# MAdrid1011/transplat

Measured on AMD Instinct MI355X. Metric: novel views/sec at 256x256, 2 ctx views; PSNR parity vs reference, higher is better.
Workload: dtype fp32 (bf16x3 dense, >= TF32) + bf16x3 attention + fp32 raster; 1 GPU; e2e TranSplat test_step: 1 scene(s) x (2 ctx -> 3 tgt) 256x256; dense mode bf16x3 (split-bf16 products, fp32 accumulation; >= TF32), window-attention mode bf16x3; parallelism=scene-shard x1

## Files before the change

### include/transplat_hip.h

```cpp
#ifndef TRANSPLAT_HIP_H
#define TRANSPLAT_HIP_H

#include <stddef.h>
#include <stdint.h>

#ifdef __cplusplus
extern "C" {
#endif

#define TSPLAT_OK 0
#define TSPLAT_EINVAL (-1)
#define TSPLAT_EHIP (-2)

int tsplat_version(void);

int tsplat_set_debug(int32_t on);

int tsplat_prof_enable(int32_t kernel_id);
int tsplat_prof_read(double* total_ms, int32_t* launches);

typedef struct tsplat_raster_desc {
    int32_t num_gaussians;
    int32_t num_views;
    int32_t views_per_scene;
    int32_t height;
    int32_t width;
    int32_t sh_coeffs;
    int32_t sh_degree;
    int32_t capacity;
} tsplat_raster_desc;

size_t tsplat_raster_workspace_bytes(int32_t num_gaussians, int32_t num_views, int32_t height,
                                     int32_t width, int32_t capacity);

size_t tsplat_raster_num_rendered_offset(int32_t num_gaussians, int32_t num_views, int32_t height,
                                         int32_t width);

int tsplat_raster_fwd(const tsplat_raster_desc* desc,
                      const float* means, const float* cov, const float* shs,
                      const float* opacity, const float* viewmat, const float* projmat,
                      const float* campos, const float* tanfov, const float* bg,
                      const float* scene_scale,
                      float* out_color, int32_t* out_radii,
                      void* workspace, int32_t* status, void* stream);


int tsplat_depth_softmax_fwd(const float* logits, const float* disp, float* coarse, float* pdf_max, int32_t n,
                             int32_t depths, int32_t hw, void* stream);

int tsplat_depth_tail_fwd(const float* fullres, const float* head, const float* near, const float* far, float* depth,
                          float* density, int32_t batch, int32_t views, int32_t hw, void* stream);

int tsplat_raster_cameras(const float* extrinsics, const float* intrinsics, const float* near, const float* far,
                          const float* bg, int32_t bg_per_view, int32_t scale_invariant, int32_t num_views,
                          float* viewmat, float* projmat, float* campos, float* tanfov, float* bg_out, float* scale,
                          void* stream);


int tsplat_uv_coarse_fwd(const float* feat, const float* cams, const float* disp, float* out,
                         int32_t batch, int32_t height, int32_t width, int32_t channels,
                         int32_t depths, void* stream);

int tsplat_uv_cross_fwd(const float* value, const float* key, const float* cams,
                        const float* disp, const float* offsets, const float* logits, float* out,
                        int32_t batch, int32_t height, int32_t width, int32_t channels,
                        int32_t depths, int32_t points, void* stream);

int tsplat_uv_cross_table_fwd(const float* table, const float* cams, const float* disp, const float* offsets,
                              const float* logits, float* out, int32_t batch, int32_t height, int32_t width,
                              int32_t channels, int32_t depths, int32_t points, void* stream);

int tsplat_msda_fwd(const float* value, const float* loc, const float* weights, float* out,
                    int32_t n, int32_t height, int32_t width, int32_t channels, int32_t queries,
                    int32_t points, void* stream);

int tsplat_msda_raw_fwd(const float* value, const float* ow, float* out, int32_t n, int32_t height, int32_t width,
                        int32_t channels, int32_t points, int32_t ow_stride, void* stream);

int tsplat_ms_deform_attn_fwd(const float* value, const int64_t* spatial_shapes, const int64_t* level_start_index,
                              const float* sampling_loc, const float* attn_weight, float* out, int32_t batch,
                              int32_t num_keys, int32_t num_heads, int32_t head_dim, int32_t num_levels,
                              int32_t num_queries, int32_t num_points, int32_t im2col_step, void* stream);

int tsplat_sh_rotation_fwd(const float* rotations, const double* basis, float* out, int32_t num_cameras,
                           int32_t d_sh, void* stream);

size_t tsplat_group_norm_workspace_bytes(int32_t n, int32_t c, int64_t hw, int32_t groups);
int tsplat_group_norm_fwd(const float* x, const float* pre_bias, const float* gamma, const float* beta,
                          const float* residual,
                          float* y, void* workspace, int32_t n, int32_t c, int64_t hw, int32_t groups,
                          float eps, int32_t act, void* stream);
int tsplat_group_norm_cat_res_fwd(const float* x, const float* pre_bias, const float* gamma, const float* beta,
                                  const float* residual, const float* residual2, int32_t c1, float* y,
                                  void* workspace, int32_t n, int32_t c, int64_t hw, int32_t groups, float eps,
                                  int32_t act, void* stream);
int tsplat_group_norm_bf16_fwd(const void* x, const float* pre_bias, const float* gamma, const float* beta,
                               const void* residual, void* y, void* workspace, int32_t n, int32_t c, int64_t hw,
                               int32_t groups, float eps, int32_t act, void* stream);

int tsplat_bias_act_fwd(const float* x, const float* bias, const float* residual, float* y, int32_t n, int32_t c,
                        int64_t hw, int32_t act, void* stream);

int tsplat_bias_act_nhwc_fwd(const float* x, const float* bias, const float* res1, const float* res2, float* y,
                             int64_t rows, int32_t c, int32_t act, void* stream);

int tsplat_residual_ln_fwd(const float* x, const float* y, const float* ls, const float* ln_w, const float* ln_b,
                           float ln_eps, float* x_out, float* n_out, int32_t rows, int32_t dim, void* stream);
int tsplat_layer_norm128_fwd(const void* y, int32_t y_bf16, const float* residual, const float* ln_w,
                             const float* ln_b, float ln_eps, void* out, int32_t out_bf16, int32_t rows,
                             void* stream);
int tsplat_residual_ln_bf16_fwd(const float* x, const void* y, const float* ls, const float* ln_w, const float* ln_b,
                                float ln_eps, float* x_out, void* n_out, int32_t rows, int32_t dim, void* stream);

int tsplat_gaussian_adapter_fwd(const float* raw, const float* depths, const float* densities,
                                const float* cams, const float* sh_rot, float* means, float* cov,
                                float* harmonics, float* opacities, int32_t batch, int32_t views,
                                int32_t height, int32_t width, int32_t raw_ch, int32_t d_sh,
                                float scale_min, float scale_max, float opacity_exponent,
                                int32_t gaussians_per_pixel, int32_t raw_nchw, void* stream);

size_t tsplat_win_attn_workspace_bytes(int32_t batch, int32_t height, int32_t width, int32_t key_views,
                                       int32_t splits);
int tsplat_win_attn_fwd(const float* q, const float* k, const float* v, float* out, void* workspace,
                        int32_t batch, int32_t height, int32_t width, int32_t channels,
                        int32_t key_views, int32_t splits, int32_t with_shift, void* stream);

int32_t tsplat_win_attn_split(int32_t batch, int32_t height, int32_t width, int32_t key_views, int32_t splits);
int tsplat_win_attn_partials_fwd(const float* q, const float* k, const float* v, void* workspace, int32_t batch,
                                 int32_t height, int32_t width, int32_t channels, int32_t key_views,
                                 int32_t splits, int32_t with_shift, int32_t key_batch_shift, void* stream);

int tsplat_split_kv_bf16x3(const float* k, const float* v, void* kv_x3, int64_t n, void* stream);
int tsplat_linear_f32_split_x3_fwd(const float* x1, int32_t k1, const float* w, float* out, void* kv_x3, int32_t M,
                                   int32_t N, int32_t x3_from, int32_t flags, void* stream);
int tsplat_win_attn_x3_fwd(const float* q, const void* kv_x3, float* out, void* workspace, int32_t batch,
                           int32_t height, int32_t width, int32_t channels, int32_t key_views, int32_t splits,
                           int32_t with_shift, void* stream);
int tsplat_win_attn_x3_partials_fwd(const float* q, const void* kv_x3, void* workspace, int32_t batch, int32_t height,
                                    int32_t width, int32_t channels, int32_t key_views, int32_t splits,
                                    int32_t with_shift, int32_t key_batch_shift, void* stream);

size_t tsplat_win_attn_bf16_workspace_bytes(int32_t batch, int32_t height, int32_t width, int32_t key_views,
                                            int32_t splits);
int tsplat_win_attn_bf16_fwd(const void* q, const void* k, const void* v, void* out, void* workspace,
                             int32_t batch, int32_t height, int32_t width, int32_t channels,
                             int32_t key_views, int32_t splits, int32_t with_shift, void* stream);
int tsplat_win_attn_bf16_shift_fwd(const void* q, const void* k, const void* v, void* out, void* workspace,
                                   int32_t batch, int32_t height, int32_t width, int32_t channels,
                                   int32_t key_views, int32_t splits, int32_t with_shift,
                                   int32_t key_batch_shift, void* stream);

int tsplat_linear_f32_fwd(const float* x1, int32_t k1, const float* x2, int32_t k2, const float* w,
                          const float* bias, const float* ln_gamma, const float* ln_beta, float ln_eps,
                          const float* residual, float* out, int64_t split_stride, int32_t M, int32_t N,
                          int32_t flags, void* stream);

int tsplat_linear_f32_attn_merge_fwd(const float* partials, int32_t batch, int32_t height, int32_t width,
                                     int32_t key_views, int32_t splits, int32_t with_shift, const float* w,
                                     const float* ln_gamma, const float* ln_beta, float ln_eps,
                                     const float* residual, float* out, int32_t N, int32_t flags, void* stream);

int tsplat_small_inverse(const float* in, float* out, int32_t n, int32_t dim, void* stream);

int tsplat_mha_f32_fwd(const float* qkv, float* out, int32_t batch, int32_t tokens, int32_t heads,
                       int32_t head_dim, float scale, void* stream);
int tsplat_mha_bias_f32_fwd(const float* qkv, const float* bias, float* out, int32_t batch, int32_t tokens,
                            int32_t heads, int32_t head_dim, float scale, void* stream);
int tsplat_mha_x3_presplit_fwd(const void* qkv_hi, const void* qkv_lo, float* out, int32_t batch, int32_t tokens,
                               int32_t heads, int32_t head_dim, float scale, void* stream);
size_t tsplat_mha_x3_workspace_bytes(int32_t batch, int32_t tokens, int32_t heads, int32_t head_dim);
int tsplat_mha_x3_fwd(const float* qkv, const float* bias, float* out, void* workspace, int32_t batch,
                      int32_t tokens, int32_t heads, int32_t head_dim, float scale, void* stream);

int tsplat_qkv_attention_cf_fwd(const float* qkv, float* out, int32_t batch, int32_t heads, int32_t views,
                                int32_t tokens_per_view, int32_t head_dim, float scale, void* stream);

int tsplat_conv2d_f32_fwd(const float* x1, int32_t c1, const float* x2, int32_t c2, const float* w_packed,
                          const float* bias, float* y, int32_t batch, int32_t height, int32_t width, int32_t c_out,
                          int32_t ksize, int32_t stride, int32_t upsample, int32_t ksplit, void* stream);

int tsplat_conv2d_f32_zsplit_fwd(const float* x1, int32_t c1, const float* x2, int32_t c2, const float* w_packed,
                                 const float* bias, float* y, int32_t batch, int32_t height, int32_t width,
                                 int32_t c_out, int32_t ksize, int32_t stride, int32_t upsample, int32_t ksplit,
                                 int32_t zsplit, float* partials, int32_t* counters, void* stream);

int tsplat_conv2d_bf16x3_fwd(const float* x1, int32_t c1, const float* x2, int32_t c2, const void* w_packed,
                             const float* bias, float* y, int32_t batch, int32_t height, int32_t width,
                             int32_t c_out, int32_t ksize, int32_t stride, int32_t upsample, int32_t ksplit,
                             int32_t zsplit, float* partials, int32_t* counters, void* stream);

size_t tsplat_wino_weight_floats(int32_t c_out, int32_t c_in);
int tsplat_wino_weight_f32(const float* weight, float* w_packed, int32_t c_out, int32_t c_in, void* stream);
int tsplat_conv3x3_wino_f32_fwd(const float* x, const float* w_packed, const float* bias, float* y, int32_t batch,
                                int32_t c_in, int32_t height, int32_t width, int32_t c_out, int32_t act,
                                void* stream);
int tsplat_conv3x3_wino_cat_f32_fwd(const float* const* srcs, const int32_t* chans, int32_t n_src,
                                    const float* w_packed, const float* bias, float* y, int32_t batch,
                                    int32_t height, int32_t width, int32_t c_out, int32_t act, void* stream);

size_t tsplat_wino_weight_bf16x3_bytes(int32_t c_out, int32_t c_in);
int tsplat_wino_weight_bf16x3(const float* weight, void* w_packed, int32_t c_out, int32_t c_in, void* stream);
int tsplat_conv3x3_wino_bf16x3_fwd(const float* x, const void* w_packed, const float* bias, float* y, int32_t batch,
                                   int32_t c_in, int32_t height, int32_t width, int32_t c_out, int32_t act,
                                   void* stream);
int tsplat_conv3x3_wino_bf16x3_cat_fwd(const float* const* srcs, const int32_t* chans, int32_t n_src,
                                       const void* w_packed, const float* bias, float* y, int32_t batch,
                                       int32_t height, int32_t width, int32_t c_out, int32_t act, void* stream);
int tsplat_conv3x3_wino_bf16x3_ex_fwd(const float* const* srcs, const int32_t* chans, int32_t n_src,
                                      const void* w_packed, const float* bias, const float* residual,
                                      const float* residual2, float* y, int32_t batch, int32_t height, int32_t width,
                                      int32_t c_out, int32_t act, int32_t relu_in, void* stream);

int32_t tsplat_conv3x3_few_form(int32_t batch, int32_t c_in, int32_t height, int32_t width, int32_t c_out);
int tsplat_conv3x3_few_bf16x3_fwd(const float* const* srcs, const int32_t* chans, int32_t n_src,
                                  const void* w_packed, const float* bias, const float* residual,
                                  const float* residual2, float* y, int32_t batch, int32_t height, int32_t width,
                                  int32_t c_out, int32_t act, int32_t relu_in, void* stream);

int tsplat_split_bf16x3(const float* x, void* out, int64_t rows, int32_t k, int32_t weight_order, void* stream);

size_t tsplat_conv2d_bf16_weight_bytes(int32_t c_out, int32_t c_in, int32_t ksize);
int tsplat_conv2d_bf16_fwd(const void* const* srcs, const int32_t* src_channels, int32_t n_src, const int32_t* src_f32,
                           const void* w_packed, const float* bias, void* y, int32_t batch, int32_t height,
                           int32_t width, int32_t c_out, int32_t ksize, int32_t upsample, int32_t act,
                           void* stream);

int tsplat_conv2d_f32_nhwc_fwd(const float* x, int32_t c_in, const float* w_packed, const float* bias,
                               const float* residual, float* y, int32_t batch, int32_t height, int32_t width,
                               int32_t c_out, int32_t ksize, int32_t relu_in, int32_t ksplit, void* stream);

int tsplat_upsample_bilinear_act_fwd(const float* x, const float* bias, float* y, int32_t n, int32_t c,
                                     int32_t height, int32_t width, int32_t scale, int32_t act, void* stream);

int tsplat_resize_bilinear_nhwc_fwd(const float* x, float* y, int32_t n, int32_t height, int32_t width, int32_t c,
                                    int32_t out_height, int32_t out_width, void* stream);

int tsplat_resize_bilinear_nchw_fwd(const float* x, float* y, int32_t planes, int32_t height, int32_t width,
                                    int32_t out_height, int32_t out_width, void* stream);

size_t tsplat_gemm_x3_pack_bytes(int32_t n, int32_t k);
int tsplat_gemm_x3_pack(const float* w, void* wp, int32_t n, int32_t k, void* stream);
int tsplat_gemm_x3_fwd(const float* x, const void* wp, const float* bias, float* out, int32_t m, int32_t n, int32_t k,
                       int32_t ksplit, int32_t act, void* stream);

int tsplat_residual_ln_slabs_fwd(const float* x, const float* y, int32_t nslab, const float* ls, const float* ln_w,
                                 const float* ln_b, float ln_eps, float* x_out, float* n_out, int32_t rows,
                                 int32_t dim, void* stream);

int tsplat_timestamp(void* buf, int32_t slot, void* stream);

#ifdef __cplusplus
}
#endif

#endif
```

### transplat_amd/_lib.py

```python
from __future__ import annotations

import ctypes
import os
from pathlib import Path

import torch

_LIB_PATH = Path(os.environ.get("TSPLAT_LIB") or Path(__file__).resolve().parent / "libtransplat_hip.so")
_lib = None


class RasterDesc(ctypes.Structure):
    _fields_ = [
        ("num_gaussians", ctypes.c_int32),
        ("num_views", ctypes.c_int32),
        ("views_per_scene", ctypes.c_int32),
        ("height", ctypes.c_int32),
        ("width", ctypes.c_int32),
        ("sh_coeffs", ctypes.c_int32),
        ("sh_degree", ctypes.c_int32),
        ("capacity", ctypes.c_int32),
    ]


_P = ctypes.c_void_p
_I32 = ctypes.c_int32

SIGNATURES = {
    "tsplat_version": (ctypes.c_int, []),
    "tsplat_set_debug": (ctypes.c_int, [_I32]),
    "tsplat_timestamp": (ctypes.c_int, [_P, _I32, _P]),
    "tsplat_prof_enable": (ctypes.c_int, [_I32]),
    "tsplat_prof_read": (ctypes.c_int, [ctypes.POINTER(ctypes.c_double), ctypes.POINTER(_I32)]),
    "tsplat_raster_workspace_bytes": (ctypes.c_size_t, [_I32, _I32, _I32, _I32, _I32]),
    "tsplat_raster_num_rendered_offset": (ctypes.c_size_t, [_I32, _I32, _I32, _I32]),
    "tsplat_raster_fwd": (
        ctypes.c_int,
        [ctypes.POINTER(RasterDesc)] + [_P] * 15,
    ),
    "tsplat_uv_coarse_fwd": (ctypes.c_int, [_P] * 4 + [_I32] * 5 + [_P]),
    "tsplat_uv_cross_fwd": (ctypes.c_int, [_P] * 7 + [_I32] * 6 + [_P]),
    "tsplat_uv_cross_table_fwd": (ctypes.c_int, [_P] * 6 + [_I32] * 6 + [_P]),
    "tsplat_msda_fwd": (ctypes.c_int, [_P] * 4 + [_I32] * 6 + [_P]),
    "tsplat_msda_raw_fwd": (ctypes.c_int, [_P, _P, _P] + [_I32] * 6 + [_P]),
    "tsplat_ms_deform_attn_fwd": (ctypes.c_int, [_P] * 6 + [_I32] * 8 + [_P]),
    "tsplat_win_attn_workspace_bytes": (ctypes.c_size_t, [_I32] * 5),
    "tsplat_win_attn_fwd": (ctypes.c_int, [_P] * 5 + [_I32] * 7 + [_P]),
    "tsplat_win_attn_bf16_workspace_bytes": (ctypes.c_size_t, [_I32] * 5),
    "tsplat_win_attn_bf16_fwd": (ctypes.c_int, [_P] * 5 + [_I32] * 7 + [_P]),
    "tsplat_win_attn_bf16_shift_fwd": (ctypes.c_int, [_P] * 5 + [_I32] * 8 + [_P]),
    "tsplat_group_norm_workspace_bytes": (ctypes.c_size_t, [_I32, _I32, ctypes.c_int64, _I32]),
    "tsplat_group_norm_fwd": (ctypes.c_int, [_P] * 7 + [_I32, _I32, ctypes.c_int64, _I32, ctypes.c_float, _I32, _P]),
    "tsplat_group_norm_cat_res_fwd": (ctypes.c_int, [_P] * 6 + [_I32, _P, _P, _I32, _I32, ctypes.c_int64, _I32,
                                                                ctypes.c_float, _I32, _P]),
    "tsplat_layer_norm128_fwd": (ctypes.c_int, [_P, _I32, _P, _P, _P, ctypes.c_float, _P, _I32, _I32, _P]),
    "tsplat_group_norm_bf16_fwd": (ctypes.c_int, [_P] * 7 + [_I32, _I32, ctypes.c_int64, _I32, ctypes.c_float, _I32,
                                                            _P]),
    "tsplat_sh_rotation_fwd": (ctypes.c_int, [_P] * 3 + [_I32] * 2 + [_P]),
    "tsplat_gaussian_adapter_fwd": (ctypes.c_int, [_P] * 9 + [_I32] * 6 + [ctypes.c_float] * 3 + [_I32, _I32, _P]),
    "tsplat_win_attn_split": (_I32, [_I32] * 5),
    "tsplat_depth_softmax_fwd": (ctypes.c_int, [_P] * 4 + [_I32] * 3 + [_P]),
    "tsplat_depth_tail_fwd": (ctypes.c_int, [_P] * 6 + [_I32] * 3 + [_P]),
    "tsplat_raster_cameras": (ctypes.c_int, [_P] * 5 + [_I32] * 3 + [_P] * 7),
    "tsplat_small_inverse": (ctypes.c_int, [_P, _P, _I32, _I32, _P]),
    "tsplat_mha_f32_fwd": (ctypes.c_int, [_P, _P, _I32, _I32, _I32, _I32, ctypes.c_float, _P]),
    "tsplat_mha_bias_f32_fwd": (ctypes.c_int, [_P, _P, _P, _I32, _I32, _I32, _I32, ctypes.c_float, _P]),
    "tsplat_mha_x3_workspace_bytes": (ctypes.c_size_t, [_I32] * 4),
    "tsplat_mha_x3_fwd": (ctypes.c_int, [_P, _P, _P, _P, _I32, _I32, _I32, _I32, ctypes.c_float, _P]),
    "tsplat_mha_x3_presplit_fwd": (ctypes.c_int, [_P, _P, _P, _I32, _I32, _I32, _I32, ctypes.c_float, _P]),
    "tsplat_qkv_attention_cf_fwd": (ctypes.c_int, [_P, _P] + [_I32] * 5 + [ctypes.c_float, _P]),
    "tsplat_conv2d_f32_fwd": (ctypes.c_int, [_P, _I32, _P, _I32, _P, _P, _P] + [_I32] * 8 + [_P]),
    "tsplat_conv2d_f32_zsplit_fwd": (ctypes.c_int, [_P, _I32, _P, _I32, _P, _P, _P] + [_I32] * 9 + [_P, _P, _P]),
    "tsplat_conv2d_bf16x3_fwd": (ctypes.c_int, [_P, _I32, _P, _I32, _P, _P, _P] + [_I32] * 9 + [_P, _P, _P]),
    "tsplat_resize_bilinear_nhwc_fwd": (ctypes.c_int, [_P, _P] + [_I32] * 6 + [_P]),
    "tsplat_resize_bilinear_nchw_fwd": (ctypes.c_int, [_P, _P] + [_I32] * 5 + [_P]),
    "tsplat_upsample_bilinear_act_fwd": (ctypes.c_int, [_P, _P, _P] + [_I32] * 6 + [_P]),
    "tsplat_conv2d_f32_nhwc_fwd": (ctypes.c_int, [_P, _I32, _P, _P, _P, _P] + [_I32] * 7 + [_P]),
    "tsplat_residual_ln_fwd": (ctypes.c_int, [_P] * 5 + [ctypes.c_float, _P, _P, _I32, _I32, _P]),
    "tsplat_residual_ln_slabs_fwd": (ctypes.c_int, [_P, _P, _I32, _P, _P, _P, ctypes.c_float, _P, _P, _I32, _I32, _P]),
    "tsplat_gemm_x3_pack_bytes": (ctypes.c_size_t, [_I32, _I32]),
    "tsplat_gemm_x3_pack": (ctypes.c_int, [_P, _P, _I32, _I32, _P]),
    "tsplat_gemm_x3_fwd": (ctypes.c_int, [_P, _P, _P, _P, _I32, _I32, _I32, _I32, _I32, _P]),
    "tsplat_residual_ln_bf16_fwd": (ctypes.c_int, [_P] * 5 + [ctypes.c_float, _P, _P, _I32, _I32, _P]),
    "tsplat_bias_act_fwd": (ctypes.c_int, [_P] * 4 + [_I32, _I32, ctypes.c_int64, _I32, _P]),
    "tsplat_bias_act_nhwc_fwd": (ctypes.c_int, [_P, _P, _P, _P, _P, ctypes.c_int64, _I32, _I32, _P]),
    "tsplat_win_attn_partials_fwd": (ctypes.c_int, [_P] * 4 + [_I32] * 8 + [_P]),
    "tsplat_split_kv_bf16x3": (ctypes.c_int, [_P, _P, _P, ctypes.c_int64, _P]),
    "tsplat_linear_f32_split_x3_fwd": (ctypes.c_int, [_P, _I32, _P, _P, _P] + [_I32] * 4 + [_P]),
    "tsplat_win_attn_x3_fwd": (ctypes.c_int, [_P] * 4 + [_I32] * 7 + [_P]),
    "tsplat_win_attn_x3_partials_fwd": (ctypes.c_int, [_P] * 3 + [_I32] * 8 + [_P]),
    "tsplat_linear_f32_attn_merge_fwd": (ctypes.c_int, [_P] + [_I32] * 6 + [_P] * 3 + [ctypes.c_float, _P, _P, _I32,
                                                                                       _I32, _P]),
    "tsplat_linear_f32_fwd": (ctypes.c_int, [_P, _I32, _P, _I32] + [_P] * 4 + [ctypes.c_float, _P, _P, ctypes.c_int64]
                              + [_I32] * 3 + [_P]),
    "tsplat_wino_weight_floats": (ctypes.c_size_t, [_I32, _I32]),
    "tsplat_wino_weight_f32": (ctypes.c_int, [_P, _P, _I32, _I32, _P]),
    "tsplat_conv3x3_wino_f32_fwd": (ctypes.c_int, [_P, _P, _P, _P] + [_I32] * 6 + [_P]),
    "tsplat_conv3x3_wino_cat_f32_fwd": (ctypes.c_int, [_P, _P, _I32, _P, _P, _P] + [_I32] * 5 + [_P]),
    "tsplat_wino_weight_bf16x3_bytes": (ctypes.c_size_t, [_I32, _I32]),
    "tsplat_wino_weight_bf16x3": (ctypes.c_int, [_P, _P, _I32, _I32, _P]),
    "tsplat_conv3x3_wino_bf16x3_fwd": (ctypes.c_int, [_P, _P, _P, _P] + [_I32] * 6 + [_P]),
    "tsplat_conv3x3_wino_bf16x3_cat_fwd": (ctypes.c_int, [_P, _P, _I32, _P, _P, _P] + [_I32] * 5 + [_P]),
    "tsplat_conv3x3_wino_bf16x3_ex_fwd": (ctypes.c_int, [_P, _P, _I32, _P, _P, _P, _P, _P] + [_I32] * 6 + [_P]),
    "tsplat_conv3x3_few_form": (ctypes.c_int32, [_I32] * 5),
    "tsplat_conv3x3_few_bf16x3_fwd": (ctypes.c_int, [_P, _P, _I32, _P, _P, _P, _P, _P] + [_I32] * 6 + [_P]),
    "tsplat_split_bf16x3": (ctypes.c_int, [_P, _P, ctypes.c_int64, _I32, _I32, _P]),
    "tsplat_conv2d_bf16_weight_bytes": (ctypes.c_size_t, [_I32, _I32, _I32]),
    "tsplat_conv2d_bf16_fwd": (ctypes.c_int, [_P, _P, _I32, _P, _P, _P, _P] + [_I32] * 7 + [_P]),
}

ERRORS = {-1: "invalid argument", -2: "HIP launch error"}


def lib_path() -> Path:
    return _LIB_PATH


def load(build_if_missing: bool = False):
    global _lib
    if _lib is not None:
        return _lib
    if not _LIB_PATH.exists():
        if build_if_missing:
            from .build import build

            build()
        else:
            raise RuntimeError(
                f"transplat HIP library not built ({_LIB_PATH}); run `python -m transplat_amd.build`"
            )
    lib = ctypes.CDLL(str(_LIB_PATH), mode=os.RTLD_NOW | os.RTLD_GLOBAL)
    for name, (res, args) in SIGNATURES.items():
        fn = getattr(lib, name)
        fn.restype = res
        fn.argtypes = args
    if os.environ.get("TSPLAT_DEBUG", "0") == "1":
        lib.tsplat_set_debug(1)
    _lib = lib
    return lib


def debug_enabled() -> bool:
    lib = load()
    was = lib.tsplat_set_debug(1)
    lib.tsplat_set_debug(was)
    return bool(was)


ROUTE_HOOK = None


def check(status: int, what: str, route: str | None = None) -> None:
    if status != 0:
        raise RuntimeError(f"{what} failed: {ERRORS.get(status, status)}")
    if ROUTE_HOOK is not None:
        ROUTE_HOOK(what, route)


def ptr(t: torch.Tensor | None) -> int | None:
    if t is None:
        return None
    if not t.is_cuda:
        raise RuntimeError("transplat HIP ops need device tensors (no CPU path)")
    return t.data_ptr()


def stream_ptr(device: torch.device | None = None) -> int:
    return torch.cuda.current_stream(device).cuda_stream


PROF_IDS = {"raster_preprocess": 1, "raster_scan": 2, "raster_scatter": 3, "raster_render": 4,
            "uv_coarse": 5, "uv_cross": 6, "msda": 7, "win_attn": 8, "raster": 9,
            "group_norm": 10, "uv_cross_table": 11, "linear": 12, "mha": 13, "conv": 14, "wino_conv": 15,
            "gemm_x3": 16}


def prof_enable(name: str | None) -> None:
    check(load().tsplat_prof_enable(PROF_IDS[name] if name else 0), "tsplat_prof_enable")


def prof_read() -> tuple[float, int]:
    ms = ctypes.c_double(0.0)
    n = _I32(0)
    check(load().tsplat_prof_read(ctypes.byref(ms), ctypes.byref(n)), "tsplat_prof_read")
    return ms.value, n.value
```

### transplat_amd/csrc/convfew.hip

```cpp
#include <stdlib.h>

#include "common.h"
#include "prof.h"

namespace tsplat {
namespace convfew {

typedef __bf16 bf16x8 __attribute__((ext_vector_type(8)));
typedef float floatx16 __attribute__((ext_vector_type(16)));

constexpr int kMaxSrc = 6;
constexpr int kCols = 64;
constexpr int kRC = kCols + 8;
constexpr int kCP = 32;
constexpr int kPS = kCP + 8;
constexpr int kMaxCi = 128;

struct Args {
    const float* src[kMaxSrc];
    int cs[kMaxSrc];
    int nsrc;
    const uint4* wp;
    const float* bias;
    const float* res;
    const float* res2;
    float* y;
    int n, ci, h, w, co, ng, cot;
    int act;
    int relu_in;
    int rb, cb;
    int abl;
};

__device__ __forceinline__ float act_fn(float v, int act) {
    if (act == 1) return fmaxf(v, 0.0f);
    if (act == 2) return 0.5f * v * (1.0f + erff(v * 0.70710678118654752f));
    return v;
}

__device__ __forceinline__ const float* plane(const Args& a, int img, int c) {
    const float* p = nullptr;
    if (c >= a.ci) return p;
#pragma unroll
    for (int q = 0; q < kMaxSrc; ++q) {
        if (!p && q < a.nsrc) {
            if (c < a.cs[q])
                p = a.src[q] + ((size_t)img * a.cs[q] + c) * ((size_t)a.h * a.w);
            else
                c -= a.cs[q];
        }
    }
    return p;
}

template <int TR, int CB>
__global__ void __launch_bounds__(256, 2) conv_kernel(Args a) {
    constexpr int R = TR + 2;
    constexpr int WPC = 4 / CB;
    constexpr int UPW = 2 * TR / WPC;
    static_assert(UPW >= 1 && (2 * TR) % WPC == 0, "segments per wave");
    constexpr int HL = R * kRC * kPS;
    __shared__ __attribute__((aligned(16))) __bf16 sIn[2 * HL];
    __shared__ const float* sPlane[kMaxCi];

    const int tid = threadIdx.x, lane = tid & 63, wid = tid >> 6;
    const int blk = blockIdx.x;
    const int img = blk / (a.rb * a.cb), rem = blk - img * (a.rb * a.cb);
    const int y0 = (rem / a.cb) * TR, x0 = (rem % a.cb) * kCols;
    const int cob0 = blockIdx.y * CB;
    const int cbw = wid / WPC, wi = wid % WPC;

    floatx16 acc[UPW];
#pragma unroll
    for (int u = 0; u < UPW; ++u)
#pragma unroll
        for (int e = 0; e < 16; ++e) acc[u][e] = 0.0f;
    for (int c = tid; c < kMaxCi; c += 256) sPlane[c] = plane(a, img, min(c, a.ci - 1));
    __syncthreads();

    constexpr int ITEMS = (kCP / 8) * R * (kRC / 4);
    constexpr int IPT = (ITEMS + 255) / 256;
    auto stage = [&](int pass) __attribute__((always_inline)) {
        float4 v[IPT][8];
#pragma unroll
        for (int k = 0; k < IPT; ++k) {
            const int it = tid + 256 * k;
            const int q = it & 3, c4 = (it >> 2) % (kRC / 4), row = (it >> 2) / (kRC / 4);
            const int y = y0 - 1 + row, x = x0 - 4 + 4 * c4;
            const bool in = it < ITEMS && y >= 0 && y < a.h && x >= 0 && x < a.w;
            const int c0 = pass * kCP + 8 * q;
            const size_t po = (size_t)min(max(y, 0), a.h - 1) * a.w + min(max(x, 0), a.w - 4);
#pragma unroll
            for (int j = 0; j < 8; ++j) {
                const bool ok = in && c0 + j < a.ci && !(a.abl & 1);
                const float* p = sPlane[min(c0 + j, kMaxCi - 1)] + po;
                typedef float f4v __attribute__((ext_vector_type(4)));
                const f4v f = *(const __attribute__((address_space(1))) f4v*)p;
                v[k][j] = ok ? make_float4(f.x, f.y, f.z, f.w) : make_float4(0.f, 0.f, 0.f, 0.f);
            }
        }
#pragma unroll
        for (int k = 0; k < IPT; ++k) {
            const int it = tid + 256 * k;
            if (it >= ITEMS) break;
            const int q = it & 3, c4 = (it >> 2) % (kRC / 4), row = (it >> 2) / (kRC / 4);
#pragma unroll
            for (int px = 0; px < 4; ++px) {
                bf16x8 hi, lo;
#pragma unroll
                for (int j = 0; j < 8; ++j) {
                    float f = px == 0 ? v[k][j].x : px == 1 ? v[k][j].y : px == 2 ? v[k][j].z : v[k][j].w;
                    if (a.relu_in) f = fmaxf(f, 0.0f);
                    hi[j] = (__bf16)f;
                    lo[j] = (__bf16)(f - (float)hi[j]);
                }
                const int off = (row * kRC + 4 * c4 + px) * kPS + 8 * q;
                *reinterpret_cast<bf16x8*>(&sIn[off]) = hi;
                *reinterpret_cast<bf16x8*>(&sIn[HL + off]) = lo;
            }
        }
    };

    const int h = lane >> 5, n = lane & 31;
    const int passes = (a.ng + 1) / 2;
    uint4 ar[18][2];
    for (int pass = 0; pass < passes; ++pass) {
        if (pass) __syncthreads();
        stage(pass);
        {
            const int cot = min(cob0 + cbw, a.cot - 1);
#pragma unroll
            for (int ks = 0; ks < 18; ++ks) {
                const int g = 2 * pass + (ks & 1);
                const uint4* p = a.wp + ((((size_t)cot * 9 + (ks >> 1)) * a.ng + min(g, a.ng - 1)) * 2) * 64 + lane;
                ar[ks][0] = g < a.ng ? p[0] : make_uint4(0u, 0u, 0u, 0u);
                ar[ks][1] = g < a.ng ? p[64] : make_uint4(0u, 0u, 0u, 0u);
            }
        }
        __syncthreads();
        if (a.abl & 2) continue;
#pragma unroll
        for (int ks = 0; ks < 18; ++ks) {
            const int tap = ks >> 1, gl = ks & 1;
            const int dy = tap / 3, dx = tap - 3 * dy;
            const bf16x8 ah = __builtin_bit_cast(bf16x8, ar[ks][0]);
            const bf16x8 al = __builtin_bit_cast(bf16x8, ar[ks][1]);
#pragma unroll
            for (int u = 0; u < UPW; ++u) {
                const int seg = wi + WPC * u;
                const int i = seg >> 1, j = (seg & 1) * 32 + n;
                const int off = ((i + dy) * kRC + j + dx + 3) * kPS + 16 * gl + 8 * h;
                const bf16x8 bh = *reinterpret_cast<const bf16x8*>(&sIn[off]);
                const bf16x8 bl = *reinterpret_cast<const bf16x8*>(&sIn[HL + off]);
                acc[u] = __builtin_amdgcn_mfma_f32_32x32x16_bf16(al, bh, acc[u], 0, 0, 0);
                acc[u] = __builtin_amdgcn_mfma_f32_32x32x16_bf16(ah, bl, acc[u], 0, 0, 0);
                acc[u] = __builtin_amdgcn_mfma_f32_32x32x16_bf16(ah, bh, acc[u], 0, 0, 0);
            }
        }
    }

    const size_t hw = (size_t)a.h * a.w;
    if (a.abl & 4) {
        if (acc[0][0] == 12345.0f) a.y[0] = acc[UPW - 1][15];
        return;
    }
    constexpr int CO = 32 * CB;
    static_assert(CO * TR * kCols * 4 <= 2 * HL * 2, "output tile fits the input image's LDS");
    float* sOut = reinterpret_cast<float*>(sIn);
    __syncthreads();
#pragma unroll
    for (int u = 0; u < UPW; ++u) {
        const int seg = wi + WPC * u;
        const int i = seg >> 1, j = (seg & 1) * 32 + n;
#pragma unroll
        for (int r = 0; r < 16; ++r) {
            const int col = 32 * cbw + 8 * (r >> 2) + 4 * h + (r & 3);
            sOut[(col * TR + i) * kCols + j] = acc[u][r];
        }
    }
    __syncthreads();
    constexpr int V4 = CO * TR * (kCols / 4);
#pragma unroll 4
    for (int idx = tid; idx < V4; idx += 256) {
        const int c4 = idx % (kCols / 4), t2 = idx / (kCols / 4);
        const int i = t2 % TR, col = t2 / TR;
        const int o = 32 * cob0 + col, yy = y0 + i, xx = x0 + 4 * c4;
        if (o >= a.co || yy >= a.h || xx >= a.w) continue;
        const size_t off = ((size_t)img * a.co + o) * hw + (size_t)yy * a.w + xx;
        float4 v = *reinterpret_cast<const float4*>(&sOut[(col * TR + i) * kCols + 4 * c4]);
        const float bb = a.bias ? a.bias[o] : 0.0f;
        v = make_float4(act_fn(v.x + bb, a.act), act_fn(v.y + bb, a.act), act_fn(v.z + bb, a.act),
                        act_fn(v.w + bb, a.act));
        if (a.res) {
            const float4 r = *reinterpret_cast<const float4*>(a.res + off);
            v = make_float4(v.x + r.x, v.y + r.y, v.z + r.z, v.w + r.w);
        }
        if (a.res2) {
            const float4 r = *reinterpret_cast<const float4*>(a.res2 + off);
            v = make_float4(v.x + r.x, v.y + r.y, v.z + r.z, v.w + r.w);
        }
        *reinterpret_cast<float4*>(a.y + off) = v;
    }
}

}
}

using namespace tsplat;

extern "C" int32_t tsplat_conv3x3_few_form(int32_t n, int32_t ci, int32_t h, int32_t w, int32_t co) {
    if (n <= 0 || ci <= 0 || h <= 0 || w <= 0 || co <= 0 || w % 4 || co > 64 || ci > convfew::kMaxCi) return 0;
    const long cbk = (w + convfew::kCols - 1) / convfew::kCols;
    if (co > 32) return 22;
    if (const char* e = getenv("TSPLAT_FEW_TR")) {
        const int tr = atoi(e);
        if (tr == 4 || tr == 2) return tr * 10 + 1;
    }
    return (long)n * ((h + 3) / 4) * cbk >= 256 ? 41 : 21;
}

extern "C" int tsplat_conv3x3_few_bf16x3_fwd(const float* const* srcs, const int32_t* chans, int32_t nsrc,
                                             const void* packed, const float* bias, const float* residual,
                                             const float* residual2, float* y, int32_t n, int32_t h, int32_t w,
                                             int32_t co, int32_t act, int32_t relu_in, void* stream_) {
    using namespace tsplat::convfew;
    if (!srcs || !chans || nsrc <= 0 || nsrc > kMaxSrc || !packed || !y || act < 0 || act > 2) return TSPLAT_EINVAL;
    Args a;
    int ci = 0;
    for (int q = 0; q < kMaxSrc; ++q) {
        a.src[q] = q < nsrc ? srcs[q] : nullptr;
        a.cs[q] = q < nsrc ? chans[q] : 0;
        if (q < nsrc && (!srcs[q] || chans[q] <= 0 || (reinterpret_cast<uintptr_t>(srcs[q]) & 15)))
            return TSPLAT_EINVAL;
        ci += a.cs[q];
    }
    const int form = tsplat_conv3x3_few_form(n, ci, h, w, co);
    if (!form) return TSPLAT_EINVAL;
    a.nsrc = nsrc;
    a.wp = (const uint4*)packed;
    a.bias = bias;
    a.res = residual;
    a.res2 = residual2;
    a.y = y;
    a.n = n;
    a.ci = ci;
    a.h = h;
    a.w = w;
    a.co = co;
    a.ng = (ci + 15) / 16;
    a.cot = (co + 31) / 32;
    a.act = act;
    a.relu_in = relu_in != 0;
    a.abl = getenv("TSPLAT_FEW_ABL") ? atoi(getenv("TSPLAT_FEW_ABL")) : 0;
    const int tr = form / 10, cb = form % 10;
    a.rb = (h + tr - 1) / tr;
    a.cb = (w + kCols - 1) / kCols;
    const dim3 grid(n * a.rb * a.cb, (a.cot + cb - 1) / cb);
    hipStream_t stream = (hipStream_t)stream_;
    const prof::ExtEvents ev = prof::ext_events(prof::kWinoConv);
#define TSPLAT_FEW(TR, CB)                                                                                 \
    hipExtLaunchKernelGGL((convfew::conv_kernel<TR, CB>), grid, dim3(256), 0, stream, ev.start, ev.stop, 0, a)
    switch (form) {
        case 41: TSPLAT_FEW(4, 1); break;
        case 21: TSPLAT_FEW(2, 1); break;
        default: TSPLAT_FEW(2, 2); break;
    }
#undef TSPLAT_FEW
    TSPLAT_CHECK_LAUNCH();
    return TSPLAT_OK;
}
```

### transplat_amd/csrc/groupnorm.hip

```cpp
#include "common.h"
#include "prof.h"

namespace tsplat {
namespace gn {

constexpr int kThreads = 256;
constexpr int kChunk = 4096;

struct Welford {
    float n, mean, m2;
};

__device__ __forceinline__ Welford combine(Welford a, Welford b) {
    const float n = a.n + b.n;
    if (n == 0.f) return a;
    const float d = b.mean - a.mean;
    const float wb = b.n / n;
    return {n, a.mean + d * wb, a.m2 + b.m2 + d * d * a.n * wb};
}

__device__ __forceinline__ Welford push(Welford w, float x) {
    w.n += 1.f;
    const float d = x - w.mean;
    w.mean += d / w.n;
    w.m2 += d * (x - w.mean);
    return w;
}

__device__ __forceinline__ Welford wave_reduce(Welford w) {
#pragma unroll
    for (int off = kWave / 2; off > 0; off >>= 1) {
        Welford o{__shfl_xor(w.n, off), __shfl_xor(w.mean, off), __shfl_xor(w.m2, off)};
        w = combine(w, o);
    }
    return w;
}

typedef __bf16 bf16x4_t __attribute__((ext_vector_type(4)));
__device__ __forceinline__ float ld1(const float* p) { return *p; }
__device__ __forceinline__ float ld1(const __bf16* p) { return (float)*p; }
__device__ __forceinline__ void st1(float* p, float v) { *p = v; }
__device__ __forceinline__ void st1(__bf16* p, float v) { *p = (__bf16)v; }
__device__ __forceinline__ float4 ld4(const float* p) { return *reinterpret_cast<const float4*>(p); }
__device__ __forceinline__ float4 ld4(const __bf16* p) {
    const bf16x4_t v = *reinterpret_cast<const bf16x4_t*>(p);
    return make_float4((float)v[0], (float)v[1], (float)v[2], (float)v[3]);
}
__device__ __forceinline__ void st4(float* p, float4 v) { *reinterpret_cast<float4*>(p) = v; }
__device__ __forceinline__ void st4(__bf16* p, float4 v) {
    *reinterpret_cast<bf16x4_t*>(p) = bf16x4_t{(__bf16)v.x, (__bf16)v.y, (__bf16)v.z, (__bf16)v.w};
}

template <bool VEC, typename T>
__global__ void __launch_bounds__(kThreads)
stats_kernel(const T* __restrict__ x, const float* __restrict__ pb, float2* __restrict__ partials,
             int64_t L, int S, int HW, int cpg, int G) {
    const int chunk = blockIdx.x, seg = blockIdx.y, tid = threadIdx.x;
    const int64_t start = (int64_t)chunk * kChunk;
    const int n_local = (int)min((int64_t)kChunk, L - start);
    const T* p = x + (int64_t)seg * L + start;
    const int c0 = (seg % G) * cpg;
    Welford w{0.f, 0.f, 0.f};
    if (VEC) {
#pragma unroll
        for (int k = 0; k < kChunk / (4 * kThreads); ++k) {
            const int i = (k * kThreads + tid) * 4;
            if (i < n_local) {
                const float b = pb ? pb[c0 + (int)((start + i) / HW)] : 0.f;
                const float4 v = ld4(p + i);
                w = push(w, v.x + b);
                w = push(w, v.y + b);
                w = push(w, v.z + b);
                w = push(w, v.w + b);
            }
        }
    } else {
        for (int i = tid; i < n_local; i += kThreads)
            w = push(w, ld1(p + i) + (pb ? pb[c0 + (int)((start + i) / HW)] : 0.f));
    }
    w = wave_reduce(w);
    __shared__ Welford sw[kThreads / kWave];
    if ((tid & (kWave - 1)) == 0) sw[tid / kWave] = w;
    __syncthreads();
    if (tid == 0) {
        Welford t = sw[0];
#pragma unroll
        for (int i = 1; i < kThreads / kWave; ++i) t = combine(t, sw[i]);
        partials[(int64_t)seg * S + chunk] = make_float2(t.mean, t.m2);
    }
}

template <int ACT>
__device__ __forceinline__ float activate(float v) {
    if (ACT == 1) return v / (1.0f + expf(-v));
    if (ACT == 2) return 0.5f * v * (1.0f + erff(v * 0.70710678118654752f));
    if (ACT == 3) return fmaxf(v, 0.0f);
    return v;
}

template <int ACT>
__device__ __forceinline__ float post_residual(float v) { return ACT == 3 ? fmaxf(v, 0.0f) : v; }

template <typename T>
__device__ __forceinline__ const T* res_at(const T* res, const T* res2, int c1, int C, int64_t e, int n, int ch,
                                           int HW) {
    if (c1 >= C) return res + e;
    const int64_t p = e - ((int64_t)n * C + ch) * HW;
    return ch < c1 ? res + ((int64_t)n * c1 + ch) * HW + p : res2 + ((int64_t)n * (C - c1) + (ch - c1)) * HW + p;
}

template <bool VEC, int ACT, bool RES, typename T>
__global__ void __launch_bounds__(kThreads)
apply_kernel(const T* __restrict__ x, const float* __restrict__ pb, const float2* __restrict__ partials,
             const float* __restrict__ gamma, const float* __restrict__ beta,
             const T* __restrict__ res, const T* __restrict__ res2, int c1, T* __restrict__ y, int64_t L, int S,
             int HW, int C, int cpg, int G, float eps) {
    const int chunk = blockIdx.x, seg = blockIdx.y, tid = threadIdx.x;
    __shared__ float s_scale_shift[2];
    if (tid < kWave) {
        Welford w{0.f, 0.f, 0.f};
        for (int i = tid; i < S; i += kWave) {
            const float2 pm = partials[(int64_t)seg * S + i];
            const float n = (float)min((int64_t)kChunk, L - (int64_t)i * kChunk);
            w = combine(w, Welford{n, pm.x, pm.y});
        }
        w = wave_reduce(w);
        if (tid == 0) {
            s_scale_shift[0] = w.mean;
            s_scale_shift[1] = rsqrtf(w.m2 / (float)L + eps);
        }
    }
    __syncthreads();
    const float mean = s_scale_shift[0], rstd = s_scale_shift[1];
    const int g = seg % G;
    const int64_t start = (int64_t)chunk * kChunk;
    const int n_local = (int)min((int64_t)kChunk, L - start);
    const int64_t base = (int64_t)seg * L + start;
    if (VEC) {
#pragma unroll
        for (int k = 0; k < kChunk / (4 * kThreads); ++k) {
            const int i = (k * kThreads + tid) * 4;
            if (i < n_local) {
                const int c = g * cpg + (int)((start + i) / HW);
                const float sc = rstd * gamma[c];
                const float sh = beta[c] - sc * mean;
                const float b = pb ? pb[c] : 0.f;
                float4 v = ld4(x + base + i);
                v.x += b;
                v.y += b;
                v.z += b;
                v.w += b;
                v.x = activate<ACT>(v.x * sc + sh);
                v.y = activate<ACT>(v.y * sc + sh);
                v.z = activate<ACT>(v.z * sc + sh);
                v.w = activate<ACT>(v.w * sc + sh);
                if (RES) {
                    const float4 r = ld4(res_at(res, res2, c1, C, base + i, seg / G, c, HW));
                    v.x = post_residual<ACT>(v.x + r.x);
                    v.y = post_residual<ACT>(v.y + r.y);
                    v.z = post_residual<ACT>(v.z + r.z);
                    v.w = post_residual<ACT>(v.w + r.w);
                }
                st4(y + base + i, v);
            }
        }
    } else {
        for (int i = tid; i < n_local; i += kThreads) {
            const int c = g * cpg + (int)((start + i) / HW);
            const float sc = rstd * gamma[c];
            float v = activate<ACT>((ld1(x + base + i) + (pb ? pb[c] : 0.f)) * sc + (beta[c] - sc * mean));
            if (RES) v = post_residual<ACT>(v + ld1(res_at(res, res2, c1, C, base + i, seg / G, c, HW)));
            st1(y + base + i, v);
        }
    }
}

constexpr int kFusedThreads = 512;

__device__ __forceinline__ float block_sum512(float v, float* red) {
#pragma unroll
    for (int off = kWave / 2; off > 0; off >>= 1) v += __shfl_xor(v, off);
    const int w = threadIdx.x >> 6;
    __syncthreads();
    if ((threadIdx.x & (kWave - 1)) == 0) red[w] = v;
    __syncthreads();
    float t = 0.f;
#pragma unroll
    for (int i = 0; i < kFusedThreads / kWave; ++i) t += red[i];
    return t;
}

template <int NPT, int ACT, bool RES, typename T>
__global__ void __launch_bounds__(kFusedThreads)
fused_kernel(const T* __restrict__ x, const float* __restrict__ pb, const float* __restrict__ gamma,
             const float* __restrict__ beta, const T* __restrict__ res, const T* __restrict__ res2, int c1,
             T* __restrict__ y, int L, int HW, int cpg, int G, float eps) {
    __shared__ float red[kFusedThreads / kWave];
    const int seg = blockIdx.x, tid = threadIdx.x;
    const int g = seg % G;
    const int64_t base = (int64_t)seg * L;
    float4 v[NPT / 4];
    float s = 0.f;
#pragma unroll
    for (int k = 0; k < NPT / 4; ++k) {
        const int i = (k * kFusedThreads + tid) * 4;
        if (i < L) {
            v[k] = ld4(x + base + i);
            if (pb) {
                const float b = pb[g * cpg + i / HW];
                v[k].x += b;
                v[k].y += b;
                v[k].z += b;
                v[k].w += b;
            }
            s += (v[k].x + v[k].y) + (v[k].z + v[k].w);
        }
    }
    const float mean = block_sum512(s, red) / (float)L;
    float q = 0.f;
#pragma unroll
    for (int k = 0; k < NPT / 4; ++k) {
        const int i = (k * kFusedThreads + tid) * 4;
        if (i < L) {
            const float a = v[k].x - mean, b = v[k].y - mean, c = v[k].z - mean, d = v[k].w - mean;
            q += (a * a + b * b) + (c * c + d * d);
        }
    }
    const float rstd = rsqrtf(block_sum512(q, red) / (float)L + eps);
#pragma unroll
    for (int k = 0; k < NPT / 4; ++k) {
        const int i = (k * kFusedThreads + tid) * 4;
        if (i < L) {
            const int c = g * cpg + i / HW;
            const float sc = rstd * gamma[c], sh = beta[c] - sc * mean;
            float4 o;
            o.x = activate<ACT>(v[k].x * sc + sh);
            o.y = activate<ACT>(v[k].y * sc + sh);
            o.z = activate<ACT>(v[k].z * sc + sh);
            o.w = activate<ACT>(v[k].w * sc + sh);
            if (RES) {
                const float4 r = ld4(res_at(res, res2, c1, cpg * G, base + i, seg / G, c, HW));
                o.x = post_residual<ACT>(o.x + r.x);
                o.y = post_residual<ACT>(o.y + r.y);
                o.z = post_residual<ACT>(o.z + r.z);
                o.w = post_residual<ACT>(o.w + r.w);
            }
            st4(y + base + i, o);
        }
    }
}

}
}

using namespace tsplat;

extern "C" size_t tsplat_group_norm_workspace_bytes(int32_t n, int32_t c, int64_t hw, int32_t groups) {
    if (n <= 0 || c <= 0 || hw <= 0 || groups <= 0 || c % groups) return 0;
    const int64_t L = (int64_t)(c / groups) * hw;
    const int64_t S = (L + gn::kChunk - 1) / gn::kChunk;
    return (size_t)n * groups * S * sizeof(float2);
}

template <typename T>
static int group_norm_launch(const T* x, const float* pre_bias, const float* gamma, const float* beta,
                             const T* residual, T* y, void* workspace, int32_t n, int32_t c, int64_t hw,
                             int32_t groups, float eps, int32_t act, void* stream_, const T* residual2 = nullptr,
                             int32_t c1 = -1) {
    using namespace tsplat::gn;
    if (!x || !gamma || !beta || !y || !workspace) return TSPLAT_EINVAL;
    if (c1 < 0) c1 = c;
    if (c1 > c || (c1 < c && (!residual || !residual2 || c1 == 0))) return TSPLAT_EINVAL;
    if (n <= 0 || c <= 0 || hw <= 0 || groups <= 0 || c % groups || act < 0 || act > 3 ||
        hw > INT32_MAX)
        return TSPLAT_EINVAL;
    const int cpg = c / groups;
    const int64_t L = (int64_t)cpg * hw;
    const int64_t S = (L + kChunk - 1) / kChunk;
    if (S > INT32_MAX || (int64_t)n * groups > 65535) return TSPLAT_EINVAL;
    hipStream_t stream = (hipStream_t)stream_;
    const dim3 grid((unsigned)S, (unsigned)(n * groups));
    const uintptr_t al = 4 * sizeof(T);
    const bool vec = (hw % 4 == 0) && ((uintptr_t)x % al == 0) && ((uintptr_t)y % al == 0) &&
                     (!residual || (uintptr_t)residual % al == 0) && (!residual2 || (uintptr_t)residual2 % al == 0);
    if (vec && L <= (int64_t)kFusedThreads * 32 && x != y) {
        const int npt = L <= kFusedThreads * 4 ? 4 : L <= kFusedThreads * 8 ? 8 : L <= kFusedThreads * 16 ? 16 : 32;
        TSPLAT_PROF_BEGIN(prof::kGroupNorm, stream);
#define TSPLAT_GN_F(N, A, R)                                                                                  \
    hipLaunchKernelGGL((fused_kernel<N, A, R, T>), dim3((unsigned)(n * groups)), dim3(kFusedThreads), 0, stream, x, \
                       pre_bias, gamma, beta, residual, residual2, c1, y, (int)L, (int)hw, cpg, groups, eps)
#define TSPLAT_GN_FA(N, R)                   \
    switch (act) {                           \
        case 0: TSPLAT_GN_F(N, 0, R); break; \
        case 1: TSPLAT_GN_F(N, 1, R); break; \
        case 2: TSPLAT_GN_F(N, 2, R); break; \
        default: TSPLAT_GN_F(N, 3, R); break; \
    }
#define TSPLAT_GN_FN(N)                                                       \
    if (residual) { TSPLAT_GN_FA(N, true) } else { TSPLAT_GN_FA(N, false) }
        switch (npt) {
            case 4: TSPLAT_GN_FN(4); break;
            case 8: TSPLAT_GN_FN(8); break;
            case 16: TSPLAT_GN_FN(16); break;
            default: TSPLAT_GN_FN(32); break;
        }
#undef TSPLAT_GN_FN
#undef TSPLAT_GN_FA
#undef TSPLAT_GN_F
        TSPLAT_PROF_END(prof::kGroupNorm, stream);
        TSPLAT_CHECK_LAUNCH();
        return TSPLAT_OK;
    }
    float2* part = (float2*)workspace;
    TSPLAT_PROF_BEGIN(prof::kGroupNorm, stream);
    if (vec)
        hipLaunchKernelGGL((stats_kernel<true, T>), grid, dim3(kThreads), 0, stream, x, pre_bias, part, L, (int)S,
                           (int)hw, cpg, groups);
    else
        hipLaunchKernelGGL((stats_kernel<false, T>), grid, dim3(kThreads), 0, stream, x, pre_bias, part, L, (int)S,
                           (int)hw, cpg, groups);
    TSPLAT_CHECK_LAUNCH();
#define TSPLAT_GN_APPLY(V, A, R)                                                                   \
    hipLaunchKernelGGL((apply_kernel<V, A, R, T>), grid, dim3(kThreads), 0, stream, x, pre_bias, part, gamma,  \
                       beta, residual, residual2, c1, y, L, (int)S, (int)hw, c, cpg, groups, eps)
#define TSPLAT_GN_ACT(V, R)              \
    switch (act) {                       \
        case 0: TSPLAT_GN_APPLY(V, 0, R); break; \
        case 1: TSPLAT_GN_APPLY(V, 1, R); break; \
        case 2: TSPLAT_GN_APPLY(V, 2, R); break; \
        default: TSPLAT_GN_APPLY(V, 3, R); break; \
    }
    if (vec) {
        if (residual) { TSPLAT_GN_ACT(true, true) } else { TSPLAT_GN_ACT(true, false) }
    } else {
        if (residual) { TSPLAT_GN_ACT(false, true) } else { TSPLAT_GN_ACT(false, false) }
    }
#undef TSPLAT_GN_ACT
#undef TSPLAT_GN_APPLY
    TSPLAT_PROF_END(prof::kGroupNorm, stream);
    TSPLAT_CHECK_LAUNCH();
    return TSPLAT_OK;
}

extern "C" int tsplat_group_norm_fwd(const float* x, const float* pre_bias, const float* gamma, const float* beta,
                                     const float* residual, float* y, void* workspace, int32_t n,
                                     int32_t c, int64_t hw, int32_t groups, float eps, int32_t act,
                                     void* stream_) {
    return group_norm_launch<float>(x, pre_bias, gamma, beta, residual, y, workspace, n, c, hw, groups, eps, act,
                                    stream_);
}

extern "C" int tsplat_group_norm_cat_res_fwd(const float* x, const float* pre_bias, const float* gamma,
                                             const float* beta, const float* residual, const float* residual2,
                                             int32_t c1, float* y, void* workspace, int32_t n, int32_t c, int64_t hw,
                                             int32_t groups, float eps, int32_t act, void* stream_) {
    if (c1 <= 0 || c1 >= c || !residual || !residual2) return TSPLAT_EINVAL;
    return group_norm_launch<float>(x, pre_bias, gamma, beta, residual, y, workspace, n, c, hw, groups, eps, act,
                                    stream_, residual2, c1);
}

extern "C" int tsplat_group_norm_bf16_fwd(const void* x, const float* pre_bias, const float* gamma,
                                          const float* beta, const void* residual, void* y, void* workspace,
                                          int32_t n, int32_t c, int64_t hw, int32_t groups, float eps, int32_t act,
                                          void* stream_) {
    return group_norm_launch<__bf16>((const __bf16*)x, pre_bias, gamma, beta, (const __bf16*)residual, (__bf16*)y,
                                     workspace, n, c, hw, groups, eps, act, stream_);
}

namespace tsplat {
namespace gn {

template <int ACT, bool RES>
__global__ void __launch_bounds__(kThreads)
bias_act_kernel(const float* __restrict__ x, const float* __restrict__ bias, const float* __restrict__ res,
                float* __restrict__ y, int n4, int hw4, int C) {
    const int i = blockIdx.x * kThreads + threadIdx.x;
    if (i >= n4) return;
    const int c = (i / hw4) % C;
    const float b = bias ? bias[c] : 0.f;
    float4 v = reinterpret_cast<const float4*>(x)[i];
    v.x = activate<ACT>(v.x + b);
    v.y = activate<ACT>(v.y + b);
    v.z = activate<ACT>(v.z + b);
    v.w = activate<ACT>(v.w + b);
    if (RES) {
        const float4 r = reinterpret_cast<const float4*>(res)[i];
        v.x = post_residual<ACT>(v.x + r.x);
        v.y = post_residual<ACT>(v.y + r.y);
        v.z = post_residual<ACT>(v.z + r.z);
        v.w = post_residual<ACT>(v.w + r.w);
    }
    reinterpret_cast<float4*>(y)[i] = v;
}

}
}

extern "C" int tsplat_bias_act_fwd(const float* x, const float* bias, const float* residual, float* y, int32_t n,
                                   int32_t c, int64_t hw, int32_t act, void* stream_) {
    using namespace tsplat::gn;
    if (!x || !y || n <= 0 || c <= 0 || hw <= 0 || hw % 4 || act < 0 || act > 3) return TSPLAT_EINVAL;
    if ((uintptr_t)x % 16 || (uintptr_t)y % 16 || (residual && (uintptr_t)residual % 16)) return TSPLAT_EINVAL;
    const int64_t n4 = (int64_t)n * c * hw / 4;
    if (n4 > INT32_MAX) return TSPLAT_EINVAL;
    hipStream_t stream = (hipStream_t)stream_;
    const dim3 grid((unsigned)((n4 + kThreads - 1) / kThreads));
#define TSPLAT_BA(A, R) \
    hipLaunchKernelGGL((bias_act_kernel<A, R>), grid, dim3(kThreads), 0, stream, x, bias, residual, y, (int)n4, (int)(hw / 4), c)
#define TSPLAT_BA_ACT(R)                   \
    switch (act) {                         \
        case 0: TSPLAT_BA(0, R); break;    \
        case 1: TSPLAT_BA(1, R); break;    \
        case 2: TSPLAT_BA(2, R); break;    \
        default: TSPLAT_BA(3, R); break;   \
    }
    if (residual) { TSPLAT_BA_ACT(true) } else { TSPLAT_BA_ACT(false) }
#undef TSPLAT_BA_ACT
#undef TSPLAT_BA
    TSPLAT_CHECK_LAUNCH();
    return TSPLAT_OK;
}

namespace tsplat {
namespace gn {

template <int ACT, int NRES>
__global__ void __launch_bounds__(kThreads)
bias_act_nhwc_kernel(const float* __restrict__ x, const float* __restrict__ bias, const float* __restrict__ r1,
                     const float* __restrict__ r2, float* __restrict__ y, int n4, int c4) {
    const int i = blockIdx.x * kThreads + threadIdx.x;
    if (i >= n4) return;
    float4 v = reinterpret_cast<const float4*>(x)[i];
    if (bias) {
        const float4 b = reinterpret_cast<const float4*>(bias)[i % c4];
        v.x += b.x;
        v.y += b.y;
        v.z += b.z;
        v.w += b.w;
    }
    v.x = activate<ACT>(v.x);
    v.y = activate<ACT>(v.y);
    v.z = activate<ACT>(v.z);
    v.w = activate<ACT>(v.w);
    if (NRES >= 1) {
        const float4 r = reinterpret_cast<const float4*>(r1)[i];
        v.x += r.x;
        v.y += r.y;
        v.z += r.z;
        v.w += r.w;
    }
    if (NRES >= 2) {
        const float4 r = reinterpret_cast<const float4*>(r2)[i];
        v.x += r.x;
        v.y += r.y;
        v.z += r.z;
        v.w += r.w;
    }
    reinterpret_cast<float4*>(y)[i] = v;
}

}
}

extern "C" int tsplat_bias_act_nhwc_fwd(const float* x, const float* bias, const float* res1, const float* res2,
                                        float* y, int64_t rows, int32_t c, int32_t act, void* stream_) {
    using namespace tsplat::gn;
    if (!x || !y || rows <= 0 || c <= 0 || c % 4 || !(act == 0 || act == 2 || act == 3)) return TSPLAT_EINVAL;
    if (res2 && !res1) return TSPLAT_EINVAL;
    if ((uintptr_t)x % 16 || (uintptr_t)y % 16 || (bias && (uintptr_t)bias % 16) || (res1 && (uintptr_t)res1 % 16) ||
        (res2 && (uintptr_t)res2 % 16))
        return TSPLAT_EINVAL;
    const int64_t n4 = rows * c / 4;
    if (n4 > INT32_MAX) return TSPLAT_EINVAL;
    hipStream_t stream = (hipStream_t)stream_;
    const dim3 grid((unsigned)((n4 + kThreads - 1) / kThreads));
    const int nres = res2 ? 2 : (res1 ? 1 : 0);
#define TSPLAT_BAN(A, R) \
    hipLaunchKernelGGL((bias_act_nhwc_kernel<A, R>), grid, dim3(kThreads), 0, stream, x, bias, res1, res2, y, (int)n4, c / 4)
#define TSPLAT_BAN_R(A)                  \
    switch (nres) {                      \
        case 0: TSPLAT_BAN(A, 0); break; \
        case 1: TSPLAT_BAN(A, 1); break; \
        default: TSPLAT_BAN(A, 2); break; \
    }
    if (act == 0) { TSPLAT_BAN_R(0) } else if (act == 2) { TSPLAT_BAN_R(2) } else { TSPLAT_BAN_R(3) }
#undef TSPLAT_BAN_R
#undef TSPLAT_BAN
    TSPLAT_CHECK_LAUNCH();
    return TSPLAT_OK;
}

namespace tsplat {
namespace gn {

template <int V4, typename TY, typename TN>
__global__ void __launch_bounds__(kThreads)
residual_ln_kernel(const float* __restrict__ x, const TY* __restrict__ y, const float* __restrict__ ls,
                   const float* __restrict__ w, const float* __restrict__ b, float* __restrict__ x_out,
                   TN* __restrict__ n_out, int rows, float eps, int nslab) {
    const int row = blockIdx.x * (kThreads / kWave) + (threadIdx.x >> 6);
    const int lane = threadIdx.x & 63;
    if (row >= rows) return;
    constexpr int D = 256 * V4;
    const size_t off = (size_t)row * D;
    float4 v[V4];
    float s = 0.f;
#pragma unroll
    for (int k = 0; k < V4; ++k) {
        const int c = 4 * (lane + 64 * k);
        v[k] = *reinterpret_cast<const float4*>(x + off + c);
        if (y) {
            float4 t = ld4(y + off + c);
            for (int sl = 1; sl < nslab; ++sl) {
                const float4 u = ld4(y + (size_t)sl * rows * D + off + c);
                t.x += u.x;
                t.y += u.y;
                t.z += u.z;
                t.w += u.w;
            }
            float4 g = make_float4(1.f, 1.f, 1.f, 1.f);
            if (ls) g = *reinterpret_cast<const float4*>(ls + c);
            v[k].x += g.x * t.x;
            v[k].y += g.y * t.y;
            v[k].z += g.z * t.z;
            v[k].w += g.w * t.w;
        }
        s += (v[k].x + v[k].y) + (v[k].z + v[k].w);
    }
#pragma unroll
    for (int o = 32; o > 0; o >>= 1) s += __shfl_xor(s, o);
    const float mean = s * (1.0f / D);
    float q = 0.f;
#pragma unroll
    for (int k = 0; k < V4; ++k) {
        const float a = v[k].x - mean, bb = v[k].y - mean, cc = v[k].z - mean, d = v[k].w - mean;
        q += (a * a + bb * bb) + (cc * cc + d * d);
    }
#pragma unroll
    for (int o = 32; o > 0; o >>= 1) q += __shfl_xor(q, o);
    const float rstd = rsqrtf(q * (1.0f / D) + eps);
#pragma unroll
    for (int k = 0; k < V4; ++k) {
        const int c = 4 * (lane + 64 * k);
        if (x_out) *reinterpret_cast<float4*>(x_out + off + c) = v[k];
        const float4 g = *reinterpret_cast<const float4*>(w + c), bt = *reinterpret_cast<const float4*>(b + c);
        st4(n_out + off + c, make_float4((v[k].x - mean) * rstd * g.x + bt.x, (v[k].y - mean) * rstd * g.y + bt.y,
                                         (v[k].z - mean) * rstd * g.z + bt.z, (v[k].w - mean) * rstd * g.w + bt.w));
    }
}

}
}

template <typename TY, typename TN>
static int residual_ln_launch(const float* x, const TY* y, const float* ls, const float* ln_w, const float* ln_b,
                              float ln_eps, float* x_out, TN* n_out, int32_t rows, int32_t dim, void* stream_,
                              int32_t nslab = 1) {
    using namespace tsplat::gn;
    if (!x || !ln_w || !ln_b || !n_out || rows <= 0 || (ls && !y) || nslab < 1) return TSPLAT_EINVAL;
    if (y && !x_out) return TSPLAT_EINVAL;
    hipStream_t stream = (hipStream_t)stream_;
    const dim3 grid((rows + kThreads / kWave - 1) / (kThreads / kWave));
#define TSPLAT_RLN(V)                                                                                   \
    hipLaunchKernelGGL((residual_ln_kernel<V, TY, TN>), grid, dim3(kThreads), 0, stream, x, y, ls, ln_w, ln_b, \
                       x_out, n_out, rows, ln_eps, nslab)
    switch (dim) {
        case 256: TSPLAT_RLN(1); break;
        case 512: TSPLAT_RLN(2); break;
        case 768: TSPLAT_RLN(3); break;
        case 1024: TSPLAT_RLN(4); break;
        default: return TSPLAT_EINVAL;
    }
#undef TSPLAT_RLN
    TSPLAT_CHECK_LAUNCH();
    return TSPLAT_OK;
}

extern "C" int tsplat_residual_ln_fwd(const float* x, const float* y, const float* ls, const float* ln_w,
                                      const float* ln_b, float ln_eps, float* x_out, float* n_out, int32_t rows,
                                      int32_t dim, void* stream_) {
    return residual_ln_launch<float, float>(x, y, ls, ln_w, ln_b, ln_eps, x_out, n_out, rows, dim, stream_);
}

extern "C" int tsplat_residual_ln_slabs_fwd(const float* x, const float* y, int32_t nslab, const float* ls,
                                            const float* ln_w, const float* ln_b, float ln_eps, float* x_out,
                                            float* n_out, int32_t rows, int32_t dim, void* stream_) {
    if (!y) return TSPLAT_EINVAL;
    return residual_ln_launch<float, float>(x, y, ls, ln_w, ln_b, ln_eps, x_out, n_out, rows, dim, stream_, nslab);
}

extern "C" int tsplat_residual_ln_bf16_fwd(const float* x, const void* y, const float* ls, const float* ln_w,
                                           const float* ln_b, float ln_eps, float* x_out, void* n_out, int32_t rows,
                                           int32_t dim, void* stream_) {
    return residual_ln_launch<__bf16, __bf16>(x, (const __bf16*)y, ls, ln_w, ln_b, ln_eps, x_out, (__bf16*)n_out,
                                              rows, dim, stream_);
}

namespace tsplat {
namespace gn {

template <typename TY, typename TO>
__global__ void __launch_bounds__(kThreads)
ln128_kernel(const TY* __restrict__ y, const float* __restrict__ res, const float* __restrict__ w,
             const float* __restrict__ b, TO* __restrict__ out, int rows, float eps) {
    const int row = (blockIdx.x * kThreads + threadIdx.x) >> 5;
    const int l = threadIdx.x & 31;
    if (row >= rows) return;
    const size_t off = (size_t)row * 128 + 4 * l;
    const float4 v = ld4(y + off);
    float s = (v.x + v.y) + (v.z + v.w);
#pragma unroll
    for (int o = 16; o > 0; o >>= 1) s += __shfl_xor(s, o, 32);
    const float mean = s * (1.0f / 128.0f);
    const float a = v.x - mean, bb = v.y - mean, c = v.z - mean, d = v.w - mean;
    float q = (a * a + bb * bb) + (c * c + d * d);
#pragma unroll
    for (int o = 16; o > 0; o >>= 1) q += __shfl_xor(q, o, 32);
    const float rstd = rsqrtf(q * (1.0f / 128.0f) + eps);
    const float4 g = *reinterpret_cast<const float4*>(w + 4 * l), bt = *reinterpret_cast<const float4*>(b + 4 * l);
    float4 n = make_float4(a * rstd * g.x + bt.x, bb * rstd * g.y + bt.y, c * rstd * g.z + bt.z, d * rstd * g.w + bt.w);
    if (res) {
        const float4 r = *reinterpret_cast<const float4*>(res + off);
        n = make_float4(r.x + n.x, r.y + n.y, r.z + n.z, r.w + n.w);
    }
    st4(out + off, n);
}

}
}

extern "C" int tsplat_layer_norm128_fwd(const void* y, int32_t y_bf16, const float* residual, const float* ln_w,
                                        const float* ln_b, float ln_eps, void* out, int32_t out_bf16, int32_t rows,
                                        void* stream_) {
    using namespace tsplat::gn;
    if (!y || !ln_w || !ln_b || !out || rows <= 0) return TSPLAT_EINVAL;
    const uintptr_t al = y_bf16 ? 8 : 16;
    if ((uintptr_t)y % al || (uintptr_t)out % (out_bf16 ? 8 : 16) || (residual && (uintptr_t)residual % 16) ||
        (uintptr_t)ln_w % 16 || (uintptr_t)ln_b % 16)
        return TSPLAT_EINVAL;
    hipStream_t stream = (hipStream_t)stream_;
    const dim3 grid((unsigned)(((int64_t)rows * 32 + kThreads - 1) / kThreads));
#define TSPLAT_LN128(TY, TO)                                                                                 \
    hipLaunchKernelGGL((ln128_kernel<TY, TO>), grid, dim3(kThreads), 0, stream, (const TY*)y, residual, ln_w, ln_b, \
                       (TO*)out, rows, ln_eps)
    if (y_bf16 && out_bf16) TSPLAT_LN128(__bf16, __bf16);
    else if (y_bf16) TSPLAT_LN128(__bf16, float);
    else if (out_bf16) TSPLAT_LN128(float, __bf16);
    else TSPLAT_LN128(float, float);
#undef TSPLAT_LN128
    TSPLAT_CHECK_LAUNCH();
    return TSPLAT_OK;
}
```

### transplat_amd/csrc/winoconv3.hip

```cpp
#include <stdlib.h>

#include "common.h"
#include "prof.h"

#ifndef TSPLAT_W3_ABL
#define TSPLAT_W3_ABL 0
#endif

namespace tsplat {
namespace wino3 {

typedef __bf16 bf16x8 __attribute__((ext_vector_type(8)));
typedef float floatx16 __attribute__((ext_vector_type(16)));

constexpr int kMaxSrc = 6;
constexpr int kMaxCiPad = 1024;
constexpr int kPersistCiPad = 512;

__device__ uint4 g_zero16 = {0u, 0u, 0u, 0u};

#ifndef TSPLAT_W3_STAMP
#define TSPLAT_W3_STAMP 0
#endif
#if TSPLAT_W3_STAMP
__device__ unsigned long long* g_w3_stamps = nullptr;
#define W3_STAMP(slot)                                                                                  \
    do {                                                                                                \
        if (threadIdx.x == 0 && g_w3_stamps)                                                            \
            g_w3_stamps[(size_t)(blockIdx.y * gridDim.x + blockIdx.x) * 8 + (slot)] = wall_clock64();   \
    } while (0)
#else
#define W3_STAMP(slot) do {} while (0)
#endif

struct Args {
    const float* src[kMaxSrc];
    int cs[kMaxSrc];
    int nsrc;
    const uint4* u;
    const float* bias;
    float* y;
    int n, ci, h, w, co, ci_pad, cobs, nchunk;
    int th, tw, tbx, tby, bx, by;
    int act;
    int relu_in;
    const float* res;
    const float* res2;
    int cob_base;
};

__device__ __forceinline__ float act_fn(float v, int act) {
    if (act == 1) return fmaxf(v, 0.0f);
    if (act == 2) return 0.5f * v * (1.0f + erff(v * 0.70710678118654752f));
    return v;
}

typedef __bf16 bf16x2 __attribute__((ext_vector_type(2)));
typedef float floatx2 __attribute__((ext_vector_type(2)));

__device__ __forceinline__ uint32_t pack_bf16(float a, float b) {
    return __builtin_bit_cast(uint32_t, __builtin_convertvector((floatx2){a, b}, bf16x2));
}

__device__ __forceinline__ void split_pair(float a, float b, uint32_t& hi, uint32_t& lo) {
    hi = pack_bf16(a, b);
    const float ah = __builtin_bit_cast(float, hi << 16), bh = __builtin_bit_cast(float, hi & 0xffff0000u);
    lo = pack_bf16(a - ah, b - bh);
}

__global__ void __launch_bounds__(256) weight_kernel(const float* __restrict__ g, __bf16* __restrict__ u, int co,
                                                     int ci, int ci_pad, int cobs) {
    const int idx = blockIdx.x * 256 + threadIdx.x;
    if (idx >= cobs * 32 * ci_pad) return;
    const int c = idx % ci_pad, o = idx / ci_pad;
    float k[3][3];
    const bool ok = o < co && c < ci;
#pragma unroll
    for (int i = 0; i < 3; ++i)
#pragma unroll
        for (int j = 0; j < 3; ++j) k[i][j] = ok ? g[((size_t)o * ci + c) * 9 + 3 * i + j] : 0.0f;
    float t[4][3];
#pragma unroll
    for (int j = 0; j < 3; ++j) {
        t[0][j] = k[0][j];
        t[1][j] = 0.5f * (k[0][j] + k[1][j] + k[2][j]);
        t[2][j] = 0.5f * (k[0][j] - k[1][j] + k[2][j]);
        t[3][j] = k[2][j];
    }
    const int b = o / 32, ol = o % 32;
    const int chunk = c / 16, h = (c >> 3) & 1, j = c & 7;
    const int nchunk = ci_pad / 16;
    const size_t lane = 32 * h + ol;
#pragma unroll
    for (int r = 0; r < 4; ++r) {
        const float uu[4] = {t[r][0], 0.5f * (t[r][0] + t[r][1] + t[r][2]), 0.5f * (t[r][0] - t[r][1] + t[r][2]),
                             t[r][2]};
#pragma unroll
        for (int s = 0; s < 4; ++s) {
            const size_t base = ((((size_t)(4 * r + s) * cobs + b) * nchunk + chunk) * 2) * 64;
            const __bf16 hi = (__bf16)uu[s];
            const __bf16 lo = (__bf16)(uu[s] - (float)hi);
            u[((base + lane) * 8) + j] = hi;
            u[((base + 64 + lane) * 8) + j] = lo;
        }
    }
}

template <int T>
struct Patch {
    int img, y0, x0;
    bool rok[4], cok[4];

    __device__ __forceinline__ Patch(const Args& a, int blk_linear, int t) {
        const int blocks_per_img = a.bx * a.by;
        img = blk_linear / blocks_per_img;
        const int blk = blk_linear % blocks_per_img;
        const int ty = (blk / a.bx) * a.tby + t / a.tbx, tx = (blk % a.bx) * a.tbx + t % a.tbx;
        const bool tile_ok = ty < a.th && tx < a.tw;
        y0 = 2 * ty - 1;
        x0 = 2 * tx - 1;
#pragma unroll
        for (int i = 0; i < 4; ++i) {
            rok[i] = tile_ok && y0 + i >= 0 && y0 + i < a.h;
            cok[i] = x0 + i >= 0 && x0 + i < a.w;
        }
    }

    __device__ __forceinline__ void load(const Args& a, const float* const* planes, int c, float (&d)[16]) const {
#if TSPLAT_W3_ABL == 1
#pragma unroll
        for (int i = 0; i < 16; ++i) d[i] = (float)(c + i + x0) * 1e-3f;
        return;
#endif
        const __attribute__((address_space(1))) float* src =
            (const __attribute__((address_space(1))) float*)planes[min(c, a.ci_pad - 1)];
#pragma unroll
        for (int i = 0; i < 4; ++i)
#pragma unroll
            for (int j = 0; j < 4; ++j) {
                const bool ok = c < a.ci && rok[i] && cok[j];
                d[4 * i + j] = ok ? src[(size_t)(y0 + i) * a.w + (x0 + j)] : 0.0f;
                if (a.relu_in) d[4 * i + j] = fmaxf(d[4 * i + j], 0.0f);
            }
    }
};

template <int T>
__device__ __forceinline__ void transform_pair(const float (&da)[16], const float (&db)[16], uint32_t* sV) {
    float ta[16], tb[16];
#pragma unroll
    for (int j = 0; j < 4; ++j) {
        ta[0 + j] = da[0 + j] - da[8 + j];
        ta[4 + j] = da[4 + j] + da[8 + j];
        ta[8 + j] = da[8 + j] - da[4 + j];
        ta[12 + j] = da[4 + j] - da[12 + j];
        tb[0 + j] = db[0 + j] - db[8 + j];
        tb[4 + j] = db[4 + j] + db[8 + j];
        tb[8 + j] = db[8 + j] - db[4 + j];
        tb[12 + j] = db[4 + j] - db[12 + j];
    }
#pragma unroll
    for (int r = 0; r < 4; ++r) {
        const float va[4] = {ta[4 * r] - ta[4 * r + 2], ta[4 * r + 1] + ta[4 * r + 2], ta[4 * r + 2] - ta[4 * r + 1],
                             ta[4 * r + 1] - ta[4 * r + 3]};
        const float vb[4] = {tb[4 * r] - tb[4 * r + 2], tb[4 * r + 1] + tb[4 * r + 2], tb[4 * r + 2] - tb[4 * r + 1],
                             tb[4 * r + 1] - tb[4 * r + 3]};
#pragma unroll
        for (int s = 0; s < 4; ++s) {
            uint32_t hi, lo;
            split_pair(va[s], vb[s], hi, lo);
            sV[(4 * r + s) * 8 * T] = hi;
            sV[(16 + 4 * r + s) * 8 * T] = lo;
        }
    }
}

template <int T>
struct Region {
    static constexpr int kPad = 8;
    static constexpr int kMaxFloats = T == 32 ? 16 * (4 * 72 + 8) : 16 * (4 * 136 + 8);
};

template <int CB, int NB, int KS, bool ST>
__global__ void __launch_bounds__(256 * CB * KS, (NB == 1 && CB * KS <= 2) ? 2 : 1) conv_kernel(Args a) {
    constexpr int T = 32 * NB;
    constexpr int GT = 256 * CB;
    constexpr int PHR = GT / (4 * T);
    constexpr int PP = PHR > 2 ? 1 : 2 / PHR;
    constexpr bool XT = PHR > 2;
    static_assert(XT || PHR * PP == 2, "pairs per chunk");
    constexpr int BUF = 2 * 16 * 8 * T;
    constexpr int CO = 32 * CB;
    constexpr int NSV = ST ? 1 : 2;
    constexpr int RGN = Region<T>::kMaxFloats;
    constexpr int NL = ((T == 32 ? 72 : 136) + GT / 16 - 1) / (GT / 16);
    constexpr int SMEM_PIPE = KS * (NSV * BUF + (ST ? 2 * RGN : 0));
    constexpr int SMEM = SMEM_PIPE > 8 * CO * T * KS ? SMEM_PIPE : 8 * CO * T * KS;
    __shared__ __attribute__((aligned(16))) uint32_t smem[SMEM];
    __shared__ const float* planes[kMaxCiPad];

    W3_STAMP(0);
    int tbk, cbk;
    {
        const int nwg = gridDim.x * gridDim.y, id = blockIdx.x + blockIdx.y * gridDim.x;
        const int q = nwg / 8, r = nwg % 8, xcd = id % 8;
        const int logical = (xcd < r ? xcd * (q + 1) : r * (q + 1) + (xcd - r) * q) + id / 8;
        tbk = logical / gridDim.y;
        cbk = logical - tbk * gridDim.y;
    }
    const int tid = threadIdx.x, lane = tid & 63, wid = tid >> 6;
    const int kg = wid / (4 * CB), wg = wid % (4 * CB);
    const int hh = wg >> 2, rr = wg & 3;
    const int gtid = tid % GT;
    const int pl = gtid & 3, t = (gtid >> 2) % T, ph0 = (gtid >> 2) / T;
    const bool xf = !XT || ph0 < 2;
    const Patch<T> pt(a, tbk, t);

    for (int c = tid; c < a.ci_pad; c += 256 * CB * KS) {
        const float* src = nullptr;
        int rem = min(c, a.ci - 1);
        for (int q = 0; q < a.nsrc && !src; ++q) {
            if (rem < a.cs[q])
                src = a.src[q] + ((size_t)pt.img * a.cs[q] + rem) * ((size_t)a.h * a.w);
            else
                rem -= a.cs[q];
        }
        planes[c] = src;
    }
    __syncthreads();

    const int cob = a.cob_base + cbk * CB + hh;
    const bool co_ok = cob < a.cobs;
    const uint4* ub = a.u + ((size_t)(4 * rr) * a.cobs + (co_ok ? cob : 0)) * a.nchunk * 128 + lane;
    const size_t xi_stride = (size_t)a.cobs * a.nchunk * 128;
    uint4 af[4][2];
    auto load_a = [&](int chunk, int s0, int s1) {
        const size_t cofs = (size_t)min(chunk, a.nchunk - 1) * 128;
#pragma unroll
        for (int s = s0; s < s1; ++s)
#pragma unroll
            for (int hl = 0; hl < 2; ++hl) {
#if TSPLAT_W3_ABL == 3
                af[s][hl] = make_uint4(chunk, s, hl, lane);
#else
                af[s][hl] = ub[s * xi_stride + cofs + hl * 64];
#endif
            }
    };

    floatx16 acc[4][NB];
#pragma unroll
    for (int s = 0; s < 4; ++s)
#pragma unroll
        for (int nb = 0; nb < NB; ++nb)
#pragma unroll
            for (int e = 0; e < 16; ++e) acc[s][nb][e] = 0.0f;

    float d[PP][2][16];
    auto load_patches = [&](int chunk) {
        if (!xf) return;
#pragma unroll
        for (int q = 0; q < PP; ++q) {
            const int c0 = chunk * 16 + 2 * (4 * (ph0 + q * PHR) + pl);
            pt.load(a, planes, c0, d[q][0]);
            pt.load(a, planes, c0 + 1, d[q][1]);
        }
    };
    uint32_t* sG = smem + kg * (NSV * BUF + (ST ? 2 * RGN : 0));
    auto transform = [&](uint32_t* sV) {
        if (!xf) return;
#pragma unroll
        for (int q = 0; q < PP; ++q) transform_pair<T>(d[q][0], d[q][1], sV + ((ph0 + q * PHR) * T + t) * 4 + pl);
    };
    const int blk = tbk % (a.bx * a.by);
    const int R = 2 * a.tby + 2, C4 = a.tbx / 2 + 2, RP = 4 * C4;
    const int ry0 = 2 * (blk / a.bx) * a.tby - 1, rx0 = 2 * (blk % a.bx) * a.tbx - 4;
    float* sIn = reinterpret_cast<float*>(sG + NSV * BUF);
    constexpr bool DS = ST && CB == 1 && NB == 1;
    float4 gr[DS ? 2 : 1][ST ? NL : 1];
    constexpr int TPC = GT / 16;
    const int gch = gtid / TPC, sub = gtid % TPC;
    int g_code[ST ? NL : 1];
#pragma unroll
    for (int k = 0; k < (ST ? NL : 0); ++k) {
        const int j = sub + TPC * k;
        const int row = j / C4, c4 = j - row * C4;
        const int y = ry0 + row, x = rx0 + 4 * c4;
        const bool ok = j < R * C4 && y >= 0 && y < a.h && x >= 0 && x < a.w;
        g_code[k] = ok ? y * a.w + x : -1;
    }
    auto gload = [&](int chunk, auto S) {
        const int c = chunk * 16 + gch;
        typedef float f4v __attribute__((ext_vector_type(4)));
        typedef const __attribute__((address_space(1))) f4v* gptr;
        const float* plane = planes[min(c, a.ci_pad - 1)];
        const bool cok = c < a.ci;
#pragma unroll
        for (int k = 0; k < (ST ? NL : 0); ++k) {
            const float* addr = cok && g_code[k] >= 0 ? plane + g_code[k] : reinterpret_cast<const float*>(&g_zero16);
            const f4v v = *(gptr)addr;
            gr[decltype(S)::value][k] = make_float4(v.x, v.y, v.z, v.w);
        }
    };
    auto sstore = [&](int slot, auto S) {
        float4* dst = reinterpret_cast<float4*>(sIn + slot * RGN) + gch * ((R * RP + Region<T>::kPad) / 4);
#pragma unroll
        for (int k = 0; k < (ST ? NL : 0); ++k) {
            const int j = sub + TPC * k;
            float4 v = gr[decltype(S)::value][k];
            if (a.relu_in) v = make_float4(fmaxf(v.x, 0.f), fmaxf(v.y, 0.f), fmaxf(v.z, 0.f), fmaxf(v.w, 0.f));
            if (j < R * C4) dst[j] = v;
        }
    };
    auto read_patches = [&](int slot) {
        if (!xf) return;
        const int tyl = t / a.tbx, txl = t - tyl * a.tbx;
        const float* base = sIn + slot * RGN + 2 * tyl * RP + 2 * txl + 3;
#pragma unroll
        for (int q = 0; q < PP; ++q)
#pragma unroll
            for (int e = 0; e < 2; ++e) {
                const float* b = base + (2 * (4 * (ph0 + q * PHR) + pl) + e) * (R * RP + Region<T>::kPad);
#pragma unroll
                for (int i = 0; i < 4; ++i)
#pragma unroll
                    for (int j = 0; j < 4; ++j) d[q][e][4 * i + j] = b[i * RP + j];
            }
    };
    auto mfma = [&](const uint32_t* sV, int s0, int s1) {
#if TSPLAT_W3_ABL == 2
        const uint32_t* bq = sV + ((lane >> 5) * T + (lane & 31)) * 4;
        for (int s = s0; s < s1; ++s) acc[s][0][0] += __builtin_bit_cast(float, bq[(4 * rr + s) * 8 * T]);
        return;
#endif
        const uint32_t* bb = sV + ((lane >> 5) * T + (lane & 31)) * 4;
#pragma unroll
        for (int s = s0; s < s1; ++s) {
            const int xi = 4 * rr + s;
            const bf16x8 ah = __builtin_bit_cast(bf16x8, af[s][0]);
            const bf16x8 al = __builtin_bit_cast(bf16x8, af[s][1]);
#pragma unroll
            for (int nb = 0; nb < NB; ++nb) {
                const uint32_t* ph = bb + xi * 8 * T + 32 * nb * 4;
                const bf16x8 bh = __builtin_bit_cast(bf16x8, *reinterpret_cast<const uint4*>(ph));
                const bf16x8 bl = __builtin_bit_cast(bf16x8, *reinterpret_cast<const uint4*>(ph + 16 * 8 * T));
                acc[s][nb] = __builtin_amdgcn_mfma_f32_32x32x16_bf16(al, bh, acc[s][nb], 0, 0, 0);
                acc[s][nb] = __builtin_amdgcn_mfma_f32_32x32x16_bf16(ah, bl, acc[s][nb], 0, 0, 0);
                acc[s][nb] = __builtin_amdgcn_mfma_f32_32x32x16_bf16(ah, bh, acc[s][nb], 0, 0, 0);
            }
        }
    };

    const int iters = (a.nchunk + KS - 1) / KS;
    const std::integral_constant<int, 0> I0;
    const std::integral_constant<int, DS ? 1 : 0> I1;
    if constexpr (ST) {
        gload(kg, I0);
        sstore(0, I0);
        gload(kg + KS, I1);
        if (DS) gload(kg + 2 * KS, I0);
        load_a(kg, 0, 4);
        __syncthreads();
        W3_STAMP(1);
        auto step = [&](int it, auto S) {
            const int ch = kg + it * KS;
            const bool more = it + 1 < iters;
            if (more) sstore((it + 1) & 1, S);
            read_patches(it & 1);
            transform(sG);
            gload(ch + (DS ? 3 : 2) * KS, S);
            __syncthreads();
            mfma(sG, 0, 4);
            load_a(ch + KS, 0, 4);
            __syncthreads();
        };
        if constexpr (DS) {
            for (int it = 0; it < iters; it += 2) {
                step(it, I1);
                if (it + 1 < iters) step(it + 1, I0);
            }
        } else {
            for (int it = 0; it < iters; ++it) step(it, I0);
        }
    } else {
    load_patches(kg);
    load_a(kg, 0, 4);
    transform(sG);
    if (iters > 1) load_patches(kg + KS);
    __syncthreads();
    for (int it = 0; it < iters; ++it) {
        const int ch = kg + it * KS;
        const uint32_t* sV = sG + (it & 1) * BUF;
        const bool more = it + 1 < iters;
        mfma(sV, 0, 2);
        if (more) load_a(ch + KS, 0, 2);
        if (more) {
            transform(sG + ((it + 1) & 1) * BUF);
            if (it + 2 < iters) load_patches(ch + 2 * KS);
        }
        mfma(sV, 2, 4);
        if (more) {
            load_a(ch + KS, 2, 4);
            __syncthreads();
        }
    }
    }
    __syncthreads();
    W3_STAMP(2);
    float* zs = reinterpret_cast<float*>(smem) + kg * (8 * CO * T);
#pragma unroll
    for (int nb = 0; nb < NB; ++nb)
#pragma unroll
        for (int e = 0; e < 16; ++e) {
            const int col = 32 * hh + (e & 3) + 8 * (e >> 2) + 4 * (lane >> 5);
            const int tt = 32 * nb + (lane & 31);
            zs[((rr * 2 + 0) * CO + col) * T + tt] = acc[0][nb][e] + acc[1][nb][e] + acc[2][nb][e];
            zs[((rr * 2 + 1) * CO + col) * T + tt] = acc[1][nb][e] - acc[2][nb][e] - acc[3][nb][e];
        }
    __syncthreads();
    const float* z0 = reinterpret_cast<const float*>(smem);
    if (KS > 1) {
        float* zw = reinterpret_cast<float*>(smem);
        for (int i = tid; i < 8 * CO * T; i += 256 * CB * KS) {
            float z = zw[i];
#pragma unroll
            for (int g2 = 1; g2 < KS; ++g2) z += zw[g2 * (8 * CO * T) + i];
            zw[i] = z;
        }
        __syncthreads();
    }
    const size_t hw = (size_t)a.h * a.w;
    for (int pidx = tid; pidx < CO * T; pidx += 256 * CB * KS) {
        const int col = pidx / T, t2 = pidx % T;
        const int o = (a.cob_base + cbk * CB) * 32 + col;
        const int oty = (blk / a.bx) * a.tby + t2 / a.tbx, otx = (blk % a.bx) * a.tbx + t2 % a.tbx;
        if (o >= a.co || oty >= a.th || otx >= a.tw) continue;
        const float bv = a.bias ? a.bias[o] : 0.0f;
        float z[4][2];
#pragma unroll
        for (int r = 0; r < 4; ++r)
#pragma unroll
            for (int j = 0; j < 2; ++j) z[r][j] = z0[((r * 2 + j) * CO + col) * T + t2];
        float* dst = a.y + ((size_t)pt.img * a.co + o) * hw;
#pragma unroll
        for (int i = 0; i < 2; ++i) {
            const int py = 2 * oty + i;
            if (py >= a.h) continue;
            const float y0v = i == 0 ? z[0][0] + z[1][0] + z[2][0] : z[1][0] - z[2][0] - z[3][0];
            const float y1v = i == 0 ? z[0][1] + z[1][1] + z[2][1] : z[1][1] - z[2][1] - z[3][1];
            float r0 = act_fn(y0v + bv, a.act), r1 = act_fn(y1v + bv, a.act);
            const int px = 2 * otx;
            float* p = dst + (size_t)py * a.w + px;
            const size_t off = ((size_t)pt.img * a.co + o) * hw + (size_t)py * a.w + px;
            if (a.res) {
                r0 += a.res[off];
                if (px + 1 < a.w) r1 += a.res[off + 1];
            }
            if (a.res2) {
                r0 += a.res2[off];
                if (px + 1 < a.w) r1 += a.res2[off + 1];
            }
            if (px + 1 < a.w && ((reinterpret_cast<uintptr_t>(p) & 7) == 0)) {
                *reinterpret_cast<float2*>(p) = make_float2(r0, r1);
            } else {
                p[0] = r0;
                if (px + 1 < a.w) p[1] = r1;
            }
        }
    }
    W3_STAMP(3);
}

__global__ void __launch_bounds__(256, 2) conv_persist_kernel(Args a, int nblocks) {
    constexpr int T = 32, GT = 256;
    constexpr int BUF = 2 * 16 * 8 * T;
    constexpr int RGN = Region<T>::kMaxFloats;
    constexpr int NL = (72 + 15) / 16;
    constexpr int CO = 32;
    __shared__ __attribute__((aligned(16))) uint32_t smem[BUF + 2 * RGN];
    __shared__ const float* planes[kPersistCiPad];
    __shared__ int cstride[kPersistCiPad];

    const int tid = threadIdx.x, lane = tid & 63, rr = tid >> 6;
    const int pl = tid & 3, t = (tid >> 2) % T, ph0 = (tid >> 2) / T;
    const size_t hw = (size_t)a.h * a.w;
    for (int c = tid; c < a.ci_pad; c += GT) {
        const float* src = nullptr;
        int rem = min(c, a.ci - 1), cs = 0;
        for (int q = 0; q < a.nsrc && !src; ++q) {
            if (rem < a.cs[q]) {
                src = a.src[q] + (size_t)rem * hw;
                cs = a.cs[q];
            } else {
                rem -= a.cs[q];
            }
        }
        planes[c] = src;
        cstride[c] = (int)(cs * hw);
    }

    const int cob = a.cob_base + blockIdx.y;
    float bias_r[CO * T / GT];
#pragma unroll
    for (int i = 0; i < CO * T / GT; ++i) {
        const int o = cob * 32 + (tid + GT * i) / T;
        bias_r[i] = a.bias && o < a.co ? a.bias[o] : 0.0f;
    }
    const uint4* ub = a.u + ((size_t)(4 * rr) * a.cobs + cob) * a.nchunk * 128 + lane;
    const size_t xi_stride = (size_t)a.cobs * a.nchunk * 128;
    uint4 af[4][2];
    auto load_a = [&](int chunk) {
#pragma unroll
        for (int s = 0; s < 4; ++s)
#pragma unroll
            for (int hl = 0; hl < 2; ++hl) af[s][hl] = ub[s * xi_stride + (size_t)chunk * 128 + hl * 64];
    };
    floatx16 acc[4];
#pragma unroll
    for (int s = 0; s < 4; ++s)
#pragma unroll
        for (int e = 0; e < 16; ++e) acc[s][e] = 0.0f;

    const int R = 2 * a.tby + 2, C4 = a.tbx / 2 + 2, RP = 4 * C4;
    const int bpi = a.bx * a.by;
    float* sIn = reinterpret_cast<float*>(smem + BUF);
    const int gch = tid >> 4, sub = tid & 15;
    int g_pos[NL];
#pragma unroll
    for (int k = 0; k < NL; ++k) {
        const int j = sub + 16 * k;
        const int row = j / C4, c4 = j - row * C4;
        g_pos[k] = j < R * C4 ? (row << 12) | c4 : -1;
    }
    float4 gr[2][NL];
    int o_jb = -1, img = 0, ry0 = 0, rx0 = 0;
    auto gload = [&](int jb, int chunk, bool valid, auto S) {
        if (jb != o_jb) {
            const int bl = blockIdx.x + jb * gridDim.x;
            img = bl / bpi;
            const int blk = bl - img * bpi;
            ry0 = 2 * (blk / a.bx) * a.tby - 1;
            rx0 = 2 * (blk % a.bx) * a.tbx - 4;
            o_jb = jb;
        }
        const int c = chunk * 16 + gch;
        const bool cok = valid && c < a.ci;
        const int cc = min(c, a.ci_pad - 1);
        const float* plane = planes[cc] + (size_t)img * cstride[cc];
        typedef float f4v __attribute__((ext_vector_type(4)));
#pragma unroll
        for (int k = 0; k < NL; ++k) {
            const int code = g_pos[k];
            const int y = ry0 + ((code >> 12) & 4095), x = rx0 + 4 * (code & 4095);
            const bool ok = cok && code >= 0 && y >= 0 && y < a.h && x >= 0 && x < a.w;
            const float* addr = ok ? plane + (size_t)y * a.w + x : reinterpret_cast<const float*>(&g_zero16);
            const f4v v = *(const __attribute__((address_space(1))) f4v*)addr;
            gr[decltype(S)::value][k] = make_float4(v.x, v.y, v.z, v.w);
        }
    };
    auto sstore = [&](int slot, auto S) {
        float4* dst = reinterpret_cast<float4*>(sIn + slot * RGN) + gch * ((R * RP + Region<T>::kPad) / 4);
#pragma unroll
        for (int k = 0; k < NL; ++k) {
            float4 v = gr[decltype(S)::value][k];
            if (a.relu_in) v = make_float4(fmaxf(v.x, 0.f), fmaxf(v.y, 0.f), fmaxf(v.z, 0.f), fmaxf(v.w, 0.f));
            if (g_pos[k] >= 0) dst[sub + 16 * k] = v;
        }
    };
    float d[2][16];
    auto read_transform = [&](int slot) {
        const int tyl = t / a.tbx, txl = t - tyl * a.tbx;
        const float* base = sIn + slot * RGN + 2 * tyl * RP + 2 * txl + 3;
#pragma unroll
        for (int e = 0; e < 2; ++e) {
            const float* b = base + (2 * (4 * ph0 + pl) + e) * (R * RP + Region<T>::kPad);
#pragma unroll
            for (int i = 0; i < 4; ++i)
#pragma unroll
                for (int j = 0; j < 4; ++j) d[e][4 * i + j] = b[i * RP + j];
        }
        transform_pair<T>(d[0], d[1], smem + (ph0 * T + t) * 4 + pl);
    };

    const int nmine = (nblocks - (int)blockIdx.x + (int)gridDim.x - 1) / (int)gridDim.x;
    const int G = nmine * a.nchunk;
    if (G <= 0) return;
    W3_STAMP(0);
    __syncthreads();
    const std::integral_constant<int, 0> I0;
    const std::integral_constant<int, 1> I1;
    gload(0, 0, true, I0);
    sstore(0, I0);
    gload(1 / a.nchunk, 1 % a.nchunk, G > 1, I1);
    gload(2 / a.nchunk, 2 % a.nchunk, G > 2, I0);
    load_a(0);
    __syncthreads();
    W3_STAMP(1);
    int j = 0, c = 0;
    int nj = 3 / a.nchunk, nc = 3 % a.nchunk;
    auto step = [&](int g, auto S) {
        if (g + 1 < G) sstore((g + 1) & 1, S);
        read_transform(g & 1);
        gload(nj, nc, g + 3 < G, S);
        if (++nc == a.nchunk) {
            nc = 0;
            ++nj;
        }
        __syncthreads();
        const uint32_t* bb = smem + ((lane >> 5) * T + (lane & 31)) * 4;
#pragma unroll
        for (int s = 0; s < 4; ++s) {
            const int xi = 4 * rr + s;
            const bf16x8 ah = __builtin_bit_cast(bf16x8, af[s][0]);
            const bf16x8 al = __builtin_bit_cast(bf16x8, af[s][1]);
            const uint32_t* ph = bb + xi * 8 * T;
            const bf16x8 bh = __builtin_bit_cast(bf16x8, *reinterpret_cast<const uint4*>(ph));
            const bf16x8 bl = __builtin_bit_cast(bf16x8, *reinterpret_cast<const uint4*>(ph + 16 * 8 * T));
            acc[s] = __builtin_amdgcn_mfma_f32_32x32x16_bf16(al, bh, acc[s], 0, 0, 0);
            acc[s] = __builtin_amdgcn_mfma_f32_32x32x16_bf16(ah, bl, acc[s], 0, 0, 0);
            acc[s] = __builtin_amdgcn_mfma_f32_32x32x16_bf16(ah, bh, acc[s], 0, 0, 0);
        }
        load_a(c + 1 < a.nchunk ? c + 1 : 0);
        __syncthreads();
        if (++c < a.nchunk) return;
        if (j == 0) W3_STAMP(2);
        float* zs = reinterpret_cast<float*>(smem);
#pragma unroll
        for (int e = 0; e < 16; ++e) {
            const int col = (e & 3) + 8 * (e >> 2) + 4 * (lane >> 5), tt = lane & 31;
            zs[((rr * 2 + 0) * CO + col) * T + tt] = acc[0][e] + acc[1][e] + acc[2][e];
            zs[((rr * 2 + 1) * CO + col) * T + tt] = acc[1][e] - acc[2][e] - acc[3][e];
#pragma unroll
            for (int s = 0; s < 4; ++s) acc[s][e] = 0.0f;
        }
        __syncthreads();
        const int bl = blockIdx.x + j * gridDim.x;
        const int img = bl / bpi, blk = bl - img * bpi;
#pragma unroll
        for (int i = 0; i < CO * T / GT; ++i) {
            const int pidx = tid + GT * i;
            const int col = pidx / T, t2 = pidx % T;
            const int o = cob * 32 + col;
            const int oty = (blk / a.bx) * a.tby + t2 / a.tbx, otx = (blk % a.bx) * a.tbx + t2 % a.tbx;
            if (o >= a.co || oty >= a.th || otx >= a.tw) continue;
            const float bv = bias_r[i];
            float z[4][2];
#pragma unroll
            for (int r = 0; r < 4; ++r)
#pragma unroll
                for (int q = 0; q < 2; ++q) z[r][q] = zs[((r * 2 + q) * CO + col) * T + t2];
#pragma unroll
            for (int i = 0; i < 2; ++i) {
                const int py = 2 * oty + i;
                if (py >= a.h) continue;
                const float y0v = i == 0 ? z[0][0] + z[1][0] + z[2][0] : z[1][0] - z[2][0] - z[3][0];
                const float y1v = i == 0 ? z[0][1] + z[1][1] + z[2][1] : z[1][1] - z[2][1] - z[3][1];
                float r0 = act_fn(y0v + bv, a.act), r1 = act_fn(y1v + bv, a.act);
                const int px = 2 * otx;
                const size_t off = ((size_t)img * a.co + o) * hw + (size_t)py * a.w + px;
                if (a.res) {
                    r0 += a.res[off];
                    if (px + 1 < a.w) r1 += a.res[off + 1];
                }
                if (a.res2) {
                    r0 += a.res2[off];
                    if (px + 1 < a.w) r1 += a.res2[off + 1];
                }
                float* p = a.y + off;
                if (px + 1 < a.w && ((reinterpret_cast<uintptr_t>(p) & 7) == 0)) {
                    *reinterpret_cast<float2*>(p) = make_float2(r0, r1);
                } else {
                    p[0] = r0;
                    if (px + 1 < a.w) p[1] = r1;
                }
            }
        }
        asm volatile("s_waitcnt lgkmcnt(0)" ::: "memory");
        __builtin_amdgcn_s_barrier();
        if (j == 0) W3_STAMP(3);
        c = 0;
        ++j;
    };
    for (int g = 0; g < G; g += 2) {
        step(g, I1);
        if (g + 1 < G) step(g + 1, I0);
    }
    W3_STAMP(4);
}

}
}

using namespace tsplat;

#if TSPLAT_W3_STAMP
extern "C" int tsplat_wino3_stamps(void* buf) {
    return hipMemcpyToSymbol(HIP_SYMBOL(wino3::g_w3_stamps), &buf, sizeof(buf)) == hipSuccess ? TSPLAT_OK
                                                                                             : TSPLAT_EINVAL;
}
#endif

static int wino3_ci_pad(int ci) { return (ci + 15) / 16 * 16; }
static int wino3_cobs(int co) { return (co + 63) / 64 * 2; }

extern "C" size_t tsplat_wino_weight_bf16x3_bytes(int32_t co, int32_t ci) {
    if (co <= 0 || ci <= 0) return 0;
    return (size_t)16 * wino3_cobs(co) * wino3_ci_pad(ci) * 32 * 2 * 2;
}

extern "C" int tsplat_wino_weight_bf16x3(const float* weight, void* packed, int32_t co, int32_t ci, void* stream_) {
    if (!weight || !packed || co <= 0 || ci <= 0) return TSPLAT_EINVAL;
    const int ci_pad = wino3_ci_pad(ci);
    const int cobs = wino3_cobs(co);
    const int total = cobs * 32 * ci_pad;
    hipLaunchKernelGGL(wino3::weight_kernel, dim3((total + 255) / 256), dim3(256), 0, (hipStream_t)stream_, weight,
                       (__bf16*)packed, co, ci, ci_pad, cobs);
    TSPLAT_CHECK_LAUNCH();
    return TSPLAT_OK;
}

static int pick_form(int n, int th, int tw, int co) {
    if (const char* e = getenv("TSPLAT_WINO3_FORM")) {
        const int f = atoi(e);
        if (f >= 1 && f <= 6) return f;
    }
    const long tiles = (long)n * th * tw;
    const int cob32 = (co + 31) / 32;
    const long wg64 = (tiles + 63) / 64 * ((co + 63) / 64);
    const long wg32 = (tiles + 31) / 32 * cob32;
    const long wg6 = (tiles + 31) / 32 * ((co + 63) / 64);
    static const bool p5 = !getenv("TSPLAT_WINO3_P5") || atoi(getenv("TSPLAT_WINO3_P5")) != 0;
    if (p5 && co <= 32 && wg32 >= 2048) return 5;
    static const bool f6 = !getenv("TSPLAT_WINO3_F6") || atoi(getenv("TSPLAT_WINO3_F6")) != 0;
    if (f6 && co % 64 == 0 && wg6 >= 150 && wg6 <= 320) return 6;
    if (co > 32 && wg64 > 128) return 4;
    return wg32 <= 256 ? 2 : 1;
}

template <int CB, int NB, int KS>
static void launch(wino3::Args a, int blocks, bool staged, hipStream_t stream, hipEvent_t start, hipEvent_t stop,
                   int coblocks = -1) {
    if (coblocks < 0) coblocks = (a.co - 32 * a.cob_base + 32 * CB - 1) / (32 * CB);
    if (staged)
        hipExtLaunchKernelGGL((wino3::conv_kernel<CB, NB, KS, true>), dim3(blocks, coblocks), dim3(256 * CB * KS), 0,
                              stream, start, stop, 0, a);
    else
        hipExtLaunchKernelGGL((wino3::conv_kernel<CB, NB, KS, false>), dim3(blocks, coblocks), dim3(256 * CB * KS),
                              0, stream, start, stop, 0, a);
}

extern "C" int tsplat_conv3x3_wino_bf16x3_ex_fwd(const float* const* srcs, const int32_t* chans, int32_t nsrc,
                                                 const void* packed, const float* bias, const float* residual,
                                                 const float* residual2, float* y, int32_t n, int32_t h, int32_t w,
                                                 int32_t co, int32_t act, int32_t relu_in, void* stream_) {
    if (!srcs || !chans || nsrc <= 0 || nsrc > wino3::kMaxSrc || !packed || !y || n <= 0 || h <= 0 || w <= 0 ||
        co <= 0 || act < 0 || act > 2)
        return TSPLAT_EINVAL;
    wino3::Args a;
    int ci = 0;
    for (int q = 0; q < wino3::kMaxSrc; ++q) {
        a.src[q] = q < nsrc ? srcs[q] : nullptr;
        a.cs[q] = q < nsrc ? chans[q] : 0;
        if (q < nsrc && (!srcs[q] || chans[q] <= 0)) return TSPLAT_EINVAL;
        ci += a.cs[q];
    }
    a.nsrc = nsrc;
    a.u = (const uint4*)packed;
    a.bias = bias;
    a.y = y;
    a.n = n;
    a.ci = ci;
    a.h = h;
    a.w = w;
    a.co = co;
    a.ci_pad = wino3_ci_pad(ci);
    if (a.ci_pad > wino3::kMaxCiPad) return TSPLAT_EINVAL;
    a.cobs = wino3_cobs(co);
    a.nchunk = a.ci_pad / 16;
    a.th = (h + 1) / 2;
    a.tw = (w + 1) / 2;
    a.act = act;
    a.relu_in = relu_in != 0;
    a.res = residual;
    a.res2 = residual2;
    a.cob_base = 0;
    int form = pick_form(n, a.th, a.tw, co);
    auto geometry = [&](int ttiles) {
        long best = -1;
        for (int tbx = ttiles; tbx >= ttiles / 8; tbx /= 2) {
            const int tby = ttiles / tbx;
            const long padded = (long)((a.tw + tbx - 1) / tbx) * tbx * ((a.th + tby - 1) / tby) * tby;
            if (best < 0 || padded < best) {
                best = padded;
                a.tbx = tbx;
            }
        }
        a.tby = ttiles / a.tbx;
        a.bx = (a.tw + a.tbx - 1) / a.tbx;
        a.by = (a.th + a.tby - 1) / a.tby;
        return (2 * a.tby + 2) * (a.tbx / 2 + 2) <= (ttiles == 32 ? 72 : 136);
    };
    if (!geometry(form == 3 || form == 4 ? 64 : 32)) return TSPLAT_EINVAL;
    const int blocks = n * a.bx * a.by;
    bool staged = w % 4 == 0;
    for (int q = 0; q < nsrc; ++q) staged = staged && (reinterpret_cast<uintptr_t>(srcs[q]) & 15) == 0;
    if (const char* e = getenv("TSPLAT_WINO3_STAGE")) staged = staged && atoi(e) != 0;
    if (form == 5 && (!staged || a.ci_pad > wino3::kPersistCiPad)) form = 1;
    hipStream_t stream = (hipStream_t)stream_;
    const prof::ExtEvents ev = prof::ext_events(prof::kWinoConv);
    if (form == 5) {
        int wgs = 512;
        if (const char* e = getenv("TSPLAT_WINO3_PWG")) wgs = std::max(1, atoi(e));
        const int cob32 = (co + 31) / 32;
        const int gx = std::max(1, std::min(blocks, (wgs + cob32 - 1) / cob32));
        hipExtLaunchKernelGGL(wino3::conv_persist_kernel, dim3(gx, cob32), dim3(256), 0, stream, ev.start, ev.stop, 0,
                              a, blocks);
        TSPLAT_CHECK_LAUNCH();
        return TSPLAT_OK;
    }
    static const bool tail = !getenv("TSPLAT_WINO3_TAIL") || atoi(getenv("TSPLAT_WINO3_TAIL")) != 0;
    if (form == 4 && tail && co > 64 && co % 64 != 0 && co % 64 <= 32) {
        launch<2, 2, 1>(a, blocks, staged, stream, ev.start, nullptr, co / 64);
        if (!geometry(32)) return TSPLAT_EINVAL;
        a.cob_base = (co / 64) * 2;
        launch<1, 1, 1>(a, n * a.bx * a.by, staged, stream, nullptr, ev.stop, 1);
        TSPLAT_CHECK_LAUNCH();
        return TSPLAT_OK;
    }
    switch (form) {
        case 4: launch<2, 2, 1>(a, blocks, staged, stream, ev.start, ev.stop); break;
        case 6: launch<2, 1, 1>(a, blocks, staged, stream, ev.start, ev.stop); break;
        case 3: launch<1, 2, 1>(a, blocks, staged, stream, ev.start, ev.stop); break;
        case 2: launch<1, 1, 2>(a, blocks, staged, stream, ev.start, ev.stop); break;
        default: launch<1, 1, 1>(a, blocks, staged, stream, ev.start, ev.stop); break;
    }
    TSPLAT_CHECK_LAUNCH();
    return TSPLAT_OK;
}

extern "C" int tsplat_conv3x3_wino_bf16x3_cat_fwd(const float* const* srcs, const int32_t* chans, int32_t nsrc,
                                                  const void* packed, const float* bias, float* y, int32_t n,
                                                  int32_t h, int32_t w, int32_t co, int32_t act, void* stream_) {
    return tsplat_conv3x3_wino_bf16x3_ex_fwd(srcs, chans, nsrc, packed, bias, nullptr, nullptr, y, n, h, w, co, act, 0,
                                             stream_);
}

extern "C" int tsplat_conv3x3_wino_bf16x3_fwd(const float* x, const void* packed, const float* bias, float* y,
                                              int32_t n, int32_t ci, int32_t h, int32_t w, int32_t co, int32_t act,
                                              void* stream_) {
    return tsplat_conv3x3_wino_bf16x3_cat_fwd(&x, &ci, 1, packed, bias, y, n, h, w, co, act, stream_);
}
```

### transplat_amd/kernels.py

```python
from __future__ import annotations

import os
import weakref

import torch

from . import _lib


def _f32(t: torch.Tensor) -> torch.Tensor:
    if t.dtype != torch.float32:
        t = t.float()
    return t.contiguous()


def small_inverse(x: torch.Tensor) -> torch.Tensor:
    if not x.is_cuda:
        return torch.linalg.inv_ex(x)[0]
    lib = _lib.load()
    d = x.shape[-1]
    xf = _f32(x)
    out = torch.empty_like(xf)
    n = xf.numel() // (d * d)
    _lib.check(lib.tsplat_small_inverse(_lib.ptr(xf), _lib.ptr(out), n, d, _lib.stream_ptr(x.device)),
# ... 920 lines not shown

_XF32 = os.environ.get("TSPLAT_XF32", "0") == "1"


class dense_precision:

    def __init__(self, mode: str):
        if mode not in _DENSE_MODES:
            raise ValueError(f"dense precision {mode!r} not in {_DENSE_MODES}")
        self.mode, self.prev, self.prev_tf32 = mode, None, None

    def __enter__(self):
        global _DENSE
        self.prev, _DENSE = _DENSE, self.mode
        self.prev_tf32 = torch.backends.cuda.matmul.allow_tf32
        torch.backends.cuda.matmul.allow_tf32 = _XF32 and self.mode == "bf16x3"
        return self

    def __exit__(self, *exc):
        global _DENSE
        _DENSE = self.prev
        torch.backends.cuda.matmul.allow_tf32 = self.prev_tf32
        return False


def split_mode() -> bool:
    return _DENSE == "bf16x3"


_ATTN = "fp32"
ATTN_MODES = ("fp32", "bf16x3", "bf16")


def auto_attention(dense_dtype: str) -> str:
    if dense_dtype == "bf16":
        return "bf16"
    return "bf16x3" if dense_dtype == "bf16x3" and _ATTN_X3 else "fp32"


class attention_precision:

    def __init__(self, mode: str):
        if mode not in ATTN_MODES:
            raise ValueError(f"attention precision {mode!r}")
        self.mode, self.prev = mode, None

    def __enter__(self):
        global _ATTN
        self.prev, _ATTN = _ATTN, self.mode
        return self

    def __exit__(self, *exc):
        global _ATTN
        _ATTN = self.prev
        return False


_SPLIT_W: dict = {}


def split_bf16x3(x: torch.Tensor, weight_order: bool = False) -> torch.Tensor:
    lib = _lib.load()
    xf = _f32(x)
    k = xf.shape[-1]
    out = torch.empty((*xf.shape[:-1], 3 * k), dtype=torch.bfloat16, device=xf.device)
    _lib.check(lib.tsplat_split_bf16x3(_lib.ptr(xf), _lib.ptr(out), xf.numel() // k, k, int(weight_order),
                                       _lib.stream_ptr(xf.device)), "tsplat_split_bf16x3")
    return out


def _split_weight(weight):
    hit = _SPLIT_W.get(id(weight))
    if hit is not None and hit[0]() is weight and hit[1] == weight._version:
        return hit[2]
    packed = split_bf16x3(weight.detach(), weight_order=True)
    if len(_SPLIT_W) > 512:
        for k in [k for k, v in _SPLIT_W.items() if v[0]() is None]:
            del _SPLIT_W[k]
    _SPLIT_W[id(weight)] = (weakref.ref(weight), weight._version, packed)
    return packed


def linear_bf16x3(x, weight, bias=None, act: str = "none", cache: bool = True):
    k, n = x.shape[-1], weight.shape[0]
    w3 = _split_weight(weight) if cache else split_bf16x3(weight, weight_order=True)
    x3 = split_bf16x3(x).reshape(-1, 3 * k)
    with torch.autocast("cuda", enabled=False):
        if bias is not None:
            y = torch.addmm(_f32(bias), x3, w3.t(), out_dtype=torch.float32)
        else:
            y = torch.mm(x3, w3.t(), out_dtype=torch.float32)
    y = y.reshape(*x.shape[:-1], n)
    if act == "gelu":
        y = torch.nn.functional.gelu(y)
    return y


_LINX = os.environ.get("TSPLAT_LINX", "0") == "1"
_LINX_SIDE = os.environ.get("TSPLAT_LINX_SIDE", "1") == "1"


def linear_xf32_ok(x, weight) -> bool:
    if not (_LINX and _DENSE == "bf16x3" and x.is_cuda and x.dtype == torch.float32
            and weight.dtype == torch.float32 and not torch.is_autocast_enabled("cuda")):
        return False
    n, k = weight.shape
    m = x.numel() // max(k, 1)
    if not _LINX_SIDE:
        from . import streams

        if streams._is_side(torch.cuda.current_stream(x.device)):
            return False
    return n % 4 == 0 and ((n >= 1024 and m >= 512) or (m >= 4096 and n >= 512))


def linear_xf32(x, weight, bias=None, act: str = "none"):
    prev = torch.backends.cuda.matmul.allow_tf32
    torch.backends.cuda.matmul.allow_tf32 = True
    try:
        y = torch.matmul(x, weight.t())
    finally:
        torch.backends.cuda.matmul.allow_tf32 = prev
    if bias is None and act == "none":
        return y
    y = y.contiguous()
    bb = _f32(bias) if bias is not None else None
    lib = _lib.load()
    rc = lib.tsplat_bias_act_nhwc_fwd(_lib.ptr(y), _lib.ptr(bb), None, None, _lib.ptr(y), y.numel() // y.shape[-1],
                                      y.shape[-1], _ACTS[act], _lib.stream_ptr(y.device))
    _lib.check(rc, "tsplat_bias_act_nhwc_fwd")
    return y


_GEMM_X3 = os.environ.get("TSPLAT_GEMM_X3", "1") == "1"
_GEMM_KSPLIT = int(os.environ.get("TSPLAT_GEMM_KSPLIT", "0"))
_GEMM_W: dict = {}
GEMM_LOG = None


def gemm_x3_ok(x, weight) -> bool:
    if not (_GEMM_X3 and _DENSE == "bf16x3" and x.is_cuda and x.dtype == torch.float32
            and weight.dtype == torch.float32 and not torch.is_autocast_enabled("cuda")):
        return False
    n, k = weight.shape
    return k % 4 == 0 and n % 4 == 0 and x.shape[-1] == k


def _gemm_pack(weight):
    hit = _GEMM_W.get(id(weight))
    if hit is not None and hit[0]() is weight and hit[1] == weight._version:
        return hit[2]
    lib = _lib.load()
    n, k = weight.shape
    wf = _f32(weight.detach())
    wp = torch.empty(int(lib.tsplat_gemm_x3_pack_bytes(n, k)), dtype=torch.uint8, device=weight.device)
    _lib.check(lib.tsplat_gemm_x3_pack(_lib.ptr(wf), _lib.ptr(wp), n, k, _lib.stream_ptr(weight.device)),
               "tsplat_gemm_x3_pack")
    if len(_GEMM_W) > 512:
        for key in [key for key, v in _GEMM_W.items() if v[0]() is None]:
            del _GEMM_W[key]
    _GEMM_W[id(weight)] = (weakref.ref(weight), weight._version, wp)
    return wp


def gemm_ksplit(m: int, n: int, k: int) -> int:
    if _GEMM_KSPLIT > 0:
        return _GEMM_KSPLIT
    tiles = -(-m // 64) * -(-n // 128)
    nchunk = -(-k // 64)
    s = max(1, min(nchunk // 2, 256 // tiles))
    while s > 1 and (s - 1) * -(-nchunk // s) >= nchunk:
        s -= 1
    return s


def gemm_x3(x, weight, bias=None, act: str = "none", ksplit: int = 1):
    lib = _lib.load()
    n, k = weight.shape
    xf = _f32(x)
    m = xf.numel() // k
    if ksplit == 0:
        ksplit = 1 if act != "none" else gemm_ksplit(m, n, k)
    if act == "split":
        if ksplit != 1:
            raise ValueError("gemm_x3: the split output needs ksplit 1")
        out = torch.empty((2, *x.shape[:-1], n), dtype=torch.bfloat16, device=x.device)
    else:
        shape = (*x.shape[:-1], n) if ksplit == 1 else (ksplit, *x.shape[:-1], n)
        out = torch.empty(shape, dtype=torch.float32, device=x.device)
    if GEMM_LOG is not None:
        GEMM_LOG.append((m, n, k, ksplit))
    rc = lib.tsplat_gemm_x3_fwd(_lib.ptr(xf), _lib.ptr(_gemm_pack(weight)), _lib.ptr(_f32(bias)) if bias is not None else None,
                                _lib.ptr(out), m, n, k, ksplit, {"none": 0, "gelu": 1, "split": 2}[act],
                                _lib.stream_ptr(x.device))
    _lib.check(rc, "tsplat_gemm_x3_fwd", "bf16x3")
    return out


def linear_forward(mod, x):
    import torch.nn.functional as F

    if linear_xf32_ok(x, mod.weight):
        return linear_xf32(x, mod.weight, mod.bias)
    if gemm_x3_ok(x, mod.weight) and x.numel() // x.shape[-1] >= 64:
        return gemm_x3(x, mod.weight, mod.bias)
    return F.linear(x, mod.weight, mod.bias)


def install_linear_dispatch(module) -> int:
    import functools

    n = 0
    for m in module.modules():
        if type(m) is torch.nn.Linear:
            m.forward = functools.partial(linear_forward, m)
            n += 1
    return n


WINO_FLOP_LOG = None


_WINO3_PACKED: dict = {}


def wino_pack_weight_bf16x3(weight):
    hit = _WINO3_PACKED.get(id(weight))
    if hit is not None and hit[0]() is weight and hit[1] == weight._version:
        return hit[2]
    lib = _lib.load()
    co, ci = weight.shape[:2]
    packed = torch.empty(int(lib.tsplat_wino_weight_bf16x3_bytes(co, ci)), dtype=torch.uint8, device=weight.device)
    w = weight.detach().float().contiguous()
    _lib.check(lib.tsplat_wino_weight_bf16x3(_lib.ptr(w), _lib.ptr(packed), co, ci, _lib.stream_ptr(weight.device)),
               "tsplat_wino_weight_bf16x3")
    if len(_WINO3_PACKED) > 512:
        for k in [k for k, v in _WINO3_PACKED.items() if v[0]() is None]:
            del _WINO3_PACKED[k]
    _WINO3_PACKED[id(weight)] = (weakref.ref(weight), weight._version, packed)
    return packed


_FEW = os.environ.get("TSPLAT_CONV_FEW", "1") != "0"
FEW_MIN_PX = int(os.environ.get("TSPLAT_CONV_FEW_MIN_PX", str(2 * 256 * 256)))
FEW_MAX_CI = int(os.environ.get("TSPLAT_CONV_FEW_MAX_CI", "64"))
FEW_MAX_CO = int(os.environ.get("TSPLAT_CONV_FEW_MAX_CO", "32"))


def _few_ok(srcs, n: int, h: int, w: int, co: int) -> bool:
    ci = sum(t.shape[1] for t in srcs)
    return (_FEW and co <= FEW_MAX_CO and ci <= FEW_MAX_CI and n * h * w >= FEW_MIN_PX and w % 4 == 0
            and all(t.data_ptr() % 16 == 0 for t in srcs)
            and int(_lib.load().tsplat_conv3x3_few_form(n, ci, h, w, co)) != 0)


def conv3x3_wino(x, weight, bias=None, act: str = "none", extra=(), precision: str | None = None, residual=None,
                 residual2=None, relu_in: bool = False):
    import ctypes

    lib = _lib.load()
    precision = precision or _DENSE
    if precision != "bf16x3" and (relu_in or residual is not None or residual2 is not None):
        y = conv3x3_wino(torch.relu(x) if relu_in else x, weight, bias, act,
                         tuple(torch.relu(t) for t in extra) if relu_in else extra, precision)
        for r in (residual, residual2):
            if r is not None:
                y = y + r
        return y
    srcs = [_f32(t) for t in (x, *extra)]
    n, _, h, w = srcs[0].shape
    co = weight.shape[0]
    if WINO_FLOP_LOG is not None:
        ci = sum(t.shape[1] for t in srcs)
        WINO_FLOP_LOG.append((2.0 * 16 * ci * co * n * ((h + 1) // 2) * ((w + 1) // 2), 2.0 * n * h * w * co * ci * 9))
    y = torch.empty((n, co, h, w), dtype=torch.float32, device=x.device)
    pb = _f32(bias) if bias is not None else None
    ptrs = (ctypes.c_void_p * len(srcs))(*[_lib.ptr(t) for t in srcs])
    chans = (ctypes.c_int32 * len(srcs))(*[t.shape[1] for t in srcs])
    if precision == "bf16x3":
        res = [_f32(r) if r is not None else None for r in (residual, residual2)]
        for r in res:
            if r is not None and tuple(r.shape) != tuple(y.shape):
                raise ValueError(f"residual {tuple(r.shape)} != output {tuple(y.shape)}")
        if _few_ok(srcs, n, h, w, co):
            rc = lib.tsplat_conv3x3_few_bf16x3_fwd(
                ctypes.cast(ptrs, ctypes.c_void_p), ctypes.cast(chans, ctypes.c_void_p), len(srcs),
                _lib.ptr(conv_pack_weight_x3(weight)), _lib.ptr(pb), _lib.ptr(res[0]), _lib.ptr(res[1]),
                _lib.ptr(y), n, h, w, co, _WINO_ACT[act], int(relu_in), _lib.stream_ptr(x.device))
            _lib.check(rc, "tsplat_conv3x3_few_bf16x3_fwd")
            return y
        rc = lib.tsplat_conv3x3_wino_bf16x3_ex_fwd(
            ctypes.cast(ptrs, ctypes.c_void_p), ctypes.cast(chans, ctypes.c_void_p), len(srcs),
            _lib.ptr(wino_pack_weight_bf16x3(weight)), _lib.ptr(pb), _lib.ptr(res[0]), _lib.ptr(res[1]), _lib.ptr(y),
            n, h, w, co, _WINO_ACT[act], int(relu_in), _lib.stream_ptr(x.device))
        _lib.check(rc, "tsplat_conv3x3_wino_bf16x3_ex_fwd")
        return y
    rc = lib.tsplat_conv3x3_wino_cat_f32_fwd(ctypes.cast(ptrs, ctypes.c_void_p), ctypes.cast(chans, ctypes.c_void_p),
                                             len(srcs), _lib.ptr(wino_pack_weight(weight)), _lib.ptr(pb),
                                             _lib.ptr(y), n, h, w, co, _WINO_ACT[act], _lib.stream_ptr(x.device))
    _lib.check(rc, "tsplat_conv3x3_wino_cat_f32_fwd")
    return y


_CONV_BF16 = os.environ.get("TSPLAT_CONV_BF16", "1") != "0"
_BF16_PACKED: dict = {}


def conv_bf16_pack_weight(weight):
    hit = _BF16_PACKED.get(id(weight))
    if hit is not None and hit[0]() is weight and hit[1] == weight._version:
        return hit[2]
    co, ci = weight.shape[:2]
    taps = weight[0, 0].numel()
    cob, nk = (co + 31) // 32, (ci + 15) // 16
    w = torch.zeros((cob * 32, nk * 16, taps), dtype=torch.bfloat16, device=weight.device)
    w[:co, :ci] = weight.detach().reshape(co, ci, taps).to(torch.bfloat16)
    packed = w.view(cob, 32, nk, 2, 8, taps).permute(0, 2, 5, 3, 1, 4).contiguous()
    if len(_BF16_PACKED) > 512:
        for k in [k for k, v in _BF16_PACKED.items() if v[0]() is None]:
            del _BF16_PACKED[k]
    _BF16_PACKED[id(weight)] = (weakref.ref(weight), weight._version, packed)
    return packed


def _bf16_rounded_bias(bias):
    key = ("bias", id(bias))
    hit = _BF16_PACKED.get(key)
    if hit is not None and hit[0]() is bias and hit[1] == bias._version:
        return hit[2]
    rb = bias.detach().to(torch.bfloat16).float().contiguous()
    _BF16_PACKED[key] = (weakref.ref(bias), bias._version, rb)
    return rb


def conv_bf16_ok(x, weight, stride=1, padding=None, dilation=1, groups=1, extra=(), upsample: bool = False) -> bool:
    if (not _CONV_BF16 or not x.is_cuda or not torch.is_autocast_enabled("cuda")
            or torch.get_autocast_dtype("cuda") != torch.bfloat16 or len(extra) > 3):
        return False
    for t in (x, *extra):
        if (t.dtype not in (torch.float32, torch.bfloat16) or t.dim() != 4 or not t.is_contiguous()
                or t.device != x.device or t.shape[0] != x.shape[0] or t.shape[2:] != x.shape[2:]
                or t.numel() >= 2 ** 31):
            return False
    if not ((weight.dim() == 4 and weight.shape[2] == weight.shape[3] and weight.shape[2] in (1, 3))
            or (weight.dim() == 3 and weight.shape[2] == 1)) or groups != 1:
        return False
    k = weight.shape[2]
    as_int = lambda v: v if isinstance(v, int) else (v[0] if len(set(v)) == 1 else -1)
    if as_int(stride) != 1 or as_int(padding if padding is not None else k // 2) != k // 2 or as_int(dilation) != 1:
        return False
    n, _, h, w = x.shape
    if upsample:
        h, w = 2 * h, 2 * w
    ci = sum(t.shape[1] for t in (x, *extra))
    return weight.shape[1] == ci and w % 8 == 0 and n * max(weight.shape[0], ci) * h * w < 2 ** 31


def conv_bf16(x, weight, bias=None, act: str = "none", extra=(), upsample: bool = False):
    import ctypes

    if not x.is_cuda:
        raise RuntimeError("transplat HIP ops need device tensors (no CPU path)")
    lib = _lib.load()
    srcs = (x, *extra)
    n, _, h, w = x.shape
    if upsample:
        h, w = 2 * h, 2 * w
    co, k = weight.shape[0], weight.shape[2]
    y = torch.empty((n, co, h, w), dtype=torch.bfloat16, device=x.device)
    pb = _bf16_rounded_bias(bias) if bias is not None else None
    ptrs = (ctypes.c_void_p * len(srcs))(*[_lib.ptr(t) for t in srcs])
    chans = (ctypes.c_int32 * len(srcs))(*[t.shape[1] for t in srcs])
    f32 = (ctypes.c_int32 * len(srcs))(*[int(t.dtype == torch.float32) for t in srcs])
    rc = lib.tsplat_conv2d_bf16_fwd(ctypes.cast(ptrs, ctypes.c_void_p), ctypes.cast(chans, ctypes.c_void_p),
                                    len(srcs), ctypes.cast(f32, ctypes.c_void_p),
                                    _lib.ptr(conv_bf16_pack_weight(weight)), _lib.ptr(pb), _lib.ptr(y), n, h, w,
                                    co, k, int(upsample), _ACTS[act], _lib.stream_ptr(x.device))
    _lib.check(rc, "tsplat_conv2d_bf16_fwd")
    return y


def conv2d_nhwc_ok(x, weight) -> bool:
    if x.dim() != 4 or not x.is_contiguous(memory_format=torch.channels_last) or x.shape[1] == 1:
        return False
    return conv2d_direct_ok(x, weight, 1, weight.shape[-1] // 2)


def conv2d_nhwc(x, weight, bias=None, residual=None, relu_in: bool = False):
    lib = _lib.load()
    n, c, h, w = x.shape
    co, ci, k, _ = weight.shape
    if ci != c or not x.is_contiguous(memory_format=torch.channels_last) or x.dtype != torch.float32:
        raise ValueError("conv2d_nhwc needs a channels-last fp32 input matching the weight")
    y = torch.empty((n, co, h, w), dtype=torch.float32, device=x.device, memory_format=torch.channels_last)
    res = None
    if residual is not None:
        res = residual.float().contiguous(memory_format=torch.channels_last)
        if res.shape != y.shape:
            raise ValueError(f"residual {tuple(res.shape)} != output {tuple(y.shape)}")
    tiles = ((n * h * w + 31) // 32) * ((co + 31) // 32)
    ksplit = 16
    while ksplit > 1 and (tiles * ksplit > 4096 or c // 2 < (2 if k == 3 else 16) * ksplit):
        ksplit //= 2
    pb = _f32(bias) if bias is not None else None
    rc = lib.tsplat_conv2d_f32_nhwc_fwd(_lib.ptr(x), c, _lib.ptr(conv_pack_weight(weight)), _lib.ptr(pb),
                                        _lib.ptr(res), _lib.ptr(y), n, h, w, co, k, int(relu_in), ksplit,
                                        _lib.stream_ptr(x.device))
    _lib.check(rc, "tsplat_conv2d_f32_nhwc_fwd")
    return y


def upsample_bilinear_act(x, scale: int, bias=None, act: str = "none"):
    lib = _lib.load()
    n, c, h, w = x.shape
    xf = _f32(x)
    y = torch.empty((n, c, h * scale, w * scale), dtype=torch.float32, device=x.device)
    rc = lib.tsplat_upsample_bilinear_act_fwd(_lib.ptr(xf), _lib.ptr(_f32(bias) if bias is not None else None),
                                              _lib.ptr(y), n, c, h, w, int(scale), _ACTS[act],
                                              _lib.stream_ptr(x.device))
    _lib.check(rc, "tsplat_upsample_bilinear_act_fwd")
    return y


def qkv_attention_cf(qkv, heads: int, views: int = 1):
    lib = _lib.load()
    vb, width, t = qkv.shape
    ch = width // (3 * heads)
    if vb % views or ch * 3 * heads != width:
        raise ValueError(f"qkv {tuple(qkv.shape)} does not split into {views} views x {heads} heads")
    x = _f32(qkv)
    out = torch.empty((vb, heads * ch, t), dtype=torch.float32, device=qkv.device)
    rc = lib.tsplat_qkv_attention_cf_fwd(_lib.ptr(x), _lib.ptr(out), vb // views, heads, views, t, ch,
                                         float(ch ** -0.5), _lib.stream_ptr(qkv.device))
    _lib.check(rc, "tsplat_qkv_attention_cf_fwd")
    return out


def conv_nhwc_epilogue(conv, x, act: str = "none", res1=None, res2=None):
    import torch.nn.functional as F

    y = F.conv2d(x, conv.weight, None, conv.stride, conv.padding, conv.dilation, conv.groups)
    cl = torch.channels_last
    if not y.is_contiguous(memory_format=cl):
        y = y.contiguous(memory_format=cl)
    rs = [r.contiguous(memory_format=cl) if r is not None else None for r in (res1, res2)]
    for r in rs:
        if r is not None and (r.shape != y.shape or r.dtype != torch.float32):
            raise ValueError(f"residual {tuple(r.shape)} does not match the output {tuple(y.shape)}")
    lib = _lib.load()
    rc = lib.tsplat_bias_act_nhwc_fwd(_lib.ptr(y), _lib.ptr(conv.bias), _lib.ptr(rs[0]), _lib.ptr(rs[1]),
                                      _lib.ptr(y), y.numel() // y.shape[1], y.shape[1], _ACTS[act],
                                      _lib.stream_ptr(y.device))
    _lib.check(rc, "tsplat_bias_act_nhwc_fwd")
    return y


def resize_bilinear_nhwc(x, size):
    n, c, h, w = x.shape
    ho, wo = int(size[0]), int(size[1])
    if x.dtype != torch.float32 or not x.is_contiguous(memory_format=torch.channels_last) or c % 4:
        raise ValueError("resize_bilinear_nhwc needs a channels-last fp32 map with C % 4 == 0")
    y = torch.empty((n, c, ho, wo), dtype=torch.float32, device=x.device, memory_format=torch.channels_last)
    lib = _lib.load()
    rc = lib.tsplat_resize_bilinear_nhwc_fwd(_lib.ptr(x), _lib.ptr(y), n, h, w, c, ho, wo, _lib.stream_ptr(x.device))
    _lib.check(rc, "tsplat_resize_bilinear_nhwc_fwd")
    return y


def interpolate_bilinear_ac(x, size):
    import torch.nn.functional as F

    size = (int(size[0]), int(size[1]))
    if not (x.is_cuda and x.dtype == torch.float32 and x.dim() == 4 and x.is_contiguous()):
        return F.interpolate(x, size, mode="bilinear", align_corners=True)
    n, c, h, w = x.shape
    y = torch.empty((n, c, size[0], size[1]), dtype=torch.float32, device=x.device)
    lib = _lib.load()
    rc = lib.tsplat_resize_bilinear_nchw_fwd(_lib.ptr(x), _lib.ptr(y), n * c, h, w, size[0], size[1],
                                             _lib.stream_ptr(x.device))
    _lib.check(rc, "tsplat_resize_bilinear_nchw_fwd")
    return y


def sh_rotation(rotations, d_sh: int):
    from .misc.sh_rotation import x_basis_packed

    lib = _lib.load()
    rot = _f32(rotations.reshape(-1, 3, 3))
    n = rot.shape[0]
    out = torch.empty((n, d_sh, d_sh), device=rot.device)
    rc = lib.tsplat_sh_rotation_fwd(_lib.ptr(rot), _lib.ptr(x_basis_packed(rot.device)), _lib.ptr(out), n, d_sh,
                                    _lib.stream_ptr(rot.device))
    _lib.check(rc, "tsplat_sh_rotation_fwd")
    return out


def adapter_camera_consts(extrinsics, intrinsics, image_shape, d_sh: int):
    return (adapter_cameras(extrinsics, intrinsics, image_shape),
            sh_rotation(extrinsics.reshape(-1, 4, 4)[:, :3, :3], d_sh))


def gaussian_adapter(raw, depths, densities, extrinsics, intrinsics, image_shape, scale_min: float,
                     scale_max: float, opacity_exponent: float = 1.0, gaussians_per_pixel: int = 1,
                     camera_consts=None):
    lib = _lib.load()
    b, v, hw, r = raw.shape
    d_sh = (r - 9) // 3
    h, w = image_shape
    nchw = raw.dtype == torch.float32 and all(
        n == 1 or st == want for n, st, want in zip(raw.shape, raw.stride(), (r * hw, b * r * hw, 1, hw)))
    if not nchw:
        raw = _f32(raw)
    depths, densities = _f32(depths), _f32(densities)
    cams, shrot = camera_consts if camera_consts is not None else adapter_camera_consts(extrinsics, intrinsics,
                                                                                       image_shape, d_sh)
    dev = raw.device
    g = v * hw
    means = torch.empty((b, g, 3), device=dev)
    cov = torch.empty((b, g, 3, 3), device=dev)
    harm = torch.empty((b, g, 3, d_sh), device=dev)
    opac = torch.empty((b, g), device=dev)
    rc = lib.tsplat_gaussian_adapter_fwd(
        _lib.ptr(raw), _lib.ptr(depths), _lib.ptr(densities), _lib.ptr(cams), _lib.ptr(shrot), _lib.ptr(means),
        _lib.ptr(cov), _lib.ptr(harm), _lib.ptr(opac), b, v, h, w, r, d_sh, float(scale_min), float(scale_max),
        float(opacity_exponent), int(gaussians_per_pixel), int(nchw), _lib.stream_ptr(dev))
    _lib.check(rc, "tsplat_gaussian_adapter_fwd")
    return means, cov, harm, opac
```

### transplat_amd/model/encoder/matching/ldm_unet.py

```python
from __future__ import annotations

import math
import os

import torch
import torch.nn.functional as F
from einops import rearrange
from torch import nn

from .... import kernels

_ACT_OF = {nn.SiLU: "silu", nn.GELU: "gelu"}
_GEMM_1X1 = os.environ.get("TSPLAT_UNET_GEMM1X1", "1") != "0"


def gn_act(norm: nn.GroupNorm, x, act: str = "none", residual=None, pre_bias=None):
    y = kernels.group_norm(x, norm.num_groups, norm.weight, norm.bias, norm.eps, act, residual, pre_bias)
    return y.type(x.dtype)


_CAT_FREE = os.environ.get("TSPLAT_UNET_CAT_FREE", "1") == "1"


def _direct(conv: nn.Module, x, x2=None, upsample: bool = False) -> bool:
    if not (isinstance(conv, nn.Conv2d) and conv.dilation == (1, 1) and conv.groups == 1
            and conv.stride[0] == conv.stride[1]):
        return False
    c2 = x2.shape[1] if x2 is not None else 0
    return kernels.conv2d_direct_ok(x, conv.weight, conv.stride[0], conv.padding, c2=c2, upsample=upsample)


def conv(conv: nn.Module, x, x2=None, upsample: bool = False, bias: bool = True):
    b = conv.bias if bias else None
    extra = (x2,) if x2 is not None else ()
    if (isinstance(conv, nn.Conv2d) and conv.padding_mode == "zeros"
            and kernels.conv_bf16_ok(x, conv.weight, conv.stride, conv.padding, conv.dilation, conv.groups, extra,
                                     upsample)):
        return kernels.conv_bf16(x, conv.weight, b, extra=extra, upsample=upsample)
    if (isinstance(conv, nn.Conv1d) and x2 is None and not upsample and conv.kernel_size == (1,)
            and conv.stride == (1,) and conv.groups == 1 and x.dim() == 3
            and kernels.conv_bf16_ok(x.unsqueeze(2), conv.weight)):
        return kernels.conv_bf16(x.unsqueeze(2), conv.weight, b).squeeze(2)
    if _direct(conv, x, x2, upsample):
        return kernels.conv2d_direct(x, conv.weight, b, conv.stride[0], x2=x2, upsample=upsample)
    if (isinstance(conv, nn.Conv1d) and x2 is None and not upsample and conv.kernel_size == (1,)
            and conv.stride == (1,) and conv.groups == 1 and x.dim() == 3
            and kernels.conv2d_direct_ok(x.unsqueeze(-1), conv.weight)):
        return kernels.conv2d_direct(x.unsqueeze(-1), conv.weight, b).squeeze(-1)
    if (isinstance(conv, nn.Conv2d) and not upsample
            and kernels.conv3x3_wino_ok(x, conv.weight, conv.stride, conv.padding, conv.dilation, conv.groups, extra)):
        return kernels.conv3x3_wino(x, conv.weight, b, extra=extra)
    if x2 is not None:
        x = torch.cat([x, x2], dim=1)
    if upsample:
        x = F.interpolate(x, scale_factor=2, mode="nearest")
    if isinstance(conv, nn.Conv2d) and kernels.conv3x3_wino_ok(x, conv.weight, conv.stride, conv.padding,
                                                               conv.dilation, conv.groups):
        return kernels.conv3x3_wino(x, conv.weight, b)
    if (_GEMM_1X1 and isinstance(conv, nn.Conv2d) and conv.kernel_size == (1, 1) and conv.stride == (1, 1)
            and conv.groups == 1
            and conv.padding == (0, 0) and x.is_cuda and x.dtype == torch.float32 and conv.weight.dtype == torch.float32
            and not torch.is_autocast_enabled("cuda")):
        n, ci, h, w = x.shape
        co = conv.weight.shape[0]
        wm = conv.weight.view(co, ci).expand(n, co, ci)
        xm = x.contiguous().view(n, ci, h * w)
        y = torch.baddbmm(b.view(1, co, 1), wm, xm) if b is not None else torch.bmm(wm, xm)
        return y.view(n, co, h, w)
    if isinstance(conv, nn.Conv2d):
        return kernels.conv2d_fallback(x, conv.weight, b, conv.stride, conv.padding, conv.dilation, conv.groups)
    return F.conv1d(x, conv.weight, b, conv.stride, conv.padding, conv.dilation, conv.groups)


def conv_nobias(conv_mod: nn.Module, x, x2=None):
    return conv(conv_mod, x, x2, bias=False)


def conv_gn_act(conv_mod: nn.Module, norm: nn.GroupNorm, x, act: str = "none", residual=None, x2=None):
    if conv_mod.bias is None:
        return gn_act(norm, conv(conv_mod, x, x2), act, residual)
    return gn_act(norm, conv_nobias(conv_mod, x, x2), act, residual, pre_bias=conv_mod.bias)


def run_sequential(seq: nn.Sequential, x):
    mods = list(seq)
    i = 0
    while i < len(mods):
        m = mods[i]
        if isinstance(m, (nn.Conv1d, nn.Conv2d)) and i + 1 < len(mods) and isinstance(mods[i + 1], nn.GroupNorm):
            nxt = mods[i + 2] if i + 2 < len(mods) else None
            act = _ACT_OF.get(type(nxt)) if nxt is not None else None
            if isinstance(nxt, nn.GELU) and nxt.approximate != "none":
                act = None
            x = conv_gn_act(m, mods[i + 1], x, act or "none")
            i += 3 if act else 2
            continue
        if isinstance(m, nn.GroupNorm):
            nxt = mods[i + 1] if i + 1 < len(mods) else None
            act = _ACT_OF.get(type(nxt)) if nxt is not None else None
            if isinstance(nxt, nn.GELU) and nxt.approximate != "none":
                act = None
            x = gn_act(m, x, act or "none")
            i += 2 if act else 1
            continue
        x = m(x)
        i += 1
    return x


class GroupNorm32(nn.GroupNorm):
    def forward(self, x):
        return gn_act(self, x)


def normalization(channels):
    return GroupNorm32(8 if channels % 8 == 0 else 4, channels)


class ResBlock(nn.Module):

    def __init__(self, channels, out_channels=None, kernel_size=3):
        super().__init__()
        self.channels = channels
        self.out_channels = out_channels or channels
        pad = (kernel_size - 1) // 2
        self.in_layers = nn.Sequential(
            nn.Conv2d(channels, self.out_channels, kernel_size, padding=pad), normalization(self.out_channels),
            nn.SiLU())
        self.out_layers = nn.Sequential(
            nn.Conv2d(self.out_channels, self.out_channels, kernel_size, padding=pad),
            normalization(self.out_channels), nn.SiLU())
        self.skip_connection = (nn.Identity() if self.out_channels == channels
                                else nn.Conv2d(channels, self.out_channels, 1))

    def _concat_free(self, x, x2) -> bool:
        c, sk = self.in_layers[0], self.skip_connection
        if not (_CAT_FREE and kernels.split_mode() and isinstance(c, nn.Conv2d)
                and kernels.conv3x3_wino_ok(x, c.weight, c.stride, c.padding, c.dilation, c.groups, (x2,))):
            return False
        return isinstance(sk, nn.Identity) or (
            isinstance(sk, nn.Conv2d) and sk.kernel_size == (1, 1) and sk.stride == (1, 1) and sk.groups == 1
            and kernels.conv2d_direct_ok(x, sk.weight, 1, sk.padding, c2=x2.shape[1], force=True))

    def forward(self, x, x2=None):
        cat_free = False
        if x2 is not None and not _direct(self.in_layers[0], x, x2):
            cat_free = self._concat_free(x, x2)
            if not cat_free:
                x, x2 = torch.cat([x, x2], dim=1), None
        h = conv_gn_act(self.in_layers[0], self.in_layers[1], x, "silu", x2=x2)
        if isinstance(self.skip_connection, nn.Identity):
            skip = x if x2 is None else (x, x2)
        elif cat_free and not _direct(self.skip_connection, x, x2):
            sk = self.skip_connection
            skip = kernels.conv2d_direct(x, sk.weight, sk.bias, 1, x2=x2)
        else:
            skip = conv(self.skip_connection, x, x2)
        return conv_gn_act(self.out_layers[0], self.out_layers[1], h, "silu", residual=skip)


class QKVAttentionLegacy(nn.Module):

    def __init__(self, n_heads, n_frames=2, use_cross_view_self_attn=False):
        super().__init__()
        self.n_heads = n_heads
        self.n_frames = n_frames
        self.use_cross_view_self_attn = use_cross_view_self_attn

    def forward(self, qkv):
        width = qkv.shape[1]
        if qkv.is_cuda and width // (3 * self.n_heads) == 32 and (
                qkv.dtype == torch.float32 or torch.is_autocast_enabled("cuda")):
            return kernels.qkv_attention_cf(qkv.float(), self.n_heads,
                                            self.n_frames if self.use_cross_view_self_attn else 1)
        if self.use_cross_view_self_attn:
            qkv = rearrange(qkv, "(v b) n t -> b n (v t)", v=self.n_frames)
        bs, width, length = qkv.shape
        ch = width // (3 * self.n_heads)
        q, k, v = qkv.reshape(bs * self.n_heads, ch * 3, length).split(ch, dim=1)
        scale = 1 / math.sqrt(math.sqrt(ch))
        weight = torch.einsum("bct,bcs->bts", q * scale, k * scale)
        weight = torch.softmax(weight.float(), dim=-1).type(weight.dtype)
        a = torch.einsum("bts,bcs->bct", weight, v).reshape(bs, -1, length)
        if self.use_cross_view_self_attn:
            a = rearrange(a, "b n (v t) -> (v b) n t", v=self.n_frames)
        return a


class AttentionBlock(nn.Module):

    def __init__(self, channels, num_head_channels=32, num_frames=2, use_cross_view_self_attn=False):
        super().__init__()
        self.channels = channels
        self.num_heads = channels // num_head_channels
        self.qkv = nn.Conv1d(channels, channels * 3, 1)
        self.attention = QKVAttentionLegacy(self.num_heads, n_frames=num_frames,
                                            use_cross_view_self_attn=use_cross_view_self_attn)
        self.proj_out = nn.Conv1d(channels, channels, 1)
        self.norm = normalization(channels)

    def forward(self, x):
        b, c, *spatial = x.shape
        x = x.reshape(b, c, -1)
        h = self.attention(conv(self.qkv, x))
        return conv_gn_act(self.proj_out, self.norm, h, residual=x).reshape(b, c, *spatial)


class Downsample(nn.Module):
    def __init__(self, channels, out_channels=None):
        super().__init__()
        self.channels = channels
        self.op = nn.Conv2d(channels, out_channels or channels, 3, stride=2, padding=1)

    def forward(self, x):
        return conv(self.op, x)


class Upsample(nn.Module):
    def __init__(self, channels, out_channels=None):
        super().__init__()
        self.channels = channels
        self.conv = nn.Conv2d(channels, out_channels or channels, 3, padding=1)

    def forward(self, x):
        return conv(self.conv, x, upsample=True)


class UNetModel(nn.Module):
    def __init__(self, image_size, in_channels, model_channels, out_channels, num_res_blocks, attention_resolutions,
                 dropout=0, channel_mult=(1, 2, 4, 8), conv_resample=True, dims=2, postnorm=False,
                 num_head_channels=-1, num_frames=2, use_cross_view_self_attn=False, **kwargs):
        super().__init__()
        if dims != 2 or not postnorm or not conv_resample or num_head_channels <= 0:
            raise NotImplementedError("only the DepthPredictorTrans configuration is built")
        self.in_channels = in_channels
        self.model_channels = model_channels
        self.out_channels = out_channels
        attn = lambda ch: AttentionBlock(ch, num_head_channels=num_head_channels, num_frames=num_frames,
                                         use_cross_view_self_attn=use_cross_view_self_attn)
        self.input_blocks = nn.ModuleList([nn.Sequential(nn.Conv2d(in_channels, model_channels, 3, padding=1))])
        input_block_chans = [model_channels]
        ch = model_channels
        ds = 1
        for level, mult in enumerate(channel_mult):
            for _ in range(num_res_blocks):
                layers = [ResBlock(ch, out_channels=mult * model_channels)]
                ch = mult * model_channels
                if ds in attention_resolutions:
                    layers.append(attn(ch))
                self.input_blocks.append(nn.Sequential(*layers))
                input_block_chans.append(ch)
            if level != len(channel_mult) - 1:
                self.input_blocks.append(nn.Sequential(Downsample(ch, out_channels=ch)))
                input_block_chans.append(ch)
                ds *= 2
        self.middle_block = nn.Sequential(ResBlock(ch), nn.Identity(), ResBlock(ch))
        self.output_blocks = nn.ModuleList([])
        for level, mult in list(enumerate(channel_mult))[::-1]:
            for i in range(num_res_blocks + 1):
                ich = input_block_chans.pop()
                layers = [ResBlock(ch + ich, out_channels=model_channels * mult)]
                ch = model_channels * mult
                if ds in attention_resolutions:
                    layers.append(attn(ch))
                if level and i == num_res_blocks:
                    layers.append(Upsample(ch, out_channels=ch))
                    ds //= 2
                self.output_blocks.append(nn.Sequential(*layers))
        self.out = nn.Sequential(nn.Conv2d(model_channels, out_channels, 3, padding=1), normalization(out_channels),
                                 nn.SiLU())

    def forward(self, x, timesteps=None, context=None, y=None, **kwargs):
        hs = []
        h = x
        for module in self.input_blocks:
            h = module(h)
            hs.append(h)
        h = self.middle_block(h)
        for module in self.output_blocks:
            mods = list(module)
            h = mods[0](h, hs.pop())
            for m in mods[1:]:
                h = m(h)
        return run_sequential(self.out, h)
```

### transplat_amd/routes.py

```python
from __future__ import annotations

from collections import Counter
from contextlib import contextmanager

import torch
from torch.utils._python_dispatch import TorchDispatchMode

from . import _lib

_HIP = {
    "tsplat_win_attn_x3_partials_fwd": ("window attention", "bf16x3 (split-bf16 products, fp32 softmax)"),
    "tsplat_win_attn_x3_fwd": ("window attention", "bf16x3 (split-bf16 products, fp32 softmax)"),
    "tsplat_win_attn_bf16_shift_fwd": ("window attention", "bf16 MFMA, fp32 softmax"),
    "tsplat_win_attn_bf16_fwd": ("window attention", "bf16 MFMA, fp32 softmax"),
    "tsplat_win_attn_partials_fwd": ("window attention", "exact fp32"),
    "tsplat_win_attn_fwd": ("window attention", "exact fp32"),
    "tsplat_conv3x3_wino_bf16x3_fwd": ("3x3 convs (HIP Winograd)", "bf16x3"),
    "tsplat_conv3x3_wino_bf16x3_ex_fwd": ("3x3 convs (HIP Winograd)", "bf16x3"),
    "tsplat_conv3x3_wino_bf16x3_cat_fwd": ("3x3 convs (HIP Winograd)", "bf16x3"),
    "tsplat_conv3x3_wino_f32_fwd": ("3x3 convs (HIP Winograd)", "exact fp32"),
    "tsplat_conv3x3_wino_cat_f32_fwd": ("3x3 convs (HIP Winograd)", "exact fp32"),
    "tsplat_conv3x3_few_bf16x3_fwd": ("direct convs (HIP)", "bf16x3"),
    "tsplat_conv2d_bf16x3_fwd": ("direct convs (HIP)", "bf16x3"),
    "tsplat_conv2d_f32_fwd": ("direct convs (HIP)", "exact fp32"),
    "tsplat_conv2d_f32_zsplit_fwd": ("direct convs (HIP)", "exact fp32"),
    "tsplat_conv2d_f32_nhwc_fwd": ("direct convs (HIP)", "exact fp32"),
    "tsplat_conv2d_bf16_fwd": ("direct convs (HIP)", "bf16"),
    "tsplat_linear_f32_fwd": ("transformer linears (HIP)", None),
    "tsplat_linear_f32_split_x3_fwd": ("transformer linears (HIP)", None),
    "tsplat_linear_f32_attn_merge_fwd": ("transformer linears (HIP)", None),
    "tsplat_gemm_x3_fwd": ("GEMMs (HIP)", "bf16x3"),
    "tsplat_mha_x3_fwd": ("DINOv2 attention (HIP)", "bf16x3"),
    "tsplat_mha_x3_presplit_fwd": ("DINOv2 attention (HIP)", "bf16x3"),
    "tsplat_mha_f32_fwd": ("DINOv2 attention (HIP)", "exact fp32"),
    "tsplat_mha_bias_f32_fwd": ("DINOv2 attention (HIP)", "exact fp32"),
    "tsplat_qkv_attention_cf_fwd": ("U-Net attention (HIP)", "exact fp32"),
    "tsplat_uv_coarse_fwd": ("correlation (HIP)", "fp32"),
    "tsplat_uv_cross_table_fwd": ("correlation (HIP)", "fp32"),
    "tsplat_uv_cross_fwd": ("correlation (HIP)", "fp32"),
    "tsplat_msda_fwd": ("correlation (HIP)", "fp32"),
    "tsplat_msda_raw_fwd": ("correlation (HIP)", "fp32"),
    "tsplat_ms_deform_attn_fwd": ("correlation (HIP)", "fp32"),
    "tsplat_group_norm_fwd": ("norms (HIP)", "fp32"),
    "tsplat_group_norm_cat_res_fwd": ("norms (HIP)", "fp32"),
    "tsplat_group_norm_bf16_fwd": ("norms (HIP)", "bf16 I/O, fp32 statistics"),
    "tsplat_layer_norm128_fwd": ("norms (HIP)", None),
    "tsplat_residual_ln_fwd": ("norms (HIP)", "fp32"),
    "tsplat_residual_ln_slabs_fwd": ("norms (HIP)", "fp32"),
    "tsplat_residual_ln_bf16_fwd": ("norms (HIP)", "bf16 I/O, fp32 statistics"),
    "tsplat_gaussian_adapter_fwd": ("gaussian adapter (HIP)", "fp32"),
    "tsplat_sh_rotation_fwd": ("gaussian adapter (HIP)", "fp32"),
    "tsplat_raster_fwd": ("rasterizer (HIP)", "fp32"),
}
_ORDER = ("window attention", "transformer linears (HIP)", "GEMMs (HIP)", "3x3 convs (HIP Winograd)", "direct convs (HIP)",
          "DINOv2 attention (HIP)", "U-Net attention (HIP)", "library GEMMs (hipBLASLt)", "library convs (MIOpen)",
          "correlation (HIP)", "norms (HIP)", "gaussian adapter (HIP)", "rasterizer (HIP)")
_GEMMS = {"mm", "addmm", "bmm", "baddbmm", "addbmm", "_scaled_mm"}
_CONVS = {"convolution", "_convolution", "cudnn_convolution", "miopen_convolution", "convolution_overrideable",
          "conv2d", "conv_transpose2d", "miopen_convolution_transpose"}


class Routes:
    def __init__(self):
        self.calls: Counter = Counter()
        self.library: list = []

    def note(self, what: str, route: str | None = None) -> None:
        cat = _HIP.get(what)
        if cat is None:
            return
        self.calls[(cat[0], route or cat[1] or "?")] += 1

    def lib(self, op: str, arith: str, shapes) -> None:
        cat = "library GEMMs (hipBLASLt)" if op in _GEMMS else "library convs (MIOpen)"
        self.calls[(cat, arith)] += 1
        self.library.append((op, arith, shapes))

    def by_category(self) -> dict:
        out: dict = {}
        for (cat, arith), n in self.calls.items():
            out.setdefault(cat, Counter())[arith] += n
        return out

    def label(self) -> str:
        cats = self.by_category()
        parts = []
        for cat in _ORDER:
            if cat == "library convs (MIOpen)" and cat not in cats:
                parts.append("library convs (MIOpen): none")
                continue
            if cat not in cats:
                continue
            items = ", ".join(f"{a} x{n}" for a, n in sorted(cats[cat].items(), key=lambda kv: -kv[1]))
            parts.append(f"{cat}: {items}")
        return "; ".join(parts)


class _LibraryOps(TorchDispatchMode):
    def __init__(self, routes: Routes):
        super().__init__()
        self.routes = routes

    def __torch_dispatch__(self, func, types, args=(), kwargs=None):
        kwargs = kwargs or {}
        name = func.overloadpacket.__name__
        if name in _GEMMS or name in _CONVS:
            ts = [a for a in args if torch.is_tensor(a)]
            if ts and ts[0].is_cuda:
                dt = ts[-1].dtype if name in _GEMMS else ts[0].dtype
                if name in _GEMMS and dt == torch.float32:
                    arith = "xf32 (emulated, bf16 MFMA)" if torch.backends.cuda.matmul.allow_tf32 else "exact fp32"
                elif name in _GEMMS and dt == torch.bfloat16:
                    from . import kernels

                    arith = ("bf16x3 (split-bf16 K = 3k)" if kernels.split_mode()
                             and not torch.is_autocast_enabled("cuda") else "bf16")
                else:
                    arith = {torch.float32: "fp32", torch.bfloat16: "bf16", torch.float16: "fp16"}.get(dt, str(dt))
                shapes = [tuple(t.shape) for t in ts]
                if name in _CONVS and len(args) >= 7:
                    shapes.append((tuple(args[3]), tuple(args[4]), bool(args[6])))
                self.routes.lib(name, arith, shapes)
        return func(*args, **kwargs)


@contextmanager
def record():
    routes = Routes()
    prev = _lib.ROUTE_HOOK
    _lib.ROUTE_HOOK = routes.note
    try:
        with _LibraryOps(routes):
            yield routes
    finally:
        _lib.ROUTE_HOOK = prev
```

Before: 492.2 views/s.

## Fuse GroupNorm statistics into 3x3 conv epilogues and apply from partials

The Winograd and few-channel 3x3 conv kernels gain a stats variant. Its epilogue computes per-tile, per-group count, mean and centered sum of squares and writes them to a partials buffer. A new group_norm_apply kernel merges these partials and normalizes, so the separate full-tensor statistics pass over the conv output is no longer needed. The fused path is on by default in the U-Net conv+GN blocks for large groups. In exchange the conv epilogue does extra LDS reduction work and uses more registers.

New measurement: 494.4 views/s, median of 4. No clear change (+0.5%).

```diff
diff --git a/include/transplat_hip.h b/include/transplat_hip.h
--- a/include/transplat_hip.h
+++ b/include/transplat_hip.h
@@ -94,6 +94,10 @@
                                   const float* residual, const float* residual2, int32_t c1, float* y,
                                   void* workspace, int32_t n, int32_t c, int64_t hw, int32_t groups, float eps,
                                   int32_t act, void* stream);
+int tsplat_group_norm_apply_fwd(const float* x, const float* partials, int32_t slots, const float* gamma,
+                                const float* beta, const float* residual, const float* residual2, int32_t c1,
+                                float* y, int32_t n, int32_t c, int64_t hw, int32_t groups, float eps, int32_t act,
+                                void* stream);
 int tsplat_group_norm_bf16_fwd(const void* x, const float* pre_bias, const float* gamma, const float* beta,
                                const void* residual, void* y, void* workspace, int32_t n, int32_t c, int64_t hw,
                                int32_t groups, float eps, int32_t act, void* stream);
@@ -210,12 +214,24 @@
                                       const void* w_packed, const float* bias, const float* residual,
                                       const float* residual2, float* y, int32_t batch, int32_t height, int32_t width,
                                       int32_t c_out, int32_t act, int32_t relu_in, void* stream);
+int32_t tsplat_conv3x3_wino_gn_slots(int32_t batch, int32_t height, int32_t width, int32_t c_out, int32_t groups,
+                                     int32_t form);
+int tsplat_conv3x3_wino_bf16x3_gn_fwd(const float* const* srcs, const int32_t* chans, int32_t n_src,
+                                      const void* w_packed, const float* bias, float* y, float* partials,
+                                      int32_t batch, int32_t height, int32_t width, int32_t c_out, int32_t groups,
+                                      int32_t relu_in, int32_t form, void* stream);
 
 int32_t tsplat_conv3x3_few_form(int32_t batch, int32_t c_in, int32_t height, int32_t width, int32_t c_out);
 int tsplat_conv3x3_few_bf16x3_fwd(const float* const* srcs, const int32_t* chans, int32_t n_src,
                                   const void* w_packed, const float* bias, const float* residual,
                                   const float* residual2, float* y, int32_t batch, int32_t height, int32_t width,
                                   int32_t c_out, int32_t act, int32_t relu_in, void* stream);
+int32_t tsplat_conv3x3_few_gn_slots(int32_t batch, int32_t c_in, int32_t height, int32_t width, int32_t c_out,
+                                    int32_t groups, int32_t form);
+int tsplat_conv3x3_few_bf16x3_gn_fwd(const float* const* srcs, const int32_t* chans, int32_t n_src,
+                                     const void* w_packed, const float* bias, float* y, float* partials,
+                                     int32_t batch, int32_t height, int32_t width, int32_t c_out, int32_t groups,
+                                     int32_t relu_in, int32_t form, void* stream);
 
 int tsplat_split_bf16x3(const float* x, void* out, int64_t rows, int32_t k, int32_t weight_order, void* stream);
 
diff --git a/transplat_amd/_lib.py b/transplat_amd/_lib.py
--- a/transplat_amd/_lib.py
+++ b/transplat_amd/_lib.py
@@ -104,6 +104,12 @@
     "tsplat_conv3x3_wino_bf16x3_ex_fwd": (ctypes.c_int, [_P, _P, _I32, _P, _P, _P, _P, _P] + [_I32] * 6 + [_P]),
     "tsplat_conv3x3_few_form": (ctypes.c_int32, [_I32] * 5),
     "tsplat_conv3x3_few_bf16x3_fwd": (ctypes.c_int, [_P, _P, _I32, _P, _P, _P, _P, _P] + [_I32] * 6 + [_P]),
+    "tsplat_conv3x3_wino_gn_slots": (ctypes.c_int32, [_I32] * 6),
+    "tsplat_conv3x3_wino_bf16x3_gn_fwd": (ctypes.c_int, [_P, _P, _I32, _P, _P, _P, _P] + [_I32] * 7 + [_P]),
+    "tsplat_conv3x3_few_gn_slots": (ctypes.c_int32, [_I32] * 7),
+    "tsplat_conv3x3_few_bf16x3_gn_fwd": (ctypes.c_int, [_P, _P, _I32, _P, _P, _P, _P] + [_I32] * 7 + [_P]),
+    "tsplat_group_norm_apply_fwd": (ctypes.c_int, [_P, _P, _I32, _P, _P, _P, _P, _I32, _P, _I32, _I32, ctypes.c_int64,
+                                                   _I32, ctypes.c_float, _I32, _P]),
     "tsplat_split_bf16x3": (ctypes.c_int, [_P, _P, ctypes.c_int64, _I32, _I32, _P]),
     "tsplat_conv2d_bf16_weight_bytes": (ctypes.c_size_t, [_I32, _I32, _I32]),
     "tsplat_conv2d_bf16_fwd": (ctypes.c_int, [_P, _P, _I32, _P, _P, _P, _P] + [_I32] * 7 + [_P]),
diff --git a/transplat_amd/csrc/convfew.hip b/transplat_amd/csrc/convfew.hip
--- a/transplat_amd/csrc/convfew.hip
+++ b/transplat_amd/csrc/convfew.hip
@@ -2,6 +2,10 @@
 
 #include "common.h"
 #include "prof.h"
+
+#ifndef TSPLAT_FEW_ABL
+#define TSPLAT_FEW_ABL 0
+#endif
 
 namespace tsplat {
 namespace convfew {
@@ -30,6 +34,8 @@
     int relu_in;
     int rb, cb;
     int abl;
+    float* gnp;
+    int cpg;
 };
 
 __device__ __forceinline__ float act_fn(float v, int act) {
@@ -53,7 +59,7 @@
     return p;
 }
 
-template <int TR, int CB>
+template <int TR, int CB, bool ST = false>
 __global__ void __launch_bounds__(256, 2) conv_kernel(Args a) {
     constexpr int R = TR + 2;
     constexpr int WPC = 4 / CB;
@@ -64,6 +70,7 @@
     __shared__ const float* sPlane[kMaxCi];
 
     const int tid = threadIdx.x, lane = tid & 63, wid = tid >> 6;
+    const int abl = a.abl;
     const int blk = blockIdx.x;
     const int img = blk / (a.rb * a.cb), rem = blk - img * (a.rb * a.cb);
     const int y0 = (rem / a.cb) * TR, x0 = (rem % a.cb) * kCols;
@@ -92,7 +99,7 @@
             const size_t po = (size_t)min(max(y, 0), a.h - 1) * a.w + min(max(x, 0), a.w - 4);
 #pragma unroll
             for (int j = 0; j < 8; ++j) {
-                const bool ok = in && c0 + j < a.ci && !(a.abl & 1);
+                const bool ok = in && c0 + j < a.ci && !(abl & 1);
                 const float* p = sPlane[min(c0 + j, kMaxCi - 1)] + po;
                 typedef float f4v __attribute__((ext_vector_type(4)));
                 const f4v f = *(const __attribute__((address_space(1))) f4v*)p;
@@ -138,7 +145,7 @@
             }
         }
         __syncthreads();
-        if (a.abl & 2) continue;
+        if (abl & 2) continue;
 #pragma unroll
         for (int ks = 0; ks < 18; ++ks) {
             const int tap = ks >> 1, gl = ks & 1;
@@ -160,13 +167,15 @@
     }
 
     const size_t hw = (size_t)a.h * a.w;
-    if (a.abl & 4) {
+    if (abl & 4) {
         if (acc[0][0] == 12345.0f) a.y[0] = acc[UPW - 1][15];
         return;
     }
     constexpr int CO = 32 * CB;
     static_assert(CO * TR * kCols * 4 <= 2 * HL * 2, "output tile fits the input image's LDS");
     float* sOut = reinterpret_cast<float*>(sIn);
+    float bias_l = 0.0f;
+    if constexpr (ST) bias_l = a.bias && lane < CO && 32 * cob0 + lane < a.co ? a.bias[32 * cob0 + lane] : 0.0f;
     __syncthreads();
 #pragma unroll
     for (int u = 0; u < UPW; ++u) {
@@ -180,6 +189,7 @@
     }
     __syncthreads();
     constexpr int V4 = CO * TR * (kCols / 4);
+    if constexpr (ST) asm volatile("" : "+v"(bias_l));
 #pragma unroll 4
     for (int idx = tid; idx < V4; idx += 256) {
         const int c4 = idx % (kCols / 4), t2 = idx / (kCols / 4);
@@ -191,15 +201,50 @@
         const float bb = a.bias ? a.bias[o] : 0.0f;
         v = make_float4(act_fn(v.x + bb, a.act), act_fn(v.y + bb, a.act), act_fn(v.z + bb, a.act),
                         act_fn(v.w + bb, a.act));
-        if (a.res) {
+        if (!ST && a.res) {
             const float4 r = *reinterpret_cast<const float4*>(a.res + off);
             v = make_float4(v.x + r.x, v.y + r.y, v.z + r.z, v.w + r.w);
         }
-        if (a.res2) {
+        if (!ST && a.res2) {
             const float4 r = *reinterpret_cast<const float4*>(a.res2 + off);
             v = make_float4(v.x + r.x, v.y + r.y, v.z + r.z, v.w + r.w);
         }
         *reinterpret_cast<float4*>(a.y + off) = v;
+    }
+    if constexpr (ST) {
+        const int gs4 = a.cpg * TR * (kCols / 4);
+        const int vr = min(TR, a.h - y0), vc = min(kCols, a.w - x0);
+        const float cnt = (float)(a.cpg * vr * vc);
+        for (int gl = wid; gl < CO / a.cpg; gl += 4) {
+            const int o0 = 32 * cob0 + gl * a.cpg;
+            if (o0 >= a.co) break;
+            float mean = 0.0f, red = 0.0f;
+#pragma unroll
+            for (int pass = 0; pass < 2; ++pass) {
+                float s = 0.0f;
+                for (int it = lane; it < gs4; it += 64) {
+                    const int idx = gl * gs4 + it;
+                    const int c4 = idx % (kCols / 4), t2 = idx / (kCols / 4);
+                    const int i = t2 % TR, col = t2 / TR;
+                    const float bb = __shfl(bias_l, col);
+                    const float4 t = *reinterpret_cast<const float4*>(&sOut[(col * TR + i) * kCols + 4 * c4]);
+                    if (i < vr && 4 * c4 < vc) {
+                        const float v0 = t.x + bb - mean, v1 = t.y + bb - mean, v2 = t.z + bb - mean, v3 = t.w + bb - mean;
+                        s += pass == 0 ? (v0 + v1) + (v2 + v3) : (v0 * v0 + v1 * v1) + (v2 * v2 + v3 * v3);
+                    }
+                }
+#pragma unroll
+                for (int off = kWave / 2; off > 0; off >>= 1) s += __shfl_xor(s, off);
+                if (pass == 0) mean = s / cnt;
+                red = s;
+            }
+            if (lane == 0) {
+                float* p = a.gnp + (((size_t)img * (a.co / a.cpg) + o0 / a.cpg) * (a.rb * a.cb) + rem) * 3;
+                p[0] = cnt;
+                p[1] = mean;
+                p[2] = red;
+            }
+        }
     }
 }
 
@@ -212,19 +257,38 @@
     if (n <= 0 || ci <= 0 || h <= 0 || w <= 0 || co <= 0 || w % 4 || co > 64 || ci > convfew::kMaxCi) return 0;
     const long cbk = (w + convfew::kCols - 1) / convfew::kCols;
     if (co > 32) return 22;
-    if (const char* e = getenv("TSPLAT_FEW_TR")) {
-        const int tr = atoi(e);
-        if (tr == 4 || tr == 2) return tr * 10 + 1;
-    }
+    static const int knob_tr = getenv("TSPLAT_FEW_TR") ? atoi(getenv("TSPLAT_FEW_TR")) : 0;
+    if (knob_tr == 4 || knob_tr == 2) return knob_tr * 10 + 1;
     return (long)n * ((h + 3) / 4) * cbk >= 256 ? 41 : 21;
 }
 
-extern "C" int tsplat_conv3x3_few_bf16x3_fwd(const float* const* srcs, const int32_t* chans, int32_t nsrc,
-                                             const void* packed, const float* bias, const float* residual,
-                                             const float* residual2, float* y, int32_t n, int32_t h, int32_t w,
-                                             int32_t co, int32_t act, int32_t relu_in, void* stream_) {
+static int few_gn_form(int n, int ci, int h, int w, int co, int groups, int form) {
+    const int own = tsplat_conv3x3_few_form(n, ci, h, w, co);
+    if (!own || groups <= 0 || co % groups) return 0;
+    if (form == 0) form = own;
+    if (!(form == 22 || ((form == 41 || form == 21) && co <= 32))) return 0;
+    const int cpg = co / groups, tr = form / 10, cob = 32 * (form % 10);
+    if (cob % cpg || (cpg * tr) % 4) return 0;
+    return form;
+}
+
+extern "C" int32_t tsplat_conv3x3_few_gn_slots(int32_t n, int32_t ci, int32_t h, int32_t w, int32_t co,
+                                               int32_t groups, int32_t form) {
+    form = few_gn_form(n, ci, h, w, co, groups, form);
+    if (!form) return 0;
+    const int tr = form / 10;
+    return ((h + tr - 1) / tr) * ((w + convfew::kCols - 1) / convfew::kCols);
+}
+
+static int few_launch(const float* const* srcs, const int32_t* chans, int32_t nsrc, const void* packed,
+                      const float* bias, const float* residual, const float* residual2, float* y, float* partials,
+                      int32_t groups, int32_t form, int32_t n, int32_t h, int32_t w, int32_t co, int32_t act,
+                      int32_t relu_in, void* stream_) {
     using namespace tsplat::convfew;
     if (!srcs || !chans || nsrc <= 0 || nsrc > kMaxSrc || !packed || !y || act < 0 || act > 2) return TSPLAT_EINVAL;
+    if ((reinterpret_cast<uintptr_t>(y) & 15) || (reinterpret_cast<uintptr_t>(residual) & 15) ||
+        (reinterpret_cast<uintptr_t>(residual2) & 15))
+        return TSPLAT_EINVAL;
     Args a;
     int ci = 0;
     for (int q = 0; q < kMaxSrc; ++q) {
@@ -234,7 +298,7 @@
             return TSPLAT_EINVAL;
         ci += a.cs[q];
     }
-    const int form = tsplat_conv3x3_few_form(n, ci, h, w, co);
+    form = partials ? few_gn_form(n, ci, h, w, co, groups, form) : tsplat_conv3x3_few_form(n, ci, h, w, co);
     if (!form) return TSPLAT_EINVAL;
     a.nsrc = nsrc;
     a.wp = (const uint4*)packed;
@@ -251,21 +315,52 @@
     a.cot = (co + 31) / 32;
     a.act = act;
     a.relu_in = relu_in != 0;
-    a.abl = getenv("TSPLAT_FEW_ABL") ? atoi(getenv("TSPLAT_FEW_ABL")) : 0;
+    a.abl = 0;
+#if TSPLAT_FEW_ABL
+    static const int knob_abl = getenv("TSPLAT_FEW_ABL") ? atoi(getenv("TSPLAT_FEW_ABL")) : 0;
+    a.abl = knob_abl;
+#endif
+    a.gnp = partials;
+    a.cpg = partials ? co / groups : 0;
     const int tr = form / 10, cb = form % 10;
     a.rb = (h + tr - 1) / tr;
     a.cb = (w + kCols - 1) / kCols;
     const dim3 grid(n * a.rb * a.cb, (a.cot + cb - 1) / cb);
     hipStream_t stream = (hipStream_t)stream_;
     const prof::ExtEvents ev = prof::ext_events(prof::kWinoConv);
-#define TSPLAT_FEW(TR, CB)                                                                                 \
-    hipExtLaunchKernelGGL((convfew::conv_kernel<TR, CB>), grid, dim3(256), 0, stream, ev.start, ev.stop, 0, a)
-    switch (form) {
-        case 41: TSPLAT_FEW(4, 1); break;
-        case 21: TSPLAT_FEW(2, 1); break;
-        default: TSPLAT_FEW(2, 2); break;
+#define TSPLAT_FEW(TR, CB, ST)                                                                                 \
+    hipExtLaunchKernelGGL((convfew::conv_kernel<TR, CB, ST>), grid, dim3(256), 0, stream, ev.start, ev.stop, 0, a)
+    if (partials) {
+        switch (form) {
+            case 41: TSPLAT_FEW(4, 1, true); break;
+            case 21: TSPLAT_FEW(2, 1, true); break;
+            default: TSPLAT_FEW(2, 2, true); break;
+        }
+    } else {
+        switch (form) {
+            case 41: TSPLAT_FEW(4, 1, false); break;
+            case 21: TSPLAT_FEW(2, 1, false); break;
+            default: TSPLAT_FEW(2, 2, false); break;
+        }
     }
 #undef TSPLAT_FEW
     TSPLAT_CHECK_LAUNCH();
     return TSPLAT_OK;
 }
+
+extern "C" int tsplat_conv3x3_few_bf16x3_fwd(const float* const* srcs, const int32_t* chans, int32_t nsrc,
+                                             const void* packed, const float* bias, const float* residual,
+                                             const float* residual2, float* y, int32_t n, int32_t h, int32_t w,
+                                             int32_t co, int32_t act, int32_t relu_in, void* stream_) {
+    return few_launch(srcs, chans, nsrc, packed, bias, residual, residual2, y, nullptr, 0, 0, n, h, w, co, act,
+                      relu_in, stream_);
+}
+
+extern "C" int tsplat_conv3x3_few_bf16x3_gn_fwd(const float* const* srcs, const int32_t* chans, int32_t nsrc,
+                                                const void* packed, const float* bias, float* y, float* partials,
+                                                int32_t n, int32_t h, int32_t w, int32_t co, int32_t groups,
+                                                int32_t relu_in, int32_t form, void* stream_) {
+    if (!partials || (reinterpret_cast<uintptr_t>(partials) & 3)) return TSPLAT_EINVAL;
+    return few_launch(srcs, chans, nsrc, packed, bias, nullptr, nullptr, y, partials, groups, form, n, h, w, co, 0,
+                      relu_in, stream_);
+}
diff --git a/transplat_amd/csrc/groupnorm.hip b/transplat_amd/csrc/groupnorm.hip
--- a/transplat_amd/csrc/groupnorm.hip
+++ b/transplat_amd/csrc/groupnorm.hip
@@ -110,12 +110,19 @@
 }
 
 template <bool VEC, int ACT, bool RES, typename T>
+__device__ __forceinline__ void apply_chunk(const T* __restrict__ x, const float* __restrict__ pb,
+                                            const float* __restrict__ gamma, const float* __restrict__ beta,
+                                            const T* __restrict__ res, const T* __restrict__ res2, int c1,
+                                            T* __restrict__ y, int64_t L, int HW, int C, int cpg, int G, float mean,
+                                            float rstd);
+
+template <bool VEC, int ACT, bool RES, typename T>
 __global__ void __launch_bounds__(kThreads)
 apply_kernel(const T* __restrict__ x, const float* __restrict__ pb, const float2* __restrict__ partials,
              const float* __restrict__ gamma, const float* __restrict__ beta,
              const T* __restrict__ res, const T* __restrict__ res2, int c1, T* __restrict__ y, int64_t L, int S,
              int HW, int C, int cpg, int G, float eps) {
-    const int chunk = blockIdx.x, seg = blockIdx.y, tid = threadIdx.x;
+    const int seg = blockIdx.y, tid = threadIdx.x;
     __shared__ float s_scale_shift[2];
     if (tid < kWave) {
         Welford w{0.f, 0.f, 0.f};
@@ -131,7 +138,42 @@
         }
     }
     __syncthreads();
-    const float mean = s_scale_shift[0], rstd = s_scale_shift[1];
+    apply_chunk<VEC, ACT, RES, T>(x, pb, gamma, beta, res, res2, c1, y, L, HW, C, cpg, G, s_scale_shift[0],
+                                  s_scale_shift[1]);
+}
+
+template <bool VEC, int ACT, bool RES, typename T>
+__global__ void __launch_bounds__(kThreads)
+apply_slots_kernel(const T* __restrict__ x, const float* __restrict__ partials, int slots,
+                   const float* __restrict__ gamma, const float* __restrict__ beta, const T* __restrict__ res,
+                   const T* __restrict__ res2, int c1, T* __restrict__ y, int64_t L, int HW, int C, int cpg, int G,
+                   float eps) {
+    const int seg = blockIdx.y, tid = threadIdx.x;
+    __shared__ float s_scale_shift[2];
+    if (tid < kWave) {
+        Welford w{0.f, 0.f, 0.f};
+        for (int i = tid; i < slots; i += kWave) {
+            const float* p = partials + ((int64_t)seg * slots + i) * 3;
+            w = combine(w, Welford{p[0], p[1], p[2]});
+        }
+        w = wave_reduce(w);
+        if (tid == 0) {
+            s_scale_shift[0] = w.mean;
+            s_scale_shift[1] = rsqrtf(w.m2 / (float)L + eps);
+        }
+    }
+    __syncthreads();
+    apply_chunk<VEC, ACT, RES, T>(x, nullptr, gamma, beta, res, res2, c1, y, L, HW, C, cpg, G, s_scale_shift[0],
+                                  s_scale_shift[1]);
+}
+
+template <bool VEC, int ACT, bool RES, typename T>
+__device__ __forceinline__ void apply_chunk(const T* __restrict__ x, const float* __restrict__ pb,
+                                            const float* __restrict__ gamma, const float* __restrict__ beta,
+                                            const T* __restrict__ res, const T* __restrict__ res2, int c1,
+                                            T* __restrict__ y, int64_t L, int HW, int C, int cpg, int G, float mean,
+                                            float rstd) {
+    const int chunk = blockIdx.x, seg = blockIdx.y, tid = threadIdx.x;
     const int g = seg % G;
     const int64_t start = (int64_t)chunk * kChunk;
     const int n_local = (int)min((int64_t)kChunk, L - start);
@@ -359,6 +401,47 @@
                                     stream_, residual2, c1);
 }
 
+extern "C" int tsplat_group_norm_apply_fwd(const float* x, const float* partials, int32_t slots, const float* gamma,
+                                           const float* beta, const float* residual, const float* residual2,
+                                           int32_t c1, float* y, int32_t n, int32_t c, int64_t hw, int32_t groups,
+                                           float eps, int32_t act, void* stream_) {
+    using namespace tsplat::gn;
+    if (!x || !partials || slots <= 0 || !gamma || !beta || !y) return TSPLAT_EINVAL;
+    if (!residual2) c1 = c;
+    if (c1 <= 0 || c1 > c || (c1 < c && !residual)) return TSPLAT_EINVAL;
+    if (n <= 0 || c <= 0 || hw <= 0 || groups <= 0 || c % groups || act < 0 || act > 3 || hw > INT32_MAX)
+        return TSPLAT_EINVAL;
+    const int cpg = c / groups;
+    const int64_t L = (int64_t)cpg * hw;
+    const int64_t S = (L + kChunk - 1) / kChunk;
+    if (S > INT32_MAX || (int64_t)n * groups > 65535) return TSPLAT_EINVAL;
+    hipStream_t stream = (hipStream_t)stream_;
+    const dim3 grid((unsigned)S, (unsigned)(n * groups));
+    const bool vec = (hw % 4 == 0) && ((uintptr_t)x % 16 == 0) && ((uintptr_t)y % 16 == 0) &&
+                     (!residual || (uintptr_t)residual % 16 == 0) && (!residual2 || (uintptr_t)residual2 % 16 == 0);
+    TSPLAT_PROF_BEGIN(prof::kGroupNorm, stream);
+#define TSPLAT_GN_APPLY(V, A, R)                                                                             \
+    hipLaunchKernelGGL((apply_slots_kernel<V, A, R, float>), grid, dim3(kThreads), 0, stream, x, partials, slots, \
+                       gamma, beta, residual, residual2, c1, y, L, (int)hw, c, cpg, groups, eps)
+#define TSPLAT_GN_ACT(V, R)                      \
+    switch (act) {                               \
+        case 0: TSPLAT_GN_APPLY(V, 0, R); break; \
+        case 1: TSPLAT_GN_APPLY(V, 1, R); break; \
+        case 2: TSPLAT_GN_APPLY(V, 2, R); break; \
+        default: TSPLAT_GN_APPLY(V, 3, R); break; \
+    }
+    if (vec) {
+        if (residual) { TSPLAT_GN_ACT(true, true) } else { TSPLAT_GN_ACT(true, false) }
+    } else {
+        if (residual) { TSPLAT_GN_ACT(false, true) } else { TSPLAT_GN_ACT(false, false) }
+    }
+#undef TSPLAT_GN_ACT
+#undef TSPLAT_GN_APPLY
+    TSPLAT_PROF_END(prof::kGroupNorm, stream);
+    TSPLAT_CHECK_LAUNCH();
+    return TSPLAT_OK;
+}
+
 extern "C" int tsplat_group_norm_bf16_fwd(const void* x, const float* pre_bias, const float* gamma,
                                           const float* beta, const void* residual, void* y, void* workspace,
                                           int32_t n, int32_t c, int64_t hw, int32_t groups, float eps, int32_t act,
diff --git a/transplat_amd/csrc/winoconv3.hip b/transplat_amd/csrc/winoconv3.hip
--- a/transplat_amd/csrc/winoconv3.hip
+++ b/transplat_amd/csrc/winoconv3.hip
@@ -47,6 +47,8 @@
     const float* res;
     const float* res2;
     int cob_base;
+    float* gnp;
+    int cpg;
 };
 
 __device__ __forceinline__ float act_fn(float v, int act) {
@@ -181,7 +183,7 @@
     static constexpr int kMaxFloats = T == 32 ? 16 * (4 * 72 + 8) : 16 * (4 * 136 + 8);
 };
 
-template <int CB, int NB, int KS, bool ST>
+template <int CB, int NB, int KS, bool ST, bool GS = false>
 __global__ void __launch_bounds__(256 * CB * KS, (NB == 1 && CB * KS <= 2) ? 2 : 1) conv_kernel(Args a) {
     constexpr int T = 32 * NB;
     constexpr int GT = 256 * CB;
@@ -407,6 +409,15 @@
     }
     __syncthreads();
     W3_STAMP(2);
+    constexpr int GNT = GS ? CO * T / (256 * CB * KS) : 1;
+    float gbias[GNT];
+    if constexpr (GS) {
+#pragma unroll
+        for (int k = 0; k < GNT; ++k) {
+            const int o = (a.cob_base + cbk * CB) * 32 + (tid + 256 * CB * KS * k) / T;
+            gbias[k] = a.bias && o < a.co ? a.bias[o] : 0.0f;
+        }
+    }
     float* zs = reinterpret_cast<float*>(smem) + kg * (8 * CO * T);
 #pragma unroll
     for (int nb = 0; nb < NB; ++nb)
@@ -430,6 +441,10 @@
         __syncthreads();
     }
     const size_t hw = (size_t)a.h * a.w;
+    if constexpr (GS) {
+#pragma unroll
+        for (int k = 0; k < GNT; ++k) asm volatile("" : "+v"(gbias[k]));
+    }
     for (int pidx = tid; pidx < CO * T; pidx += 256 * CB * KS) {
         const int col = pidx / T, t2 = pidx % T;
         const int o = (a.cob_base + cbk * CB) * 32 + col;
@@ -452,11 +467,11 @@
             const int px = 2 * otx;
             float* p = dst + (size_t)py * a.w + px;
             const size_t off = ((size_t)pt.img * a.co + o) * hw + (size_t)py * a.w + px;
-            if (a.res) {
+            if (!GS && a.res) {
                 r0 += a.res[off];
                 if (px + 1 < a.w) r1 += a.res[off + 1];
             }
-            if (a.res2) {
+            if (!GS && a.res2) {
                 r0 += a.res2[off];
                 if (px + 1 < a.w) r1 += a.res2[off + 1];
             }
@@ -466,6 +481,75 @@
                 p[0] = r0;
                 if (px + 1 < a.w) p[1] = r1;
             }
+        }
+    }
+    if constexpr (GS) {
+        constexpr int NTH = 256 * CB * KS, NT = CO * T / NTH, NW = NTH / 64;
+        static_assert(CO * T % NTH == 0, "whole trips");
+        __shared__ float sRed[2 * NT * NW];
+        const int epg = a.cpg * T / 64;
+        const int ty0 = (blk / a.bx) * a.tby, tx0 = (blk % a.bx) * a.tbx;
+        const float cnt = (float)(a.cpg * (min(a.h, 2 * (ty0 + a.tby)) - 2 * ty0) * (min(a.w, 2 * (tx0 + a.tbx)) - 2 * tx0));
+        float v[NT][4];
+        bool ok[NT][4];
+#pragma unroll
+        for (int k = 0; k < NT; ++k) {
+            const int pidx = tid + NTH * k;
+            const int col = pidx / T, t2 = pidx % T;
+            const int o = (a.cob_base + cbk * CB) * 32 + col;
+            const int oty = ty0 + t2 / a.tbx, otx = tx0 + t2 % a.tbx;
+            const bool tok = o < a.co && oty < a.th && otx < a.tw;
+            const float bv = gbias[k];
+            float z[4][2];
+#pragma unroll
+            for (int r = 0; r < 4; ++r)
+#pragma unroll
+                for (int j = 0; j < 2; ++j) z[r][j] = z0[((r * 2 + j) * CO + col) * T + t2];
+            float s = 0.0f;
+#pragma unroll
+            for (int i = 0; i < 2; ++i)
+#pragma unroll
+                for (int j = 0; j < 2; ++j) {
+                    const float yv = i == 0 ? z[0][j] + z[1][j] + z[2][j] : z[1][j] - z[2][j] - z[3][j];
+                    ok[k][2 * i + j] = tok && 2 * oty + i < a.h && 2 * otx + j < a.w;
+                    v[k][2 * i + j] = ok[k][2 * i + j] ? yv + bv : 0.0f;
+                }
+            s = (v[k][0] + v[k][1]) + (v[k][2] + v[k][3]);
+#pragma unroll
+            for (int off = 32; off > 0; off >>= 1) s += __shfl_xor(s, off);
+            if (lane == 0) sRed[NW * k + wid] = s;
+        }
+        asm volatile("s_waitcnt lgkmcnt(0)" ::: "memory");
+        __builtin_amdgcn_s_barrier();
+#pragma unroll
+        for (int k = 0; k < NT; ++k) {
+            const int e0 = (NW * k + wid) / epg * epg;
+            float t = 0.0f;
+            for (int e = 0; e < epg; ++e) t += sRed[e0 + e];
+            const float mean = t / cnt;
+            float q = 0.0f;
+#pragma unroll
+            for (int e = 0; e < 4; ++e) {
+                const float dd = v[k][e] - mean;
+                q += ok[k][e] ? dd * dd : 0.0f;
+            }
+#pragma unroll
+            for (int off = 32; off > 0; off >>= 1) q += __shfl_xor(q, off);
+            if (lane == 0) sRed[NT * NW + NW * k + wid] = q;
+        }
+        asm volatile("s_waitcnt lgkmcnt(0)" ::: "memory");
+        __builtin_amdgcn_s_barrier();
+        const int o0 = (a.cob_base + cbk * CB) * 32 + tid * a.cpg;
+        if (tid < CO / a.cpg && o0 < a.co) {
+            float t = 0.0f, q = 0.0f;
+            for (int e = 0; e < epg; ++e) {
+                t += sRed[tid * epg + e];
+                q += sRed[NT * NW + tid * epg + e];
+            }
+            float* p = a.gnp + (((size_t)pt.img * (a.co / a.cpg) + o0 / a.cpg) * (a.bx * a.by) + blk) * 3;
+            p[0] = cnt;
+            p[1] = t / cnt;
+            p[2] = q;
         }
     }
     W3_STAMP(3);
@@ -737,10 +821,34 @@
     return wg32 <= 256 ? 2 : 1;
 }
 
+static bool tail_split(int form, int co) {
+    static const bool tail = !getenv("TSPLAT_WINO3_TAIL") || atoi(getenv("TSPLAT_WINO3_TAIL")) != 0;
+    return form == 4 && tail && co > 64 && co % 64 != 0 && co % 64 <= 32;
+}
+
+static int wino3_gn_form(int n, int h, int w, int co, int groups, int form) {
+    if (n <= 0 || h <= 0 || w <= 0 || co <= 0 || groups <= 0 || co % groups || form < 0 || form > 6) return 0;
+    if (form == 0) form = pick_form(n, (h + 1) / 2, (w + 1) / 2, co);
+    if (form == 5) form = 1;
+    if (tail_split(form, co)) return 0;
+    const int cpg = co / groups, cob = form == 4 || form == 6 ? 64 : 32, tiles = form == 3 || form == 4 ? 64 : 32;
+    if (cob % cpg || (cpg * tiles) % 64) return 0;
+    return form;
+}
+
 template <int CB, int NB, int KS>
 static void launch(wino3::Args a, int blocks, bool staged, hipStream_t stream, hipEvent_t start, hipEvent_t stop,
                    int coblocks = -1) {
     if (coblocks < 0) coblocks = (a.co - 32 * a.cob_base + 32 * CB - 1) / (32 * CB);
+    if (a.gnp) {
+        if (staged)
+            hipExtLaunchKernelGGL((wino3::conv_kernel<CB, NB, KS, true, true>), dim3(blocks, coblocks),
+                                  dim3(256 * CB * KS), 0, stream, start, stop, 0, a);
+        else
+            hipExtLaunchKernelGGL((wino3::conv_kernel<CB, NB, KS, false, true>), dim3(blocks, coblocks),
+                                  dim3(256 * CB * KS), 0, stream, start, stop, 0, a);
+        return;
+    }
     if (staged)
         hipExtLaunchKernelGGL((wino3::conv_kernel<CB, NB, KS, true>), dim3(blocks, coblocks), dim3(256 * CB * KS), 0,
                               stream, start, stop, 0, a);
@@ -749,10 +857,37 @@
                               0, stream, start, stop, 0, a);
 }
 
-extern "C" int tsplat_conv3x3_wino_bf16x3_ex_fwd(const float* const* srcs, const int32_t* chans, int32_t nsrc,
-                                                 const void* packed, const float* bias, const float* residual,
-                                                 const float* residual2, float* y, int32_t n, int32_t h, int32_t w,
-                                                 int32_t co, int32_t act, int32_t relu_in, void* stream_) {
+static bool wino3_geometry(wino3::Args& a, int ttiles) {
+    long best = -1;
+    for (int tbx = ttiles; tbx >= ttiles / 8; tbx /= 2) {
+        const int tby = ttiles / tbx;
+        const long padded = (long)((a.tw + tbx - 1) / tbx) * tbx * ((a.th + tby - 1) / tby) * tby;
+        if (best < 0 || padded < best) {
+            best = padded;
+            a.tbx = tbx;
+        }
+    }
+    a.tby = ttiles / a.tbx;
+    a.bx = (a.tw + a.tbx - 1) / a.tbx;
+    a.by = (a.th + a.tby - 1) / a.tby;
+    return (2 * a.tby + 2) * (a.tbx / 2 + 2) <= (ttiles == 32 ? 72 : 136);
+}
+
+extern "C" int32_t tsplat_conv3x3_wino_gn_slots(int32_t n, int32_t h, int32_t w, int32_t co, int32_t groups,
+                                                int32_t form) {
+    form = wino3_gn_form(n, h, w, co, groups, form);
+    if (!form) return 0;
+    wino3::Args a;
+    a.th = (h + 1) / 2;
+    a.tw = (w + 1) / 2;
+    if (!wino3_geometry(a, form == 3 || form == 4 ? 64 : 32)) return 0;
+    return a.bx * a.by;
+}
+
+static int wino3_launch(const float* const* srcs, const int32_t* chans, int32_t nsrc, const void* packed,
+                        const float* bias, const float* residual, const float* residual2, float* y, float* partials,
+                        int32_t groups, int32_t gn_form, int32_t n, int32_t h, int32_t w, int32_t co, int32_t act,
+                        int32_t relu_in, void* stream_) {
     if (!srcs || !chans || nsrc <= 0 || nsrc > wino3::kMaxSrc || !packed || !y || n <= 0 || h <= 0 || w <= 0 ||
         co <= 0 || act < 0 || act > 2)
         return TSPLAT_EINVAL;
@@ -784,22 +919,11 @@
     a.res = residual;
     a.res2 = residual2;
     a.cob_base = 0;
-    int form = pick_form(n, a.th, a.tw, co);
-    auto geometry = [&](int ttiles) {
-        long best = -1;
-        for (int tbx = ttiles; tbx >= ttiles / 8; tbx /= 2) {
-            const int tby = ttiles / tbx;
-            const long padded = (long)((a.tw + tbx - 1) / tbx) * tbx * ((a.th + tby - 1) / tby) * tby;
-            if (best < 0 || padded < best) {
-                best = padded;
-                a.tbx = tbx;
-            }
-        }
-        a.tby = ttiles / a.tbx;
-        a.bx = (a.tw + a.tbx - 1) / a.tbx;
-        a.by = (a.th + a.tby - 1) / a.tby;
-        return (2 * a.tby + 2) * (a.tbx / 2 + 2) <= (ttiles == 32 ? 72 : 136);
-    };
+    a.gnp = partials;
+    a.cpg = partials ? co / groups : 0;
+    int form = partials ? wino3_gn_form(n, h, w, co, groups, gn_form) : pick_form(n, a.th, a.tw, co);
+    if (!form) return TSPLAT_EINVAL;
+    auto geometry = [&](int ttiles) { return wino3_geometry(a, ttiles); };
     if (!geometry(form == 3 || form == 4 ? 64 : 32)) return TSPLAT_EINVAL;
     const int blocks = n * a.bx * a.by;
     bool staged = w % 4 == 0;
@@ -818,8 +942,7 @@
         TSPLAT_CHECK_LAUNCH();
         return TSPLAT_OK;
     }
-    static const bool tail = !getenv("TSPLAT_WINO3_TAIL") || atoi(getenv("TSPLAT_WINO3_TAIL")) != 0;
-    if (form == 4 && tail && co > 64 && co % 64 != 0 && co % 64 <= 32) {
+    if (tail_split(form, co)) {
         launch<2, 2, 1>(a, blocks, staged, stream, ev.start, nullptr, co / 64);
         if (!geometry(32)) return TSPLAT_EINVAL;
         a.cob_base = (co / 64) * 2;
@@ -838,6 +961,24 @@
     return TSPLAT_OK;
 }
 
+extern "C" int tsplat_conv3x3_wino_bf16x3_ex_fwd(const float* const* srcs, const int32_t* chans, int32_t nsrc,
+                                                 const void* packed, const float* bias, const float* residual,
+                                                 const float* residual2, float* y, int32_t n, int32_t h, int32_t w,
+                                                 int32_t co, int32_t act, int32_t relu_in, void* stream_) {
+    return wino3_launch(srcs, chans, nsrc, packed, bias, residual, residual2, y, nullptr, 0, 0, n, h, w, co, act,
+                        relu_in, stream_);
+}
+
+extern "C" int tsplat_conv3x3_wino_bf16x3_gn_fwd(const float* const* srcs, const int32_t* chans, int32_t nsrc,
+                                                 const void* packed, const float* bias, float* y, float* partials,
+                                                 int32_t n, int32_t h, int32_t w, int32_t co, int32_t groups,
+                                                 int32_t relu_in, int32_t form, void* stream_) {
+    if (!partials || (reinterpret_cast<uintptr_t>(partials) & 3) || (reinterpret_cast<uintptr_t>(y) & 15))
+        return TSPLAT_EINVAL;
+    return wino3_launch(srcs, chans, nsrc, packed, bias, nullptr, nullptr, y, partials, groups, form, n, h, w, co, 0,
+                        relu_in, stream_);
+}
+
 extern "C" int tsplat_conv3x3_wino_bf16x3_cat_fwd(const float* const* srcs, const int32_t* chans, int32_t nsrc,
                                                   const void* packed, const float* bias, float* y, int32_t n,
                                                   int32_t h, int32_t w, int32_t co, int32_t act, void* stream_) {
diff --git a/transplat_amd/kernels.py b/transplat_amd/kernels.py
--- a/transplat_amd/kernels.py
+++ b/transplat_amd/kernels.py
@@ -1246,6 +1246,108 @@
     return y
 
 
+_GN_CONV_STATS = os.environ.get("TSPLAT_GN_CONV_STATS", "1")
+GN_SINGLE_LAUNCH_MAX = 16384
+
+
+def conv3x3_few_gn(srcs, weight, bias, num_groups: int, relu_in: bool = False, form: int = 0):
+    import ctypes
+
+    lib = _lib.load()
+    srcs = [_f32(t) for t in srcs]
+    n, _, h, w = srcs[0].shape
+    co, ci = weight.shape[0], sum(t.shape[1] for t in srcs)
+    slots = int(lib.tsplat_conv3x3_few_gn_slots(n, ci, h, w, co, num_groups, form))
+    if slots == 0 or any(t.data_ptr() % 16 for t in srcs):
+        return None
+    y = torch.empty((n, co, h, w), dtype=torch.float32, device=srcs[0].device)
+    partials = torch.empty((n, num_groups, slots, 3), dtype=torch.float32, device=y.device)
+    pb = _f32(bias) if bias is not None else None
+    ptrs = (ctypes.c_void_p * len(srcs))(*[_lib.ptr(t) for t in srcs])
+    chans = (ctypes.c_int32 * len(srcs))(*[t.shape[1] for t in srcs])
+    rc = lib.tsplat_conv3x3_few_bf16x3_gn_fwd(
+        ctypes.cast(ptrs, ctypes.c_void_p), ctypes.cast(chans, ctypes.c_void_p), len(srcs),
+        _lib.ptr(conv_pack_weight_x3(weight)), _lib.ptr(pb), _lib.ptr(y), _lib.ptr(partials), n, h, w, co,
+        num_groups, int(relu_in), form, _lib.stream_ptr(y.device))
+    _lib.check(rc, "tsplat_conv3x3_few_bf16x3_gn_fwd")
+    return y, partials, slots
+
+
+def conv3x3_wino_gn(srcs, weight, bias, num_groups: int, relu_in: bool = False, form: int = 0):
+    import ctypes
+
+    lib = _lib.load()
+    srcs = [_f32(t) for t in srcs]
+    n, _, h, w = srcs[0].shape
+    co = weight.shape[0]
+    slots = int(lib.tsplat_conv3x3_wino_gn_slots(n, h, w, co, num_groups, form))
+    if slots == 0:
+        return None
+    y = torch.empty((n, co, h, w), dtype=torch.float32, device=srcs[0].device)
+    partials = torch.empty((n, num_groups, slots, 3), dtype=torch.float32, device=y.device)
+    pb = _f32(bias) if bias is not None else None
+    ptrs = (ctypes.c_void_p * len(srcs))(*[_lib.ptr(t) for t in srcs])
+    chans = (ctypes.c_int32 * len(srcs))(*[t.shape[1] for t in srcs])
+    rc = lib.tsplat_conv3x3_wino_bf16x3_gn_fwd(
+        ctypes.cast(ptrs, ctypes.c_void_p), ctypes.cast(chans, ctypes.c_void_p), len(srcs),
+        _lib.ptr(wino_pack_weight_bf16x3(weight)), _lib.ptr(pb), _lib.ptr(y), _lib.ptr(partials), n, h, w, co,
+        num_groups, int(relu_in), form, _lib.stream_ptr(y.device))
+    _lib.check(rc, "tsplat_conv3x3_wino_bf16x3_gn_fwd")
+    return y, partials, slots
+
+
+def group_norm_apply(x, partials, num_groups: int, weight, bias, eps: float, act: str = "none", residual=None):
+    lib = _lib.load()
+    n, c = x.shape[:2]
+    hw = x[0, 0].numel()
+    if tuple(partials.shape[:2]) != (n, num_groups) or partials.shape[-1] != 3 or not partials.is_contiguous():
+        raise ValueError(f"partials {tuple(partials.shape)} for input {tuple(x.shape)}, {num_groups} groups")
+    r1 = r2 = None
+    c1 = c
+    if isinstance(residual, (tuple, list)):
+        r1, r2 = (_f32(r) for r in residual)
+        c1 = r1.shape[1]
+        if (r1.shape[0] != n or r2.shape[0] != n or c1 + r2.shape[1] != c or r1.shape[2:] != x.shape[2:]
+                or r2.shape[2:] != x.shape[2:]):
+            raise ValueError(f"residual parts {tuple(r1.shape)} + {tuple(r2.shape)} != input {tuple(x.shape)}")
+    elif residual is not None:
+        r1 = _f32(residual)
+        if r1.shape != x.shape:
+            raise ValueError(f"residual {tuple(r1.shape)} != input {tuple(x.shape)}")
+    y = torch.empty_like(x)
+    rc = lib.tsplat_group_norm_apply_fwd(_lib.ptr(x), _lib.ptr(partials), partials.shape[2], _lib.ptr(_f32(weight)),
+                                         _lib.ptr(_f32(bias)), _lib.ptr(r1), _lib.ptr(r2), c1, _lib.ptr(y), n, c, hw,
+                                         num_groups, float(eps), _ACTS[act], _lib.stream_ptr(x.device))
+    _lib.check(rc, "tsplat_group_norm_apply_fwd")
+    return y
+
+
+def conv_gn_act(conv, norm, x, act: str = "none", residual=None, extra=(), unfused=None, force=False):
+    srcs = (x, *extra)
+    co = conv.weight.shape[0]
+    g = norm.num_groups
+    fused = ((force or _GN_CONV_STATS != "0") and x.is_cuda and x.dim() == 4 and conv.weight.dim() == 4
+             and getattr(conv, "padding_mode", "zeros") == "zeros"
+             and conv3x3_wino_ok(x, conv.weight, conv.stride, conv.padding, conv.dilation, conv.groups, extra,
+                                 force=bool(force)))
+    kernel = force
+    if fused and not force:
+        n, _, h, w = x.shape
+        fused = (split_mode() and co % g == 0 and (co // g) * h * w > GN_SINGLE_LAUNCH_MAX
+                 and not conv2d_direct_ok(x, conv.weight, 1, conv.padding, c2=sum(t.shape[1] for t in extra)))
+        kernel = "few" if fused and _few_ok([_f32(t) for t in srcs], n, h, w, co) else "wino"
+        fused = fused and _GN_CONV_STATS in ("1", kernel)
+    if fused:
+        out = (conv3x3_few_gn if kernel == "few" else conv3x3_wino_gn)(srcs, conv.weight, conv.bias, g)
+        if out is not None:
+            return group_norm_apply(out[0], out[1], g, norm.weight, norm.bias, norm.eps, act, residual)
+    if unfused is None:
+        unfused = lambda with_bias: conv3x3_wino(x, conv.weight, conv.bias if with_bias else None, extra=extra,
+                                                 precision="bf16x3")
+    y = unfused(conv.bias is None)
+    return group_norm(y, g, norm.weight, norm.bias, norm.eps, act, residual, pre_bias=conv.bias).type(y.dtype)
+
+
 _CONV_BF16 = os.environ.get("TSPLAT_CONV_BF16", "1") != "0"
 _BF16_PACKED: dict = {}
 
diff --git a/transplat_amd/model/encoder/matching/ldm_unet.py b/transplat_amd/model/encoder/matching/ldm_unet.py
--- a/transplat_amd/model/encoder/matching/ldm_unet.py
+++ b/transplat_amd/model/encoder/matching/ldm_unet.py
@@ -77,6 +77,9 @@
 
 
 def conv_gn_act(conv_mod: nn.Module, norm: nn.GroupNorm, x, act: str = "none", residual=None, x2=None):
+    if isinstance(conv_mod, nn.Conv2d):
+        return kernels.conv_gn_act(conv_mod, norm, x, act, residual, (x2,) if x2 is not None else (),
+                                   unfused=lambda bias: conv(conv_mod, x, x2, bias=bias))
     if conv_mod.bias is None:
         return gn_act(norm, conv(conv_mod, x, x2), act, residual)
     return gn_act(norm, conv_nobias(conv_mod, x, x2), act, residual, pre_bias=conv_mod.bias)
diff --git a/transplat_amd/routes.py b/transplat_amd/routes.py
--- a/transplat_amd/routes.py
+++ b/transplat_amd/routes.py
@@ -18,9 +18,11 @@
     "tsplat_conv3x3_wino_bf16x3_fwd": ("3x3 convs (HIP Winograd)", "bf16x3"),
     "tsplat_conv3x3_wino_bf16x3_ex_fwd": ("3x3 convs (HIP Winograd)", "bf16x3"),
     "tsplat_conv3x3_wino_bf16x3_cat_fwd": ("3x3 convs (HIP Winograd)", "bf16x3"),
+    "tsplat_conv3x3_wino_bf16x3_gn_fwd": ("3x3 convs (HIP Winograd)", "bf16x3"),
     "tsplat_conv3x3_wino_f32_fwd": ("3x3 convs (HIP Winograd)", "exact fp32"),
     "tsplat_conv3x3_wino_cat_f32_fwd": ("3x3 convs (HIP Winograd)", "exact fp32"),
     "tsplat_conv3x3_few_bf16x3_fwd": ("direct convs (HIP)", "bf16x3"),
+    "tsplat_conv3x3_few_bf16x3_gn_fwd": ("direct convs (HIP)", "bf16x3"),
     "tsplat_conv2d_bf16x3_fwd": ("direct convs (HIP)", "bf16x3"),
     "tsplat_conv2d_f32_fwd": ("direct convs (HIP)", "exact fp32"),
     "tsplat_conv2d_f32_zsplit_fwd": ("direct convs (HIP)", "exact fp32"),
@@ -43,6 +45,7 @@
     "tsplat_ms_deform_attn_fwd": ("correlation (HIP)", "fp32"),
     "tsplat_group_norm_fwd": ("norms (HIP)", "fp32"),
     "tsplat_group_norm_cat_res_fwd": ("norms (HIP)", "fp32"),
+    "tsplat_group_norm_apply_fwd": ("norms (HIP)", "fp32"),
     "tsplat_group_norm_bf16_fwd": ("norms (HIP)", "bf16 I/O, fp32 statistics"),
     "tsplat_layer_norm128_fwd": ("norms (HIP)", None),
     "tsplat_residual_ln_fwd": ("norms (HIP)", "fp32"),
```
